# sohamazing/image-stitcher

Hardware: AMD Instinct MI355X
Metric: stitched Mvoxels/s (higher is better)
Workload: dtype u16

## Files before the change

### image-stitcher_amd/csrc/fuse.hip

```cpp
#include "fuse_device.h"

namespace {

template <typename T, int FLAT>
struct Slot {
    static constexpr int VEC = Pix<T>::N;
    u32x4 px;
    f32x4 g32[FLAT == 1 ? VEC / 4 : 1];
    f64x2 g64[FLAT == 2 ? VEC / 2 : 1];
    T edge;
    float eg32;
    double eg64;
};

template <typename T, int FLAT>
__device__ __forceinline__ void slot_load(Slot<T, FLAT> &S, const Row<T> &J, int lane, int k) {
    constexpr int VEC = Pix<T>::N;
    const int v = lane + 64 * k;
    if (v >= J.v_first && v < J.v_end) {
        const int p0 = v * VEC - J.mis;
        S.px = ldg<U32x4U>(J.srow + p0);
        if (FLAT == 1 && J.frow) {
#pragma unroll
            for (int q = 0; q < VEC / 4; ++q) S.g32[q] = ldg<F32x4U>(reinterpret_cast<const float *>(J.frow) + p0 + 4 * q);
// ... 136 lines not shown
                row_zero<T>(d - head, n + head, lane, leave_tail);
            } else {
                row_zero<T>(d, n, lane, leave_tail);
            }
        }
        return;
    }
    for (int rb = wave; rb < rows; rb += 4 * RB) {
        Row<T> J[RB];
#pragma unroll
        for (int j = 0; j < RB; ++j) {
            const int r = rb + 4 * j;
            J[j].n = r < rows ? n : 0;
            J[j].drow = canvas + (int64_t)(it.dst_y + r) * P.canvas_pitch + it.dst_x;
            J[j].srow = tile + (int64_t)(it.b + r) * P.tile_pitch + it.c;
            J[j].frow = flat ? flat + ((int64_t)(it.b + r) * P.tile_w + it.c) * FSZ : nullptr;
            const bool lt = has_left && !lzero;
            J[j].lsrow = lt ? ltile + (int64_t)(seam.b + r) * P.tile_pitch + seam.c : J[j].srow;
            J[j].lfrow = (lt && flat) ? flat + ((int64_t)(seam.b + r) * P.tile_w + seam.c) * FSZ : J[j].frow;
            row_setup<T>(J[j], lane, sflags);
        }
        if (fast) pipeline_rows<T, FLAT, true, RND, RB, SLOTS, DEPTH>(J, lane);
        else pipeline_rows<T, FLAT, false, RND, RB, SLOTS, DEPTH>(J, lane);
    }
}

struct PlaneAux {
    const void *tile, *ltile;
    Seam seam;
};
template <typename T>
__device__ __forceinline__ PlaneAux plane_aux(const FuseParams &P, int plane, const Item &it, int64_t pos) {
    PlaneAux A;
    A.tile = it.nref ? tile_ptr<T>(P, plane, it.a) : nullptr;
    A.seam = (sizeof(T) == 2 && P.seams) ? P.seams[pos] : Seam{-1, 0, 0, 0};
    A.ltile = ((A.seam.flags & SEAM_HAS_LEFT) && !(A.seam.flags & SEAM_LEFT_ZERO)) ? tile_ptr<T>(P, plane, A.seam.a) : nullptr;
    return A;
}

template <typename T, int FLAT, bool DYN>
__global__ __launch_bounds__(256, (FLAT == 1 ? (sizeof(T) == 2 ? WAVES_F32 : 1) : (FLAT == 2 ? WAVES_F64 : WAVES_PLAIN)))
void fuse_overwrite_kernel(const FuseParams P, const int64_t n_items, const int64_t n_work) {
    const int wave = __builtin_amdgcn_readfirstlane(threadIdx.x >> 6);
    const int lane = threadIdx.x & 63;

    if (!DYN) {
        int64_t work = blockIdx.x;
        if (work >= n_work) return;
        int plane = (int)(work / n_items);
        Item it = P.items[work - plane * n_items];
        PlaneAux A = plane_aux<T>(P, plane, it, work - plane * n_items);
        while (true) {
            const int64_t nwork = work + gridDim.x;
            const bool more = nwork < n_work;
            int nplane = plane;
            Item nit = it;
            PlaneAux nA = A;
            if (more) {
                nplane = (int)(nwork / n_items);
                nit = P.items[nwork - nplane * n_items];
                nA = plane_aux<T>(P, nplane, nit, nwork - nplane * n_items);
            }
            process_item<T, FLAT>(P, plane, it, static_cast<const T *>(A.tile), wave, lane, A.seam, static_cast<const T *>(A.ltile));
            if (!more) break;
            work = nwork;
            plane = nplane;
            it = nit;
            A = nA;
        }
        return;
    }
    for_each_queued_item<PlaneAux>(
        P, n_items, (uint32_t)P.n_planes,
        [&](int plane, const Item &it, int64_t pos) -> PlaneAux { return plane_aux<T>(P, plane, it, pos); },
        [&](int plane, const Item &it, const PlaneAux &A) {
            process_item<T, FLAT>(P, plane, it, sgpr(static_cast<const T *>(A.tile)), wave, lane, sgpr(A.seam),
                                  sgpr(static_cast<const T *>(A.ltile)));
        });
}

struct UnitAux {
    PlaneGroup g;
    const void *tile[ZB];
    const void *ltile[ZB];
    Seam seam;
    Seam first;
};
struct FeatherAux : UnitAux {
    Seam xref[2];
    const void *xtile[2][ZB];
};

template <bool FULL, int RND = 0, typename G = float, typename T = uint16_t>
__device__ __forceinline__ void process_item_zg(const FuseParams &P, const UnitAux &A, const int gn, const Item &it,
                                                const int wave, const int lane) {
    constexpr bool GAINS = !std::is_same<G, NoGain>::value;
    typedef typename std::conditional<GAINS, G, float>::type GT;
    constexpr uint32_t GSZ = sizeof(GT), TSZ = sizeof(T), TMAX = sizeof(T) == 1 ? 255u : 65535u;
    constexpr int VEC = 16 / (int)sizeof(T), LINE = 128 / (int)sizeof(T);
    constexpr int SLOTS = BLOCK_COLS / VEC / 64 + 1;
    const int rows = it.hw >> 16, n = it.hw & 0xFFFF;
    const int sflags = sizeof(T) == 2 ? sgpr(A.seam.flags) : 0;
    const bool leave_tail = sflags & SEAM_LEAVE_TAIL;
    T *cplane[ZB];
    const T *tiles[ZB];
#pragma unroll
    for (int z = 0; z < ZB; ++z) {
        const int zz = (FULL || z < gn) ? z : 0;
        cplane[z] = static_cast<T *>(P.canvas) + (int64_t)sgpr(A.g.plane[zz]) * P.canvas_plane_stride;
        tiles[z] = sgpr(static_cast<const T *>(A.tile[zz]));
    }
    if (!it.nref) {
        const bool has_left = sflags & SEAM_HAS_LEFT, lzero = sflags & SEAM_LEFT_ZERO;
        for (int r = wave; r < rows; r += 4) {
            const int64_t doff = (int64_t)(it.dst_y + r) * P.canvas_pitch + it.dst_x;
            const int mis = (int)((reinterpret_cast<uintptr_t>(cplane[0] + doff) / sizeof(T)) & (LINE - 1));
            const int head = (has_left && mis > 0) ? mis : 0;
            if (head && !lzero) {
                const int p = lane - mis;
                const bool left = p < 0;
                const int po = left ? p : -1;
                const int sb = sgpr(A.seam.b), sc = sgpr(A.seam.c);
                GT eg = GT(1), er = GT(1);
                if constexpr (GAINS) {
                    const GT *lflat = static_cast<const GT *>(P.flat_ptrs[sgpr(A.g.plane[0])]);
                    eg = ldg_s<GT>(reinterpret_cast<const char *>(lflat + (int64_t)(sb + r) * P.tile_w + sc) + po * (int)GSZ);
                    er = recip_of<RND>(eg);
                }
#pragma unroll
                for (int z = 0; z < ZB; ++z)
                    if (FULL || z < gn) {
                        const T *lt = sgpr(static_cast<const T *>(A.ltile[z]));
                        const T e = ldg_s<T>(reinterpret_cast<const char *>(lt + (int64_t)(sb + r) * P.tile_pitch + sc) + po * (int)TSZ);
                        uint32_t kq = e;
                        if constexpr (GAINS) kq = min(cvt_u32_sat(quot_of<RND>((GT)e, eg, er)), TMAX);
                        if (!left) kq = 0u;
                        stg_s<T>(reinterpret_cast<char *>(cplane[z] + doff) + p * (int)TSZ, (T)kq);
                    }
            }
#pragma unroll
            for (int z = 0; z < ZB; ++z)
                if (FULL || z < gn) {
                    T *d = cplane[z] + doff;
                    if (head && lzero) row_zero<T>(d - head, n + head, lane, leave_tail);
                    else if (head) row_zero<T>(d + (LINE - head), n - (LINE - head), lane, leave_tail);
                    else row_zero<T>(d, n, lane, leave_tail);
                }
        }
        return;
    }
    const GT *flat = nullptr;
    if constexpr (GAINS) flat = static_cast<const GT *>(P.flat_ptrs[sgpr(A.g.plane[0])]);
    for (int r = wave; r < rows; r += 4) {
        const int64_t doff = (int64_t)(it.dst_y + r) * P.canvas_pitch + it.dst_x;
        const int64_t soff = (int64_t)(it.b + r) * P.tile_pitch + it.c;
        const char *frow = GAINS ? reinterpret_cast<const char *>(flat + (int64_t)(it.b + r) * P.tile_w + it.c) : nullptr;
        const char *srow[ZB];
        char *drow[ZB];
#pragma unroll
        for (int z = 0; z < ZB; ++z) {
            srow[z] = reinterpret_cast<const char *>(tiles[z] + soff);
            drow[z] = reinterpret_cast<char *>(cplane[z] + doff);
        }
        const int mis = (int)((reinterpret_cast<uintptr_t>(drow[0]) / sizeof(T)) & (LINE - 1));
        const bool head_line = (sflags & SEAM_HAS_LEFT) && mis > 0;
        const int n_own = leave_tail ? n - ((n + mis) & (LINE - 1)) : n;
        const int v_first = head_line ? LINE / VEC : (mis + VEC - 1) / VEC, v_end = (n_own + mis) / VEC;
#pragma unroll
        for (int k = 0; k < SLOTS; ++k) {
            if (64 * k >= v_end || v_end <= v_first) break;
            const int v = lane + 64 * k;
            const bool act = v >= v_first && v < v_end;
            const int p0 = v * VEC - mis;
            const uint32_t o = (uint32_t)min(max(p0, v_first * VEC - mis), (v_end - 1) * VEC - mis);
            GT g[VEC], rc[VEC];
            if constexpr (GAINS) load_gains(frow + o * GSZ, g);
            u32x4 px[ZB];
#pragma unroll
            for (int z = 0; z < ZB; ++z)
                if (FULL || z < gn) px[z] = ldg<U32x4U>(srow[z] + o * TSZ);
            if constexpr (GAINS) {
#pragma unroll
                for (int c = 0; c < VEC; ++c) rc[c] = recip_of<RND>(g[c]);
            }
#pragma unroll
            for (int z = 0; z < ZB; ++z)
                if (FULL || z < gn) {
                    u32x4 ov = px[z];
                    if constexpr (GAINS) {
#pragma unroll
                        for (int c = 0; c < 4; ++c) {
                            if constexpr (sizeof(T) == 2) ov[c] = quot_pair<RND, GT>(px[z][c], g[2 * c], g[2 * c + 1], rc[2 * c], rc[2 * c + 1]);
                            else ov[c] = quot_quad<RND, GT>(px[z][c], &g[4 * c], &rc[4 * c]);
                        }
                    }
                    if (act) stg_nt_at(drow[z], o * TSZ, ov);
                }
        }
        if (head_line) {
            const int p = lane - mis;
            const bool left = p < 0, lzero = sflags & SEAM_LEFT_ZERO;
            const int sb = sgpr(A.seam.b), sc = sgpr(A.seam.c);
            const int po = (left && lzero) ? 0 : p;
            GT eg = GT(1), er = GT(1);
            if constexpr (GAINS) {
                const char *lfrow = lzero ? frow : reinterpret_cast<const char *>(flat + (int64_t)(sb + r) * P.tile_w + sc);
                eg = ldg_s<GT>((left ? lfrow : frow) + po * (int)GSZ);
            }
            T e[ZB];
#pragma unroll
            for (int z = 0; z < ZB; ++z)
                if (FULL || z < gn) {
                    const T *lt = sgpr(static_cast<const T *>(A.ltile[z]));
                    const char *lrow = lzero ? srow[z] : reinterpret_cast<const char *>(lt + (int64_t)(sb + r) * P.tile_pitch + sc);
                    e[z] = ldg_s<T>((left ? lrow : srow[z]) + po * (int)TSZ);
                }
            if constexpr (GAINS) er = recip_of<RND>(eg);
#pragma unroll
            for (int z = 0; z < ZB; ++z)
                if (FULL || z < gn) {
                    uint32_t kq = e[z];
                    if constexpr (GAINS) kq = min(cvt_u32_sat(quot_of<RND>((GT)e[z], eg, er)), TMAX);
                    if (left && lzero) kq = 0;
                    stg_s<T>(drow[z] + p * (int)TSZ, (T)kq);
                }
        }
        const int head_end = head_line ? 0 : min(n_own, v_first * VEC - mis);
        const int tail_start = max(head_end, v_end * VEC - mis);
        int ep = -1;
        if (lane < VEC) {
            if (lane < head_end) ep = lane;
        } else if (lane < 2 * VEC) {
            if (tail_start + (lane - VEC) < n_own) ep = tail_start + (lane - VEC);
        }
        if (__builtin_amdgcn_ballot_w64(ep >= 0)) {
            const uint32_t eo = (uint32_t)max(ep, 0);
            GT eg = GT(1), er = GT(1);
            if constexpr (GAINS) eg = ldg_s<GT>(frow + eo * GSZ);
            T e[ZB];
#pragma unroll
            for (int z = 0; z < ZB; ++z)
                if (FULL || z < gn) e[z] = ldg_s<T>(srow[z] + eo * TSZ);
            if constexpr (GAINS) er = recip_of<RND>(eg);
#pragma unroll
            for (int z = 0; z < ZB; ++z)
                if (FULL || z < gn) {
                    uint32_t kq = e[z];
                    if constexpr (GAINS) kq = min(cvt_u32_sat(quot_of<RND>((GT)e[z], eg, er)), TMAX);
                    if (ep >= 0) stg_s<T>(drow[z] + eo * TSZ, (T)kq);
                }
        }
    }
}

constexpr int WAVES_ZG = 1;
template <typename G, bool DYN, typename T = uint16_t>
__global__ __launch_bounds__(256, WAVES_ZG) void fuse_overwrite_zg_kernel(const FuseParams P, const int64_t n_items) {
    constexpr int FLAT = std::is_same<G, NoGain>::value ? 0 : (sizeof(G) == 8 ? 2 : 1);
    const int wave = __builtin_amdgcn_readfirstlane(threadIdx.x >> 6);
    const int lane = threadIdx.x & 63;
    const uint32_t n_groups = *P.n_groups;
    auto pre = [&](int unit, const Item &it, int64_t pos) -> UnitAux {
        UnitAux A;
        A.g = P.groups[unit];
        A.seam = P.seams ? P.seams[pos] : Seam{-1, 0, 0, 0};
        const bool left_tile = (A.seam.flags & SEAM_HAS_LEFT) && !(A.seam.flags & SEAM_LEFT_ZERO);
#pragma unroll
        for (int z = 0; z < ZB; ++z) {
            A.tile[z] = (it.nref && z < A.g.n) ? tile_ptr<T>(P, A.g.plane[z], it.a) : nullptr;
            A.ltile[z] = (left_tile && z < A.g.n) ? tile_ptr<T>(P, A.g.plane[z], A.seam.a) : nullptr;
        }
        return A;
    };
    auto body = [&](int, const Item &it, const UnitAux &A) {
        const int gn = sgpr(A.g.n);
        if (gn == 1) {
            process_item<T, FLAT>(P, sgpr(A.g.plane[0]), it, sgpr(static_cast<const T *>(A.tile[0])), wave, lane, sgpr(A.seam),
                                  sgpr(static_cast<const T *>(A.ltile[0])));
        } else if (gn == ZB) {
            process_item_zg<true, 0, G, T>(P, A, gn, it, wave, lane);
        } else {
            process_item_zg<false, 0, G, T>(P, A, gn, it, wave, lane);
        }
    };
    if (DYN) {
        for_each_queued_item<UnitAux>(P, n_items, n_groups, pre, body);
    } else {
        __shared__ Item s_it;
        __shared__ UnitAux s_A;
        const int64_t n_work = (int64_t)n_groups * n_items;
        for (int64_t work = blockIdx.x; work < n_work; work += gridDim.x) {
            __syncthreads();
            if (threadIdx.x == 0) {
                const int unit = (int)(work / n_items);
                s_it = P.items[work - unit * n_items];
                s_A = pre(unit, s_it, work - unit * n_items);
            }
            __syncthreads();
            body(0, sgpr(s_it), s_A);
        }
    }
}

__global__ __launch_bounds__(256) void build_groups_kernel(const void *const *flat_ptrs, const uint32_t *cls, uint32_t cls_mask,
                                                          int n_planes, int64_t plane_stride_bytes, int zb, uint32_t *n_groups,
                                                          PlaneGroup *groups, bool consecutive) {
    constexpr int CAP = 1024;
    __shared__ uint64_t key[CAP];
    __shared__ int first[CAP], open_group[CAP];
    __shared__ short members[CAP], dealt[CAP];
    __shared__ PlaneGroup out[CAP];
    const int tid = threadIdx.x;
    if (n_planes > CAP || zb <= 1) {
        for (int p = tid; p < n_planes; p += 256) {
            PlaneGroup g{};
            g.n = 1;
            g.plane[0] = p;
            groups[p] = g;
        }
        if (tid == 0) *n_groups = (uint32_t)n_planes;
        return;
    }
    for (int p = tid; p < n_planes; p += 256) {
        const void *f = flat_ptrs ? flat_ptrs[p] : nullptr;
        const bool ok = flat_ptrs ? (f && (cls[p] & cls_mask) == 0) : true;
        key[p] = ok ? ((reinterpret_cast<uint64_t>(f) << 7) | (uint64_t)(((int64_t)p * plane_stride_bytes) & 127) | (1ull << 63)) : 0;
        open_group[p] = -1;
    }
    __syncthreads();
    for (int p = tid; p < n_planes; p += 256) {
        int f = p;
        if (key[p])
            for (int q = 0; q < p; ++q)
                if (key[q] == key[p]) {
                    f = q;
                    break;
                }
        first[p] = f;
    }
    __syncthreads();
    if (tid == 0) {
        int ng = 0;
        for (int p = 0; p < n_planes; ++p) members[p] = dealt[p] = 0;
        for (int p = 0; p < n_planes; ++p)
            if (key[p]) ++members[first[p]];
        for (int p = 0; p < n_planes; ++p) {
            if (!key[p]) {
                open_group[p] = ng++;
            } else if (first[p] == p) {
                open_group[p] = ng;
                ng += (members[p] + zb - 1) / zb;
            }
        }
        for (int g = 0; g < ng; ++g) out[g].n = 0;
        for (int p = 0; p < n_planes; ++p) {
            int g = open_group[p];
            if (key[p]) {
                const int lead = first[p];
                const int j = dealt[lead]++;
                g = open_group[lead] + (consecutive ? j / zb : j % ((members[lead] + zb - 1) / zb));
            }
            out[g].plane[out[g].n++] = p;
        }
        for (int g = 0; g < ng; ++g)
            for (int z = out[g].n; z < 7; ++z) out[g].plane[z] = out[g].plane[0];
        *n_groups = (uint32_t)ng;
        first[0] = ng;
    }
    __syncthreads();
    const int ng = first[0];
    for (int g = tid; g < ng; g += 256) groups[g] = out[g];
}

template <typename OutT>
__device__ __forceinline__ OutT feather_out(float o) {
    if (sizeof(OutT) == 4) return (OutT)o;
    const float hi = sizeof(OutT) == 1 ? 255.0f : 65535.0f;
    return (OutT)fminf(fmaxf(rintf(o), 0.0f), hi);
}

constexpr int BLEND_MAXR = 4;

template <typename T, typename OutT, int FLAT, bool FAST>
__device__ __forceinline__ void blend_group(const FuseParams &P, int plane, const Item &it, const char *flat, int r, int p0,
                                            OutT *dst) {
    constexpr int VEC = 8;
    constexpr int MAXR = BLEND_MAXR;
    const int nref = it.nref;
    float acc[VEC], wsum[VEC], last[VEC];
#pragma unroll
    for (int e = 0; e < VEC; ++e) acc[e] = wsum[e] = last[e] = 0.0f;
    auto blend = [&](const float (&px)[VEC], int y, int x0) {
        const int wy = min(y + 1, P.tile_h - y);
#pragma unroll
        for (int e = 0; e < VEC; ++e) {
            const int x = x0 + e;
            const float w = (float)min(min(x + 1, P.tile_w - x), wy);
            acc[e] = __fadd_rn(acc[e], __fmul_rn(w, px[e]));
            wsum[e] = __fadd_rn(wsum[e], w);
            last[e] = px[e];
        }
    };
    if (sizeof(T) == 2 && FLAT != 2 && nref <= MAXR) {
        u32x4 raw[MAXR];
        f32x4 g[MAXR][2];
        int ys[MAXR], xs[MAXR];
#pragma unroll
        for (int k = 0; k < MAXR; ++k)
            if (k < nref) {
                const Ref rf = P.refs[it.a + k];
                ys[k] = rf.src_y + it.b + r;
                xs[k] = rf.src_x + it.c + p0;
                raw[k] = ldg<U32x4U>(tile_ptr<T>(P, plane, rf.tile) + (int64_t)ys[k] * P.tile_pitch + xs[k]);
                if (FLAT == 1 && flat) {
                    const float *gp = reinterpret_cast<const float *>(flat) + (int64_t)ys[k] * P.tile_w + xs[k];
                    g[k][0] = ldg<F32x4U>(gp);
                    g[k][1] = ldg<F32x4U>(gp + 4);
                }
            }
#pragma unroll
        for (int k = 0; k < MAXR; ++k)
            if (k < nref) {
                float px[VEC];
#pragma unroll
                for (int e = 0; e < VEC; ++e) {
                    px[e] = (float)Pix<uint16_t>::get(raw[k], e);
                    if (FLAT == 1 && flat) px[e] = FAST ? div_u16_normal_ieee(px[e], g[k][e >> 2][e & 3]) : __fdiv_rn(px[e], g[k][e >> 2][e & 3]);
                }
                blend(px, ys[k], xs[k]);
            }
    } else {
        for (int k = 0; k < nref; ++k) {
            const Ref rf = P.refs[it.a + k];
            const T *tile = tile_ptr<T>(P, plane, rf.tile);
            const int y = rf.src_y + it.b + r;
            const int x0 = rf.src_x + it.c + p0;
            const T *src = tile + (int64_t)y * P.tile_pitch + x0;
            float px[VEC];
            if (sizeof(T) == 2) {
                const u32x4 raw = ldg<U32x4U>(src);
#pragma unroll
                for (int e = 0; e < VEC; ++e) px[e] = (float)Pix<uint16_t>::get(raw, e);
            } else {
#pragma unroll
                for (int e = 0; e < VEC; ++e) px[e] = (float)ldg_s<T>(src + e);
            }
            if (FLAT && flat) {
#pragma unroll
                for (int e = 0; e < VEC; ++e) {
                    const char *gp = flat + ((int64_t)y * P.tile_w + x0 + e) * (FLAT == 2 ? 8 : 4);
                    const float gain = FLAT == 2 ? (float)ldg_s<double>(gp) : ldg_s<float>(gp);
                    px[e] = FAST ? div_u16_normal_ieee(px[e], gain) : __fdiv_rn(px[e], gain);
                }
            }
            blend(px, y, x0);
        }
    }
    OutT o[VEC];
#pragma unroll
    for (int e = 0; e < VEC; ++e) o[e] = feather_out<OutT>(nref == 1 ? last[e] : (nref ? __fdiv_rn(acc[e], wsum[e]) : 0.0f));
    if (sizeof(OutT) == 2) {
        u32x4 out;
#pragma unroll
        for (int q = 0; q < 4; ++q) out[q] = (uint32_t)(uint16_t)o[2 * q] | ((uint32_t)(uint16_t)o[2 * q + 1] << 16);
        stg_nt(dst, out);
    } else if (sizeof(OutT) == 4) {
        u32x4 lo, hi;
#pragma unroll
        for (int q = 0; q < 4; ++q) {
            lo[q] = __float_as_uint((float)o[q]);
            hi[q] = __float_as_uint((float)o[4 + q]);
        }
        stg_nt(dst, lo);
        stg_nt(dst + 4, hi);
    } else {
#pragma unroll
        for (int e = 0; e < VEC; ++e) stg_s<OutT>(dst + e, o[e]);
    }
}

template <typename T, typename OutT, int FLAT, bool FAST>
__device__ __forceinline__ void blend_item(const FuseParams &P, int plane, const Item &it, int tid) {
    constexpr int VEC = 8;
    const int rows = it.hw >> 16, n = it.hw & 0xFFFF;
    const int nref = it.nref;
    OutT *canvas = static_cast<OutT *>(P.canvas) + plane * P.canvas_plane_stride;
    const char *flat = (FLAT && P.flat_ptrs) ? static_cast<const char *>(P.flat_ptrs[plane]) : nullptr;
    const int G = n / VEC + 1;
    auto locate = [&](int idx, int &r, int &p0, OutT *&dst) -> bool {
        r = idx / G;
        const int j = idx - r * G;
        OutT *drow = canvas + (int64_t)(it.dst_y + r) * P.canvas_pitch + it.dst_x;
        const int mis = (int)((reinterpret_cast<uintptr_t>(drow) / sizeof(OutT)) & (VEC - 1));
        const int v = (mis ? 1 : 0) + j;
        p0 = v * VEC - mis;
        dst = drow + p0;
        return v < (n + mis) / VEC;
    };
    for (int idx = tid; idx < rows * G; idx += 256) {
        int r, p0;
        OutT *dst;
        if (!locate(idx, r, p0, dst)) continue;
        blend_group<T, OutT, FLAT, FAST>(P, plane, it, flat, r, p0, dst);
    }
    for (int idx = tid; idx < rows * 2 * VEC; idx += 256) {
        const int r = idx / (2 * VEC), l = idx - r * 2 * VEC;
        OutT *drow = canvas + (int64_t)(it.dst_y + r) * P.canvas_pitch + it.dst_x;
        const int mis = (int)((reinterpret_cast<uintptr_t>(drow) / sizeof(OutT)) & (VEC - 1));
        const int v_first = mis ? 1 : 0, v_end = (n + mis) / VEC;
        const int head_end = min(n, v_first * VEC - mis);
        const int tail_start = max(head_end, v_end * VEC - mis);
        int p = -1;
        if (l < VEC) {
            if (l < head_end) p = l;
        } else if (tail_start + (l - VEC) < n) {
            p = tail_start + (l - VEC);
        }
        if (p < 0) continue;
        float acc = 0.0f, wsum = 0.0f, last = 0.0f;
        for (int k = 0; k < nref; ++k) {
            const Ref rf = P.refs[it.a + k];
            const int y = rf.src_y + it.b + r, x = rf.src_x + it.c + p;
            float v = (float)ldg_s<T>(tile_ptr<T>(P, plane, rf.tile) + (int64_t)y * P.tile_pitch + x);
            if (FLAT && flat) {
                const char *gp = flat + ((int64_t)y * P.tile_w + x) * (FLAT == 2 ? 8 : 4);
                const float gain = FLAT == 2 ? (float)ldg_s<double>(gp) : ldg_s<float>(gp);
                v = FAST ? div_u16_normal_ieee(v, gain) : __fdiv_rn(v, gain);
            }
            const float w = (float)min(min(x + 1, P.tile_w - x), min(y + 1, P.tile_h - y));
            acc = __fadd_rn(acc, __fmul_rn(w, v));
            wsum = __fadd_rn(wsum, w);
            last = v;
        }
        stg_s<OutT>(drow + p, feather_out<OutT>(nref == 1 ? last : (nref ? __fdiv_rn(acc, wsum) : 0.0f)));
    }
}

template <typename T, typename OutT, int FLAT>
__device__ __forceinline__ void feather_one_item(const FuseParams &P, int plane, const Item &it, int wave, int lane) {
    const int nref = it.nref;
    if (sizeof(OutT) == sizeof(T) && FLAT != 2 && nref <= 1) {
        Item one = it;
        const T *tile = nullptr;
        if (nref) {
            const Ref rf = P.refs[it.a];
            tile = tile_ptr<T>(P, plane, rf.tile);
            one.a = rf.tile;
            one.b = rf.src_y + it.b;
            one.c = rf.src_x + it.c;
        }
        process_item<T, FLAT == 2 ? 0 : FLAT, 1>(P, plane, one, tile, wave, lane);
        return;
    }
    const bool fast = FLAT == 1 && P.flat_class && (P.flat_class[plane] & 1u) == 0;
    if (fast) blend_item<T, OutT, FLAT, true>(P, plane, it, threadIdx.x);
    else blend_item<T, OutT, FLAT, false>(P, plane, it, threadIdx.x);
}

constexpr int WAVES_FEATHER_F32 = 4;
template <typename T, typename OutT, int FLAT, bool DYN>
__global__ __launch_bounds__(256, (FLAT == 1 && sizeof(T) == 2 && sizeof(OutT) == 2 ? WAVES_FEATHER_F32 : 1))
void fuse_feather_kernel(const FuseParams P, const int64_t n_items, const int64_t n_work) {
    const int wave = __builtin_amdgcn_readfirstlane(threadIdx.x >> 6);
    const int lane = threadIdx.x & 63;
    if (DYN) {
        for_each_queued_item<int>(P, n_items, (uint32_t)P.n_planes, [](int, const Item &, int64_t) -> int { return 0; },
                                  [&](int plane, const Item &it, const int &) { feather_one_item<T, OutT, FLAT>(P, plane, it, wave, lane); });
    } else {
        for (int64_t work = blockIdx.x; work < n_work; work += gridDim.x) {
            const int plane = (int)(work / n_items);
            feather_one_item<T, OutT, FLAT>(P, plane, P.items[work - plane * n_items], wave, lane);
        }
    }
}

__device__ __forceinline__ float div_by_refined(float n, float d, float r) {
    const float q = n * r;
    return fmaf(fmaf(-d, q, n), r, q);
}

template <int FLAT, bool FULL, typename OutT = uint16_t, int NREF = 2>
__device__ __forceinline__ void blend_item_zg(const FuseParams &P, const UnitAux &A, const int gn, const Item &it, const int tid) {
    typedef uint16_t T;
    constexpr int VEC = 8;
    constexpr bool F32OUT = sizeof(OutT) == 4;
    static_assert(NREF == 2 || F32OUT, "one-tile and empty items of an integer canvas take process_item_zg");
    const int rows = it.hw >> 16, n = it.hw & 0xFFFF;
    OutT *cplane[ZB];
    const T *t0[ZB], *t1[ZB];
#pragma unroll
    for (int z = 0; z < ZB; ++z) {
        const int zz = (FULL || z < gn) ? z : 0;
        cplane[z] = static_cast<OutT *>(P.canvas) + (int64_t)sgpr(A.g.plane[zz]) * P.canvas_plane_stride;
        t0[z] = sgpr(static_cast<const T *>(A.tile[zz]));
        t1[z] = sgpr(static_cast<const T *>(A.ltile[zz]));
    }
    typedef typename std::conditional<FLAT == 2, double, float>::type GM;
    const GM *flat = (FLAT && NREF) ? static_cast<const GM *>(P.flat_ptrs[sgpr(A.g.plane[0])]) : nullptr;
    const int ya = sgpr(A.first.b), xa = sgpr(A.first.c), yb = sgpr(A.seam.b), xb = sgpr(A.seam.c);
    const int G = n / VEC + 1;
    auto load_gain8 = [&](int y, int x, f32x2 (&g)[4]) {
        if constexpr (FLAT == 1) {
            const float *gp = reinterpret_cast<const float *>(flat) + (int64_t)y * P.tile_w + x;
            const f32x4 a = ldg<F32x4U>(gp), b = ldg<F32x4U>(gp + 4);
            g[0] = f32x2{a[0], a[1]}, g[1] = f32x2{a[2], a[3]}, g[2] = f32x2{b[0], b[1]}, g[3] = f32x2{b[2], b[3]};
        } else if constexpr (FLAT == 2) {
            const double *gp = reinterpret_cast<const double *>(flat) + (int64_t)y * P.tile_w + x;
#pragma unroll
            for (int h = 0; h < 4; ++h) {
                const f64x2 a = ldg<F64x2U>(gp + 2 * h);
                g[h] = f32x2{(float)a[0], (float)a[1]};
            }
        }
    };
    auto refined = [](f32x2 d) {
        const f32x2 r = {__builtin_amdgcn_rcpf(d[0]), __builtin_amdgcn_rcpf(d[1])};
        return pk_fma(pk_fma(-d, r, f32x2{1.0f, 1.0f}), r, r);
    };
    for (int idx = tid; idx < rows * G; idx += 256) {
        const int r = idx / G, j = idx - r * G;
        const int64_t doff = (int64_t)(it.dst_y + r) * P.canvas_pitch + it.dst_x;
        const int mis = (int)((reinterpret_cast<uintptr_t>(cplane[0] + doff) / sizeof(OutT)) & (VEC - 1));
        const int v = (mis ? 1 : 0) + j;
        if (v >= (n + mis) / VEC) continue;
        const int p0 = v * VEC - mis;
        if constexpr (NREF == 0) {
            const u32x4 zero = {0u, 0u, 0u, 0u};
#pragma unroll
            for (int z = 0; z < ZB; ++z)
                if (FULL || z < gn) {
                    stg_nt(cplane[z] + doff + p0, zero);
                    stg_nt(cplane[z] + doff + p0 + 4, zero);
                }
            continue;
        }
        const int y0 = ya + r, x0 = xa + p0, y1 = yb + r, x1 = xb + p0;
        const int64_t s0 = (int64_t)y0 * P.tile_pitch + x0, s1 = (int64_t)y1 * P.tile_pitch + x1;
        f32x2 g0[4], g1[4];
        if constexpr (FLAT != 0) {
            load_gain8(y0, x0, g0);
            if constexpr (NREF == 2) load_gain8(y1, x1, g1);
        }
        u32x4 ra[ZB], rb[ZB];
#pragma unroll
        for (int z = 0; z < ZB; ++z)
            if (FULL || z < gn) {
                ra[z] = ldg<U32x4U>(t0[z] + s0);
                if constexpr (NREF == 2) rb[z] = ldg<U32x4U>(t1[z] + s1);
            }
        f32x2 r0[4], r1[4], w0[4], w1[4], ws[4], rw[4];
        const int wy0 = min(y0 + 1, P.tile_h - y0), wy1 = min(y1 + 1, P.tile_h - y1);
#pragma unroll
        for (int h = 0; h < 4; ++h) {
            if constexpr (FLAT != 0) {
                r0[h] = refined(g0[h]);
                if constexpr (NREF == 2) r1[h] = refined(g1[h]);
            }
            if constexpr (NREF == 2) {
#pragma unroll
                for (int c = 0; c < 2; ++c) {
                    const int e = 2 * h + c;
                    w0[h][c] = (float)min(min(x0 + e + 1, P.tile_w - (x0 + e)), wy0);
                    w1[h][c] = (float)min(min(x1 + e + 1, P.tile_w - (x1 + e)), wy1);
                }
                ws[h] = w0[h] + w1[h];
                rw[h] = refined(ws[h]);
            }
        }
#pragma unroll
        for (int z = 0; z < ZB; ++z)
            if (FULL || z < gn) {
                f32x2 o[4];
#pragma unroll
                for (int h = 0; h < 4; ++h) {
// ... 169 lines not shown
            }
    }
    for (int idx = tid; idx < rows * 2 * VEC; idx += 256) {
        const int r = idx / (2 * VEC), l = idx - r * 2 * VEC;
        const int64_t doff = (int64_t)(it.dst_y + r) * P.canvas_pitch + it.dst_x;
        const int mis = (int)((reinterpret_cast<uintptr_t>(cplane[0] + doff) / sizeof(float)) & (VEC - 1));
        const int v_first = mis ? 1 : 0, v_end = (n + mis) / VEC;
        const int head_end = min(n, v_first * VEC - mis);
        const int tail_start = max(head_end, v_end * VEC - mis);
        int p = -1;
        if (l < VEC) {
            if (l < head_end) p = l;
        } else if (tail_start + (l - VEC) < n) {
            p = tail_start + (l - VEC);
        }
        if (p < 0) continue;
        if constexpr (NREF == 0) {
#pragma unroll
            for (int z = 0; z < ZB; ++z)
                if (FULL || z < gn) stg_s<float>(cplane[z] + doff + p, 0.0f);
            continue;
        }
        const int y0 = ya + r, x0 = xa + p, y1 = yb + r, x1 = xb + p;
        const float fa = FLAT ? recip_for<1>(ldg_s<float>(flat + (int64_t)y0 * P.tile_w + x0)) : 1.0f;
        const float fb = (FLAT && NREF == 2) ? recip_for<1>(ldg_s<float>(flat + (int64_t)y1 * P.tile_w + x1)) : 1.0f;
        const float wa = (float)min(min(x0 + 1, P.tile_w - x0), min(y0 + 1, P.tile_h - y0));
        const float wb = (float)min(min(x1 + 1, P.tile_w - x1), min(y1 + 1, P.tile_h - y1));
        const float rws = recip_for<1>(__fadd_rn(wa, wb));
#pragma unroll
        for (int z = 0; z < ZB; ++z)
            if (FULL || z < gn) {
                float va = (float)ldg_s<T>(t0[z] + (int64_t)y0 * P.tile_pitch + x0);
                if (FLAT) va = __fmul_rn(va, fa);
                float o = va;
                if constexpr (NREF == 2) {
                    float vb = (float)ldg_s<T>(t1[z] + (int64_t)y1 * P.tile_pitch + x1);
                    if (FLAT) vb = __fmul_rn(vb, fb);
                    o = __fmul_rn(__fadd_rn(__fmul_rn(wa, va), __fmul_rn(wb, vb)), rws);
                }
                stg_s<float>(cplane[z] + doff + p, o);
            }
    }
}

template <int FLAT, bool FULL, typename OutT>
__device__ __forceinline__ void blend_item_zgn(const FuseParams &P, const FeatherAux &A, const int gn, const Item &it, const int tid) {
    static_assert(FLAT == 0 || FLAT == 1, "float32 gains or none");
    typedef uint16_t T;
    constexpr int VEC = 8, MAXR = 4;
    constexpr bool F32OUT = sizeof(OutT) == 4;
    const int rows = it.hw >> 16, n = it.hw & 0xFFFF;
    const bool four = sgpr((int)it.nref) == 4;
    OutT *cplane[ZB];
    const T *tp[MAXR][ZB];
#pragma unroll
    for (int z = 0; z < ZB; ++z) {
        const int zz = (FULL || z < gn) ? z : 0;
        cplane[z] = static_cast<OutT *>(P.canvas) + (int64_t)sgpr(A.g.plane[zz]) * P.canvas_plane_stride;
        tp[0][z] = sgpr(static_cast<const T *>(A.tile[zz]));
        tp[1][z] = sgpr(static_cast<const T *>(A.ltile[zz]));
        tp[2][z] = sgpr(static_cast<const T *>(A.xtile[0][zz]));
        tp[3][z] = sgpr(static_cast<const T *>(A.xtile[1][zz]));
    }
    const float *flat = FLAT ? static_cast<const float *>(P.flat_ptrs[sgpr(A.g.plane[0])]) : nullptr;
    const int ry[MAXR] = {sgpr(A.first.b), sgpr(A.seam.b), sgpr(A.xref[0].b), sgpr(A.xref[1].b)};
    const int rx[MAXR] = {sgpr(A.first.c), sgpr(A.seam.c), sgpr(A.xref[0].c), sgpr(A.xref[1].c)};
    const int G = n / VEC + 1;
    auto refined = [](f32x2 d) {
        const f32x2 r = {__builtin_amdgcn_rcpf(d[0]), __builtin_amdgcn_rcpf(d[1])};
        return pk_fma(pk_fma(-d, r, f32x2{1.0f, 1.0f}), r, r);
    };
    for (int idx = tid; idx < rows * G; idx += 256) {
        const int r = idx / G, j = idx - r * G;
        const int64_t doff = (int64_t)(it.dst_y + r) * P.canvas_pitch + it.dst_x;
        const int mis = (int)((reinterpret_cast<uintptr_t>(cplane[0] + doff) / sizeof(OutT)) & (VEC - 1));
        const int v = (mis ? 1 : 0) + j;
        if (v >= (n + mis) / VEC) continue;
        const int p0 = v * VEC - mis;
        f32x2 acc[ZB][4], ws[4];
#pragma unroll
        for (int k = 0; k < MAXR; ++k)
            if (k < 3 || four) {
                const int y = ry[k] + r, x = rx[k] + p0;
                const int64_t so = (int64_t)y * P.tile_pitch + x;
                f32x2 g[4], rr[4], w[4];
                if constexpr (FLAT != 0) {
                    const float *gp = flat + (int64_t)y * P.tile_w + x;
                    const f32x4 a = ldg<F32x4U>(gp), b = ldg<F32x4U>(gp + 4);
                    g[0] = f32x2{a[0], a[1]}, g[1] = f32x2{a[2], a[3]}, g[2] = f32x2{b[0], b[1]}, g[3] = f32x2{b[2], b[3]};
                }
                u32x4 raw[ZB];
#pragma unroll
                for (int z = 0; z < ZB; ++z)
                    if (FULL || z < gn) raw[z] = ldg<U32x4U>(tp[k][z] + so);
                const int wy = min(y + 1, P.tile_h - y);
#pragma unroll
                for (int h = 0; h < 4; ++h) {
                    if constexpr (FLAT != 0) rr[h] = refined(g[h]);
#pragma unroll
                    for (int c = 0; c < 2; ++c) w[h][c] = (float)min(min(x + 2 * h + c + 1, P.tile_w - (x + 2 * h + c)), wy);
                    ws[h] = k == 0 ? w[h] : ws[h] + w[h];
                }
#pragma unroll
                for (int z = 0; z < ZB; ++z)
                    if (FULL || z < gn) {
#pragma unroll
                        for (int h = 0; h < 4; ++h) {
                            f32x2 px = {(float)(raw[z][h] & 0xFFFFu), (float)(raw[z][h] >> 16)};
                            if constexpr (FLAT != 0) px = F32OUT ? px * rr[h] : div_by_refined2(px, g[h], rr[h]);
                            const f32x2 t = w[h] * px;
                            acc[z][h] = k == 0 ? t : acc[z][h] + t;
                        }
                    }
            }
        f32x2 rw[4];
#pragma unroll
        for (int h = 0; h < 4; ++h) rw[h] = refined(ws[h]);
#pragma unroll
        for (int z = 0; z < ZB; ++z)
            if (FULL || z < gn) {
                f32x2 o[4];
#pragma unroll
                for (int h = 0; h < 4; ++h) o[h] = F32OUT ? acc[z][h] * rw[h] : div_by_refined2(acc[z][h], ws[h], rw[h]);
                if constexpr (F32OUT) {
                    u32x4 lo, hi;
#pragma unroll
                    for (int q = 0; q < 2; ++q) {
                        lo[2 * q] = __float_as_uint(o[q][0]), lo[2 * q + 1] = __float_as_uint(o[q][1]);
                        hi[2 * q] = __float_as_uint(o[2 + q][0]), hi[2 * q + 1] = __float_as_uint(o[2 + q][1]);
                    }
                    stg_nt(cplane[z] + doff + p0, lo);
                    stg_nt(cplane[z] + doff + p0 + 4, hi);
                } else {
                    typedef unsigned short u16x2 __attribute__((ext_vector_type(2)));
                    u32x4 out;
#pragma unroll
                    for (int q = 0; q < 4; ++q) {
                        const u16x2 pk = __builtin_amdgcn_cvt_pk_u16(cvt_u32_sat(__builtin_rintf(o[q][0])), cvt_u32_sat(__builtin_rintf(o[q][1])));
                        out[q] = (uint32_t)pk[0] | ((uint32_t)pk[1] << 16);
                    }
                    stg_nt(cplane[z] + doff + p0, out);
                }
            }
    }
    for (int idx = tid; idx < rows * 2 * VEC; idx += 256) {
        const int r = idx / (2 * VEC), l = idx - r * 2 * VEC;
        const int64_t doff = (int64_t)(it.dst_y + r) * P.canvas_pitch + it.dst_x;
        const int mis = (int)((reinterpret_cast<uintptr_t>(cplane[0] + doff) / sizeof(OutT)) & (VEC - 1));
        const int v_first = mis ? 1 : 0, v_end = (n + mis) / VEC;
        const int head_end = min(n, v_first * VEC - mis);
        const int tail_start = max(head_end, v_end * VEC - mis);
        int p = -1;
        if (l < VEC) {
            if (l < head_end) p = l;
        } else if (tail_start + (l - VEC) < n) {
            p = tail_start + (l - VEC);
        }
        if (p < 0) continue;
        float acc[ZB], wsum = 0.0f;
#pragma unroll
        for (int k = 0; k < MAXR; ++k)
            if (k < 3 || four) {
                const int y = ry[k] + r, x = rx[k] + p;
                const float gk = FLAT ? ldg_s<float>(flat + (int64_t)y * P.tile_w + x) : 1.0f;
                const float fk = FLAT ? recip_for<1>(gk) : 1.0f;
                const float w = (float)min(min(x + 1, P.tile_w - x), min(y + 1, P.tile_h - y));
                wsum = k == 0 ? w : __fadd_rn(wsum, w);
#pragma unroll
                for (int z = 0; z < ZB; ++z)
                    if (FULL || z < gn) {
                        float px = (float)ldg_s<T>(tp[k][z] + (int64_t)y * P.tile_pitch + x);
                        if (FLAT) px = F32OUT ? __fmul_rn(px, fk) : div_by_refined(px, gk, fk);
                        const float t = __fmul_rn(w, px);
                        acc[z] = k == 0 ? t : __fadd_rn(acc[z], t);
                    }
            }
        const float rws = recip_for<1>(wsum);
#pragma unroll
        for (int z = 0; z < ZB; ++z)
            if (FULL || z < gn) {
                const float o = F32OUT ? __fmul_rn(acc[z], rws) : div_by_refined(acc[z], wsum, rws);
                if constexpr (F32OUT) stg_s<OutT>(cplane[z] + doff + p, o);
                else stg_s<OutT>(cplane[z] + doff + p, (OutT)min(cvt_u32_sat(__builtin_rintf(o)), 65535u));
            }
    }
}

constexpr int WAVES_FEATHER_ZG = 3;
template <int FLAT, bool DYN, typename OutT = uint16_t>
__global__ __launch_bounds__(256, FLAT ? WAVES_FEATHER_ZG : 1) void fuse_feather_zg_kernel(const FuseParams P, const int64_t n_items) {
    typedef uint16_t T;
    constexpr bool F32OUT = sizeof(OutT) == 4;
    const int wave = __builtin_amdgcn_readfirstlane(threadIdx.x >> 6);
    const int lane = threadIdx.x & 63;
    const uint32_t n_groups = *P.n_groups;
    auto pre = [&](int unit, const Item &it, int64_t) -> FeatherAux {
        FeatherAux A;
        A.g = P.groups[unit];
        A.seam = Seam{-1, 0, 0, 0};
        A.first = Seam{-1, 0, 0, 0};
        A.xref[0] = A.xref[1] = Seam{-1, 0, 0, 0};
        const bool one = it.nref >= 1 && it.nref <= 4, two = it.nref >= 2 && it.nref <= 4;
        Ref ra{}, rb{};
        if (one) {
            ra = P.refs[it.a];
            A.first = Seam{ra.tile, ra.src_y + it.b, ra.src_x + it.c, 0};
        }
        if (two) {
            rb = P.refs[it.a + 1];
            A.seam = Seam{rb.tile, rb.src_y + it.b, rb.src_x + it.c, 0};
        }
#pragma unroll
        for (int z = 0; z < ZB; ++z) {
            A.tile[z] = (one && z < A.g.n) ? tile_ptr<T>(P, A.g.plane[z], ra.tile) : nullptr;
            A.ltile[z] = (two && z < A.g.n) ? tile_ptr<T>(P, A.g.plane[z], rb.tile) : nullptr;
        }
#pragma unroll
        for (int k = 0; k < 2; ++k) {
            const bool have = it.nref >= 3 + k && it.nref <= 4;
            Ref rk{};
            if (have) {
                rk = P.refs[it.a + 2 + k];
                A.xref[k] = Seam{rk.tile, rk.src_y + it.b, rk.src_x + it.c, 0};
            }
#pragma unroll
            for (int z = 0; z < ZB; ++z) A.xtile[k][z] = (have && z < A.g.n) ? tile_ptr<T>(P, A.g.plane[z], rk.tile) : nullptr;
        }
        return A;
    };
    auto body = [&](int, const Item &it, const FeatherAux &A) {
        const int gn = sgpr(A.g.n);
        if (gn == 1) {
            feather_one_item<T, OutT, FLAT>(P, sgpr(A.g.plane[0]), it, wave, lane);
        } else if (F32OUT && it.nref <= 1) {
            if constexpr (F32OUT && FLAT != 2) {
                if (it.nref == 1) {
                    if (gn == ZB) blend_item_zg4<FLAT, true, 1>(P, A, gn, it, threadIdx.x);
                    else blend_item_zg4<FLAT, false, 1>(P, A, gn, it, threadIdx.x);
                } else {
                    if (gn == ZB) blend_item_zg4<FLAT, true, 0>(P, A, gn, it, threadIdx.x);
                    else blend_item_zg4<FLAT, false, 0>(P, A, gn, it, threadIdx.x);
                }
            } else if constexpr (F32OUT) {
                if (it.nref == 1) {
                    if (gn == ZB) blend_item_zg<FLAT, true, OutT, 1>(P, A, gn, it, threadIdx.x);
                    else blend_item_zg<FLAT, false, OutT, 1>(P, A, gn, it, threadIdx.x);
                } else {
                    if (gn == ZB) blend_item_zg<FLAT, true, OutT, 0>(P, A, gn, it, threadIdx.x);
                    else blend_item_zg<FLAT, false, OutT, 0>(P, A, gn, it, threadIdx.x);
                }
            }
        } else if (FLAT == 2 && it.nref <= 1) {
            for (int z = 0; z < gn; ++z) feather_one_item<T, OutT, FLAT>(P, sgpr(A.g.plane[z]), it, wave, lane);
        } else if (it.nref <= 1) {
            Item one = it;
            one.a = sgpr(A.first.a);
            one.b = sgpr(A.first.b);
            one.c = sgpr(A.first.c);
            if constexpr (FLAT == 2) {
            } else if (!FLAT) {
                for (int z = 0; z < gn; ++z)
                    process_item<T, 0, 1>(P, sgpr(A.g.plane[z]), one, sgpr(static_cast<const T *>(A.tile[z])), wave, lane);
            } else if (gn == ZB) {
                process_item_zg<true, 1>(P, A, gn, one, wave, lane);
            } else {
                process_item_zg<false, 1>(P, A, gn, one, wave, lane);
            }
        } else if (it.nref == 2) {
            if constexpr (F32OUT && FLAT != 2) {
                if (gn == ZB) blend_item_zg4<FLAT, true, 2>(P, A, gn, it, threadIdx.x);
                else blend_item_zg4<FLAT, false, 2>(P, A, gn, it, threadIdx.x);
            } else {
                if (gn == ZB) blend_item_zg<FLAT, true, OutT>(P, A, gn, it, threadIdx.x);
                else blend_item_zg<FLAT, false, OutT>(P, A, gn, it, threadIdx.x);
            }
        } else if (FLAT != 2 && it.nref <= 4) {
            if constexpr (FLAT != 2) {
                if (gn == ZB) blend_item_zgn<FLAT, true, OutT>(P, A, gn, it, threadIdx.x);
                else blend_item_zgn<FLAT, false, OutT>(P, A, gn, it, threadIdx.x);
            }
        } else {
            for (int z = 0; z < gn; ++z) blend_item<T, OutT, FLAT, true>(P, sgpr(A.g.plane[z]), it, threadIdx.x);
        }
    };
    if (DYN) {
        for_each_queued_item<FeatherAux>(P, n_items, n_groups, pre, body);
    } else {
        __shared__ Item s_it;
        __shared__ FeatherAux s_A;
        const int64_t n_work = (int64_t)n_groups * n_items;
        for (int64_t work = blockIdx.x; work < n_work; work += gridDim.x) {
            __syncthreads();
            if (threadIdx.x == 0) {
                const int unit = (int)(work / n_items);
                s_it = P.items[work - unit * n_items];
                s_A = pre(unit, s_it, work - unit * n_items);
            }
            __syncthreads();
            body(0, sgpr(s_it), s_A);
        }
    }
}

template <typename G>
__global__ __launch_bounds__(256) void flat_classify_kernel(const void *const *flat_ptrs, int64_t n, uint32_t *cls) {
    const int plane = blockIdx.y;
    const G *f = static_cast<const G *>(flat_ptrs[plane]);
    if (!f) return;
    for (int q = 0; q < plane; ++q)
        if (flat_ptrs[q] == f) return;
    const G lo = (G)__builtin_ldexp(1.0, FAST_MIN_EXP), hi = (G)__builtin_ldexp(1.0, FAST_END_EXP);
    const G mlo = (G)__builtin_ldexp(1.0, -MODERATE_EXP), mhi = (G)__builtin_ldexp(1.0, MODERATE_EXP);
    bool odd = false, wide = false, neg = false;
    auto look = [&](G g) {
        const G a = g < 0 ? -g : g;
        odd |= !(a >= lo && a < hi);
        wide |= !(a >= mlo && a < mhi);
        neg |= !(g > 0);
    };
    constexpr int PER = 16 / sizeof(G);
    const int64_t head = min<int64_t>(n, (int64_t)((16 - (reinterpret_cast<uintptr_t>(f) & 15)) & 15) / (int64_t)sizeof(G));
    const int64_t nvec = (n - head) / PER;
    const int64_t tid = (int64_t)blockIdx.x * blockDim.x + threadIdx.x, nthr = (int64_t)gridDim.x * blockDim.x;
    for (int64_t v = tid; v < nvec; v += nthr) {
        if constexpr (sizeof(G) == 4) {
            const f32x4 q = *reinterpret_cast<const f32x4 *>(f + head + v * PER);
            look(q[0]), look(q[1]), look(q[2]), look(q[3]);
        } else {
            const F64x2U q = *reinterpret_cast<const F64x2U *>(f + head + v * PER);
            look(q.v[0]), look(q.v[1]);
        }
    }
    for (int64_t i = tid; i < head; i += nthr) look(ldg_s<G>(f + i));
    for (int64_t i = head + nvec * PER + tid; i < n; i += nthr) look(ldg_s<G>(f + i));
    const uint32_t bits = (__builtin_amdgcn_ballot_w64(odd) ? 1u : 0u) | (__builtin_amdgcn_ballot_w64(wide) ? 2u : 0u) |
                          (__builtin_amdgcn_ballot_w64(neg) ? 4u : 0u);
    if (bits && (threadIdx.x & 63) == 0) atomicOr(&cls[plane], bits);
}

__global__ __launch_bounds__(256) void flat_class_share_kernel(const void *const *flat_ptrs, int n_planes, uint32_t *cls) {
    for (int p = threadIdx.x; p < n_planes; p += 256) {
        const void *f = flat_ptrs[p];
        if (!f) continue;
        for (int q = 0; q < p; ++q)
            if (flat_ptrs[q] == f) {
                cls[p] = cls[q];
                break;
            }
    }
}

__global__ __launch_bounds__(256) void selftest_divide_kernel(int exponent0, int negative, unsigned long long *bad) {
    const uint32_t mant = blockIdx.x * 256u + threadIdx.x;
    const int exponent = exponent0 + (int)blockIdx.y;
    const uint32_t bits = ((uint32_t)(exponent + 127) << 23) | mant | (negative ? 0x80000000u : 0u);
    const float g = __uint_as_float(bits);
    unsigned long long local = 0;
    for (int v = 0; v < 65536; ++v)
    {
        const uint32_t want = flat_f32<uint16_t>((uint16_t)v, g);
        const uint32_t pair = flat_f32_fast_pair((uint32_t)v | ((uint32_t)v << 16), g, g);
        local += want != flat_f32_fast<uint16_t>((uint16_t)v, g);
        local += want != (pair & 0xFFFFu);
        local += want != (pair >> 16);
        local += flat_f32<uint16_t, 1>((uint16_t)v, g) != flat_f32_fast<uint16_t, 1>((uint16_t)v, g);
        local += __fdiv_rn((float)v, g) != div_u16_normal_ieee((float)v, g);
    }
    for (int off = 32; off > 0; off >>= 1) local += __shfl_xor(local, off);
    if ((threadIdx.x & 63) == 0 && local) atomicAdd(bad, local);
}

}

extern "C" int sq_selftest_flat_divide(int32_t exponent, int32_t n_binades, int32_t negative, uint64_t *mismatches_dev,
                                       void *stream) {
    if (!mismatches_dev || exponent < FAST_MIN_EXP || n_binades < 1 || exponent + n_binades > FAST_END_EXP)
        return fail(SQ_ERR_INVALID, "sq_selftest_flat_divide: binades [%d, %d] outside the fast path's range [%d, %d]",
                    exponent, exponent + n_binades - 1, FAST_MIN_EXP, FAST_END_EXP - 1);
    hipStream_t s = static_cast<hipStream_t>(stream);
    hipError_t e = hipMemsetAsync(mismatches_dev, 0, sizeof(uint64_t), s);
    if (e == hipSuccess) {
        hipLaunchKernelGGL(selftest_divide_kernel, dim3(1u << 15, n_binades), dim3(256), 0, s, exponent, negative,
                           reinterpret_cast<unsigned long long *>(mismatches_dev));
        e = hipGetLastError();
    }
    if (e != hipSuccess) return fail(SQ_ERR_HIP, "sq_selftest_flat_divide: %s", hipGetErrorString(e));
    return SQ_OK;
}

__global__ __launch_bounds__(256) void selftest_blend_divide_kernel(int exponent0, int negative, unsigned long long *bad) {
    const uint32_t mant = blockIdx.x * 256u + threadIdx.x;
    const int exponent = exponent0 + (int)blockIdx.y;
    const float acc = __uint_as_float(((uint32_t)(exponent + 127) << 23) | mant | (negative ? 0x80000000u : 0u));
    unsigned long long local = 0;
    for (int ws = 2; ws <= BLEND_WSUM_MAX; ++ws) {
        const float d = (float)ws;
        const float want = __fdiv_rn(acc, d), got = div_by_refined(acc, d, recip_for<1>(d));
        local += __float_as_uint(want) != __float_as_uint(got);
    }
    if (local) atomicAdd(bad, local);
}

extern "C" int sq_selftest_blend_divide(int32_t exponent, int32_t n_binades, int32_t negative, uint64_t *mismatches_dev,
                                        void *stream) {
    if (!mismatches_dev || exponent < BLEND_ACC_MIN_EXP || n_binades < 1 || exponent + n_binades > BLEND_ACC_END_EXP)
        return fail(SQ_ERR_INVALID, "sq_selftest_blend_divide: binades [%d, %d] outside the blend's range [%d, %d]", exponent,
                    exponent + n_binades - 1, BLEND_ACC_MIN_EXP, BLEND_ACC_END_EXP - 1);
    hipStream_t s = static_cast<hipStream_t>(stream);
    hipError_t e = hipMemsetAsync(mismatches_dev, 0, sizeof(uint64_t), s);
    if (e == hipSuccess) {
        hipLaunchKernelGGL(selftest_blend_divide_kernel, dim3(1u << 15, n_binades), dim3(256), 0, s, exponent, negative,
                           reinterpret_cast<unsigned long long *>(mismatches_dev));
        e = hipGetLastError();
    }
    if (e != hipSuccess) return fail(SQ_ERR_HIP, "sq_selftest_blend_divide: %s", hipGetErrorString(e));
    return SQ_OK;
}

__global__ __launch_bounds__(256) void selftest_divide_f64_kernel(int exponent0, int negative, uint64_t seed, unsigned long long *bad) {
    const uint64_t id = ((uint64_t)blockIdx.y << 32) | (blockIdx.x * 256u + threadIdx.x);
    uint64_t x = seed + id * 0x9E3779B97F4A7C15ull;
    x ^= x >> 30; x *= 0xBF58476D1CE4E5B9ull; x ^= x >> 27; x *= 0x94D049BB133111EBull; x ^= x >> 31;
    const int exponent = exponent0 + (int)blockIdx.y;
    const uint32_t t = blockIdx.x * 256u + threadIdx.x;
    uint64_t mant = x & ((1ull << 52) - 1);
    if (t == 0) mant = 0;
    else if (t == 1) mant = (1ull << 52) - 1;
    else if (t < 54) mant = 1ull << (t - 2);
    else if (t < 106) mant = ((1ull << 52) - 1) ^ (1ull << (t - 54));
    const uint64_t bits = ((uint64_t)(exponent + 1023) << 52) | mant | (negative ? 0x8000000000000000ull : 0ull);
    const double g = __longlong_as_double((long long)bits);
    unsigned long long local = 0;
    for (int v = 0; v < 65536; ++v) {
        const double want = __ddiv_rn((double)v, g);
        const double got = div_u16_normal_f64((double)v, g);
        local += __double_as_longlong(want) != __double_as_longlong(got) && !(want == 0.0 && got == 0.0);
        local += flat_f64<uint16_t>((uint16_t)v, g) != flat_f64_fast<uint16_t>((uint16_t)v, g);
    }
    for (int off = 32; off > 0; off >>= 1) local += __shfl_xor(local, off);
    if ((threadIdx.x & 63) == 0 && local) atomicAdd(bad, local);
}

extern "C" int sq_selftest_flat_divide_f64(int32_t exponent, int32_t n_binades, int32_t negative, uint64_t seed,
                                           uint64_t *mismatches_dev, void *stream) {
    if (!mismatches_dev || exponent < FAST_MIN_EXP || n_binades < 1 || exponent + n_binades > FAST_END_EXP)
        return fail(SQ_ERR_INVALID, "sq_selftest_flat_divide_f64: binades [%d, %d] outside the fast path's range [%d, %d]",
                    exponent, exponent + n_binades - 1, FAST_MIN_EXP, FAST_END_EXP - 1);
    hipStream_t s = static_cast<hipStream_t>(stream);
    hipError_t e = hipMemsetAsync(mismatches_dev, 0, sizeof(uint64_t), s);
    if (e == hipSuccess) {
        hipLaunchKernelGGL(selftest_divide_f64_kernel, dim3(128, n_binades), dim3(256), 0, s, exponent, negative, seed,
                           reinterpret_cast<unsigned long long *>(mismatches_dev));
        e = hipGetLastError();
    }
    if (e != hipSuccess) return fail(SQ_ERR_HIP, "sq_selftest_flat_divide_f64: %s", hipGetErrorString(e));
    return SQ_OK;
}

extern "C" int64_t sq_fuse_scratch_bytes(int32_t n_planes) {
    if (n_planes < 0) return fail(SQ_ERR_INVALID, "sq_fuse_scratch_bytes: n_planes %d", n_planes);
    return scratch_layout(n_planes).total;
}

extern "C" int sq_fuse_planes(const sq_fuse_args *a, void *stream_) {
    static const char *who = "sq_fuse_planes";
    FuseParams P;
    int32_t fl = 0;
    if (const int rc = fuse_setup(who, a, fl, SQ_FUSE_FORCE_QUEUES | SQ_FUSE_FORCE_STATIC | SQ_FUSE_NO_PLANE_GROUPS | SQ_FUSE_NO_SEAM_OWNERS |
                                      SQ_FUSE_CONSECUTIVE_GROUPS, 0, true, P))
        return rc;
    const TableHeader &h = a->plan->header();
    if (a->canvas_plane_stride < (int64_t)a->canvas_h * a->canvas_pitch && a->n_planes > 1)
        return fail(SQ_ERR_INVALID, "sq_fuse_planes: canvas planes overlap");
    P.canvas_plane_stride = a->canvas_plane_stride;
    const size_t esz = a->canvas_dtype == SQ_F32 ? 4 : (size_t)a->canvas_dtype;
    hipStream_t stream = static_cast<hipStream_t>(stream_);
    const int flat = a->flat_ptrs_dev ? (a->flat_dtype == SQ_F64 ? 2 : 1) : 0;
    const ScratchLayout SL = scratch_layout(a->n_planes);
    const int64_t n_work = (int64_t)a->n_planes * h.n_items;
    if (a->scratch_dev && a->n_planes > 0) {
        if (const int rc = scratch_check(who, a, SL)) return rc;
        if (hipMemsetAsync(a->scratch_dev, 0, (size_t)SL.groups, stream) != hipSuccess)
            return fail(SQ_ERR_HIP, "sq_fuse_planes: cannot clear the scratch");
        if (flat) {
            if (flat == 1)
                hipLaunchKernelGGL(flat_classify_kernel<float>, dim3(256, a->n_planes), dim3(256), 0, stream, a->flat_ptrs_dev,
                                   (int64_t)a->tile_h * a->tile_w, static_cast<uint32_t *>(a->scratch_dev));
            else
                hipLaunchKernelGGL(flat_classify_kernel<double>, dim3(256, a->n_planes), dim3(256), 0, stream, a->flat_ptrs_dev,
                                   (int64_t)a->tile_h * a->tile_w, static_cast<uint32_t *>(a->scratch_dev));
            if (a->n_planes > 1)
                hipLaunchKernelGGL(flat_class_share_kernel, dim3(1), dim3(256), 0, stream, a->flat_ptrs_dev, a->n_planes,
                                   static_cast<uint32_t *>(a->scratch_dev));
            P.flat_class = static_cast<const uint32_t *>(a->scratch_dev);
        }
        if ((n_work >= 100000 || (fl & SQ_FUSE_FORCE_QUEUES)) && n_work < (int64_t(1) << 31) && !(fl & SQ_FUSE_FORCE_STATIC))
            P.queue = reinterpret_cast<uint32_t *>(static_cast<char *>(a->scratch_dev) + SL.queue);
    }
    const int64_t min_units = h.n_items * ((a->n_planes + ZB - 1) / ZB);
    const bool u16 = a->tile_dtype == SQ_U16;
    const bool grouping = a->scratch_dev && a->n_planes > 1 && ZB > 1 && !(fl & SQ_FUSE_NO_PLANE_GROUPS);
    auto build_groups = [&](const void *const *gains, uint32_t cls_mask) {
        char *sc = static_cast<char *>(a->scratch_dev);
        uint32_t *n_groups = reinterpret_cast<uint32_t *>(sc + SL.n_groups);
        PlaneGroup *groups = reinterpret_cast<PlaneGroup *>(sc + SL.groups);
        hipLaunchKernelGGL(build_groups_kernel, dim3(1), dim3(256), 0, stream, gains, P.flat_class, cls_mask, a->n_planes,
                           a->canvas_plane_stride * (int64_t)esz, ZB, n_groups, groups,
                           (fl & SQ_FUSE_CONSECUTIVE_GROUPS) != 0);
        P.groups = groups;
        P.n_groups = n_groups;
    };

    if (a->mode == SQ_FUSE_OVERWRITE) {
        if (a->canvas_dtype != a->tile_dtype)
            return fail(SQ_ERR_INVALID, "sq_fuse_planes: overwrite mode keeps the tile dtype (canvas %d, tile %d)",
                        a->canvas_dtype, a->tile_dtype);
#define SQ_OVERWRITE(T, F)                                                                                  \
    do {                                                                                                      \
        if (P.queue) return launch(who, fuse_overwrite_kernel<T, F, true>, P, n_work, stream, a->grid_blocks, h.n_items, n_work);  \
        return launch(who, fuse_overwrite_kernel<T, F, false>, P, n_work, stream, a->grid_blocks, h.n_items, n_work);        \
    } while (0)
        if (flat && grouping) {
            build_groups(a->flat_ptrs_dev, 1u);
#define SQ_ZG(G, T)                                                                                                                  \
    do {                                                                                                                              \
        if (P.queue) return launch(who, fuse_overwrite_zg_kernel<G, true, T>, P, min_units, stream, a->grid_blocks, h.n_items);          \
        return launch(who, fuse_overwrite_zg_kernel<G, false, T>, P, min_units, stream, a->grid_blocks, h.n_items);                      \
    } while (0)
            if (u16) {
                if (flat == 2) SQ_ZG(double, uint16_t);
                SQ_ZG(float, uint16_t);
            }
            if (flat == 2) SQ_ZG(double, uint8_t);
            SQ_ZG(float, uint8_t);
        }
        if (u16 && !flat && grouping) {
            build_groups(nullptr, 0u);
            SQ_ZG(NoGain, uint16_t);
#undef SQ_ZG
        }
        if (u16) {
            if (flat == 0) SQ_OVERWRITE(uint16_t, 0);
            if (flat == 1) SQ_OVERWRITE(uint16_t, 1);
            SQ_OVERWRITE(uint16_t, 2);
        }
        if (flat == 0) SQ_OVERWRITE(uint8_t, 0);
        if (flat == 1) SQ_OVERWRITE(uint8_t, 1);
        SQ_OVERWRITE(uint8_t, 2);
#undef SQ_OVERWRITE
    }
    const bool f32out = a->canvas_dtype == SQ_F32;
    if (!f32out && a->canvas_dtype != a->tile_dtype)
        return fail(SQ_ERR_INVALID, "sq_fuse_planes: feather canvas must be float32 or the tile dtype");
#define SQ_FEATHER_F(T, O, F)                                                                              \
    do {                                                                                                    \
        if (P.queue) return launch(who, fuse_feather_kernel<T, O, F, true>, P, n_work, stream, a->grid_blocks, h.n_items, n_work);  \
        return launch(who, fuse_feather_kernel<T, O, F, false>, P, n_work, stream, a->grid_blocks, h.n_items, n_work);      \
    } while (0)
#define SQ_FEATHER(T, O)                 \
    do {                                 \
        if (flat == 0) SQ_FEATHER_F(T, O, 0); \
        if (flat == 1) SQ_FEATHER_F(T, O, 1); \
        SQ_FEATHER_F(T, O, 2);           \
    } while (0)
    if (u16 && grouping && std::min(a->tile_h, a->tile_w) <= BLEND_WSUM_MAX) {
        build_groups(a->flat_ptrs_dev, f32out ? 7u : 3u);
#define SQ_FEATHER_ZG(F, O)                                                                                                      \
    do {                                                                                                                          \
        if (P.queue) return launch(who, fuse_feather_zg_kernel<F, true, O>, P, min_units, stream, a->grid_blocks, h.n_items);          \
        return launch(who, fuse_feather_zg_kernel<F, false, O>, P, min_units, stream, a->grid_blocks, h.n_items);                      \
    } while (0)
        if (f32out) {
            if (flat == 2) SQ_FEATHER_ZG(2, float);
            if (flat == 1) SQ_FEATHER_ZG(1, float);
            SQ_FEATHER_ZG(0, float);
        }
        if (flat == 2) SQ_FEATHER_ZG(2, uint16_t);
        if (flat == 1) SQ_FEATHER_ZG(1, uint16_t);
        SQ_FEATHER_ZG(0, uint16_t);
#undef SQ_FEATHER_ZG
    }
    if (u16) {
        if (f32out) SQ_FEATHER(uint16_t, float);
        SQ_FEATHER(uint16_t, uint16_t);
    }
    if (f32out) SQ_FEATHER(uint8_t, float);
    SQ_FEATHER(uint8_t, uint8_t);
#undef SQ_FEATHER
#undef SQ_FEATHER_F
}
```

### image-stitcher_amd/csrc/plan.cpp

```cpp
#include <hip/hip_runtime.h>

#include <algorithm>
#include <cstdlib>
#include <cstring>
#include <exception>
#include <mutex>
#include <thread>
#include <vector>

#include "common.h"

namespace sq {
std::string &last_error_ref() {
    static thread_local std::string msg;
    return msg;
}
}

using namespace sq;

namespace {

template <typename F>
void parallel_ranges(int nthreads, size_t n, F fn) {
    if (nthreads <= 1 || n == 0) {
        fn(0, (size_t)0, n);
        return;
    }
    std::vector<std::thread> pool;
    pool.reserve(nthreads - 1);
    std::exception_ptr failed;
    std::mutex failed_mutex;
    auto bound = [&](int t) { return n * (size_t)t / (size_t)nthreads; };
    auto run = [&](int t) {
        try {
            fn(t, bound(t), bound(t + 1));
        } catch (...) {
            std::lock_guard<std::mutex> lock(failed_mutex);
            if (!failed) failed = std::current_exception();
        }
    };
    try {
        for (int t = 1; t < nthreads; ++t) pool.emplace_back(run, t);
    } catch (...) {
        std::lock_guard<std::mutex> lock(failed_mutex);
        if (!failed) failed = std::current_exception();
    }
    run(0);
    for (auto &th : pool) th.join();
    if (failed) std::rethrow_exception(failed);
}

template <typename F>
sq_fuse_plan *guarded(const char *what, F make) {
    try {
        return make();
    } catch (const std::bad_alloc &) {
        sq::fail(SQ_ERR_INVALID, "%s: out of host memory while planning", what);
    } catch (const std::exception &e) {
        sq::fail(SQ_ERR_INVALID, "%s: %s", what, e.what());
    } catch (...) {
        sq::fail(SQ_ERR_INVALID, "%s: unknown failure while planning", what);
    }
    return nullptr;
}

struct Clipped {
    int y0, y1, x0, x1;
    int src_y, src_x;
    int tile;
};

}

namespace {
struct TableSlab {
    void *ptr;
    size_t capacity;
};
std::mutex g_pool_mutex;
std::vector<TableSlab> g_pool;
constexpr size_t POOL_MAX_SLABS = 4;
bool g_pinning_failed = false;
}

void *sq_table_acquire(size_t bytes, size_t *capacity, bool *pinned) {
    {
        std::lock_guard<std::mutex> lock(g_pool_mutex);
        for (size_t i = 0; i < g_pool.size(); ++i)
            if (g_pool[i].capacity >= bytes && g_pool[i].capacity <= 2 * bytes + (1 << 20)) {
                const TableSlab slab = g_pool[i];
                g_pool.erase(g_pool.begin() + (long)i);
                *capacity = slab.capacity;
                *pinned = true;
                return slab.ptr;
            }
    }
    if (!g_pinning_failed) {
        const size_t cap = (bytes + (bytes >> 2) + 4095) & ~size_t(4095);
        void *p = nullptr;
        if (hipHostMalloc(&p, cap, hipHostMallocDefault) == hipSuccess && p) {
            *capacity = cap;
            *pinned = true;
            return p;
        }
        (void)hipGetLastError();
        g_pinning_failed = true;
    }
    *capacity = bytes;
    *pinned = false;
    return malloc(bytes);
}

void sq_table_release(void *ptr, size_t capacity, bool pinned) {
    if (!pinned) {
        free(ptr);
        return;
    }
    {
        std::lock_guard<std::mutex> lock(g_pool_mutex);
        if (g_pool.size() < POOL_MAX_SLABS) {
            g_pool.push_back({ptr, capacity});
            return;
        }
    }
    (void)hipHostFree(ptr);
}

extern "C" {

int sq_version(void) { return SQ_VERSION; }
const char *sq_last_error(void) { return last_error_ref().c_str(); }

}

namespace {
struct SpanStage {
    std::vector<Span> spans;
    std::vector<Ref> refs;
    int max_refs = 0;
    int64_t covered = 0;
};

bool make_spans(const sq_rect *rects, int32_t n_rects, int32_t tile_h, int32_t tile_w, int32_t canvas_h, int32_t canvas_w,
                int32_t mode, const char *who, SpanStage &S) {
    std::vector<Span> &spans = S.spans;
    std::vector<Ref> &refs = S.refs;
    int &max_refs = S.max_refs;
    int64_t &covered = S.covered;
    if ((!rects && n_rects > 0) || n_rects < 0 || tile_h <= 0 || tile_w <= 0 || canvas_h <= 0 || canvas_w <= 0) {
        fail(SQ_ERR_INVALID, "%s: bad sizes (n_rects=%d tile=%dx%d canvas=%dx%d)", who, n_rects, tile_h,
             tile_w, canvas_h, canvas_w);
        return false;
    }
    if (mode != SQ_FUSE_OVERWRITE && mode != SQ_FUSE_FEATHER) {
        fail(SQ_ERR_INVALID, "%s: unknown mode %d", who, mode);
        return false;
    }
    std::vector<Clipped> cl;
    cl.reserve(n_rects);
    for (int i = 0; i < n_rects; ++i) {
        const sq_rect &r = rects[i];
        if (r.h < 0 || r.w < 0 || r.src_y0 < 0 || r.src_x0 < 0 || r.src_y0 + (int64_t)r.h > tile_h ||
            r.src_x0 + (int64_t)r.w > tile_w) {
            fail(SQ_ERR_INVALID, "%s: rect %d reads outside its %dx%d tile (src %d,%d size %dx%d)", who, i,
                 tile_h, tile_w, r.src_y0, r.src_x0, r.h, r.w);
            return false;
        }
        if (r.dst_y < 0 || r.dst_x < 0) {
            fail(SQ_ERR_INVALID, "%s: rect %d has a negative canvas offset (%d,%d)", who, i, r.dst_y,
                 r.dst_x);
            return false;
        }
        int h = std::min<int64_t>(r.h, (int64_t)canvas_h - r.dst_y);
        int w = std::min<int64_t>(r.w, (int64_t)canvas_w - r.dst_x);
        if (h <= 0 || w <= 0) continue;
        cl.push_back({r.dst_y, r.dst_y + h, r.dst_x, r.dst_x + w, r.src_y0, r.src_x0, i});
    }

    std::vector<int> ys = {0, canvas_h};
    for (auto &c : cl) {
        ys.push_back(c.y0);
        ys.push_back(c.y1);
    }
    std::sort(ys.begin(), ys.end());
    ys.erase(std::unique(ys.begin(), ys.end()), ys.end());

    std::vector<int> by_y0(cl.size());
    for (size_t i = 0; i < cl.size(); ++i) by_y0[i] = (int)i;
    std::stable_sort(by_y0.begin(), by_y0.end(), [&](int a, int b) { return cl[a].y0 < cl[b].y0; });

    struct Owners {
        int n = 0;
        int v[MAX_REFS];
        bool operator==(const Owners &o) const {
            if (n != o.n) return false;
            for (int i = 0; i < n; ++i)
                if (v[i] != o.v[i]) return false;
            return true;
        }
    };
    struct Run {
        int xa, xb;
        Owners own;
    };
    const size_t n_bands = ys.size() - 1;
    const int hw_sweep = (int)std::max(1u, std::min(16u, std::thread::hardware_concurrency()));
    const int sweep_threads = n_bands >= 512 ? hw_sweep : 1;
    std::vector<std::vector<Run>> runs_of(sweep_threads);
    std::vector<std::vector<uint32_t>> run_end(sweep_threads);
    std::vector<size_t> first_band(sweep_threads + 1, 0);
    std::vector<int> overflow_at(sweep_threads, -1);
    std::vector<int> overflow_x(sweep_threads, 0);
    parallel_ranges(sweep_threads, n_bands, [&](int t, size_t b_lo, size_t b_hi) {
        first_band[t] = b_lo;
        if (t + 1 == sweep_threads) first_band[t + 1] = n_bands;
        std::vector<Run> &out = runs_of[t];
        std::vector<uint32_t> &ends = run_end[t];
        out.reserve((b_hi - b_lo) * 72);
        ends.reserve(b_hi - b_lo);
        if (b_lo >= b_hi) return;
        std::vector<int> active;
        const int y_first = ys[b_lo];
        for (size_t i = 0; i < cl.size(); ++i)
            if (cl[i].y0 <= y_first && cl[i].y1 > y_first) active.push_back((int)i);
        size_t next = (size_t)(std::upper_bound(by_y0.begin(), by_y0.end(), y_first, [&](int y, int i) { return y < cl[i].y0; }) - by_y0.begin());
        std::vector<int> xs, owner_of, skip;
        for (size_t b = b_lo; b < b_hi; ++b) {
            const int ya = ys[b];
            while (next < by_y0.size() && cl[by_y0[next]].y0 <= ya) {
                active.insert(std::upper_bound(active.begin(), active.end(), by_y0[next]), by_y0[next]);
                ++next;
            }
            active.erase(std::remove_if(active.begin(), active.end(), [&](int i) { return cl[i].y1 <= ya; }), active.end());

            xs.clear();
            xs.push_back(0);
            xs.push_back(canvas_w);
            for (int i : active) {
                xs.push_back(cl[i].x0);
                xs.push_back(cl[i].x1);
            }
            std::sort(xs.begin(), xs.end());
            xs.erase(std::unique(xs.begin(), xs.end()), xs.end());
            const size_t m = xs.size() - 1;
            if (mode == SQ_FUSE_OVERWRITE) {
                owner_of.assign(m, -1);
                skip.resize(m + 1);
                for (size_t k = 0; k <= m; ++k) skip[k] = (int)k;
                auto find = [&](int k) {
                    while (skip[k] != k) k = skip[k] = skip[skip[k]];
                    return k;
                };
                for (size_t a = active.size(); a-- > 0;) {
                    const Clipped &c = cl[active[a]];
                    const int lo = (int)(std::lower_bound(xs.begin(), xs.end(), c.x0) - xs.begin());
                    const int hi = (int)(std::lower_bound(xs.begin(), xs.end(), c.x1) - xs.begin());
                    for (int k = find(lo); k < hi; k = find(k + 1)) {
                        owner_of[k] = active[a];
                        skip[k] = k + 1;
                    }
                }
            }
            bool have = false;
            Run cur{};
            for (size_t k = 0; k < m; ++k) {
                const int xa = xs[k], xb = xs[k + 1];
                Owners own;
                if (mode == SQ_FUSE_OVERWRITE) {
                    if (owner_of[k] >= 0) own.v[own.n++] = owner_of[k];
                } else {
                    for (int i : active)
                        if (cl[i].x0 <= xa && cl[i].x1 >= xb) {
                            if (own.n == MAX_REFS) {
                                if (overflow_at[t] < 0) {
                                    overflow_at[t] = ya;
                                    overflow_x[t] = xa;
                                }
                                break;
                            }
                            own.v[own.n++] = i;
                        }
                }
                if (have && cur.own == own && cur.xb == xa) {
                    cur.xb = xb;
                } else {
                    if (have) out.push_back(cur);
                    cur.xa = xa;
                    cur.xb = xb;
                    cur.own = own;
                    have = true;
                }
            }
            if (have) out.push_back(cur);
            ends.push_back((uint32_t)out.size());
        }
    });
    for (int t = 0; t < sweep_threads; ++t)
        if (overflow_at[t] >= 0) {
            fail(SQ_ERR_UNSUPPORTED, "%s: more than %d tiles overlap at canvas (%d,%d)", who, MAX_REFS, overflow_at[t],
                 overflow_x[t]);
            return false;
        }
    struct Open {
        int xa, xb;
        int64_t index;
        const Run *run;
    };
    std::vector<Open> open, open_next;
    for (int t = 0; t < sweep_threads; ++t) {
        const std::vector<Run> &rs = runs_of[t];
        size_t at = 0;
        for (size_t k = 0; k < run_end[t].size(); ++k) {
            const size_t b = first_band[t] + k;
            const int ya = ys[b], yb = ys[b + 1];
            open_next.clear();
            size_t op = 0;
            for (; at < run_end[t][k]; ++at) {
                const Run &cur = rs[at];
                while (op < open.size() && open[op].xa < cur.xa) ++op;
                int64_t index;
                if (op < open.size() && open[op].xa == cur.xa && open[op].xb == cur.xb && open[op].run->own == cur.own) {
                    index = open[op].index;
                    spans[index].h += yb - ya;
                } else {
                    Span sp{};
                    sp.dst_y = ya;
                    sp.dst_x = cur.xa;
                    sp.h = yb - ya;
                    sp.w = cur.xb - cur.xa;
                    sp.nref = cur.own.n;
                    sp.ref0 = (int)refs.size();
                    for (int q = 0; q < cur.own.n; ++q) {
                        const Clipped &c = cl[cur.own.v[q]];
                        refs.push_back({c.tile, c.src_y + (ya - c.y0), c.src_x + (cur.xa - c.x0), 0});
                    }
                    index = (int64_t)spans.size();
                    spans.push_back(sp);
                }
                open_next.push_back({cur.xa, cur.xb, index, &cur});
                if (cur.own.n) covered += (int64_t)(yb - ya) * (cur.xb - cur.xa);
                max_refs = std::max(max_refs, cur.own.n);
            }
            open.swap(open_next);
        }
    }
    return true;
}
}

extern "C" {

static sq_fuse_plan *plan_create_impl(const sq_rect *rects, int32_t n_rects, int32_t tile_h, int32_t tile_w,
                                      int32_t canvas_h, int32_t canvas_w, int32_t mode) {
    SpanStage S;
    if (!make_spans(rects, n_rects, tile_h, tile_w, canvas_h, canvas_w, mode, "sq_fuse_plan_create", S)) return nullptr;
    std::vector<Span> &spans = S.spans;
    std::vector<Ref> &refs = S.refs;
    const int max_refs = S.max_refs;
    const int64_t covered = S.covered;

    constexpr int NX = 8;
    const int nblk = tile_h / BLOCK_ROWS + 2;
    const bool ow_mode = mode == SQ_FUSE_OVERWRITE;
    auto rows_of = [&](const Span &sp) { return (!ow_mode && sp.nref >= 2) ? FEATHER_BLEND_ROWS : BLOCK_ROWS; };
    auto col_pieces = [&](const Span &sp) {
        int n = 0;
        for (int c0 = 0; c0 < sp.w; ++n) {
            int cols = std::min(BLOCK_COLS, sp.w - c0);
            const int rest = sp.w - c0 - cols;
            if (ow_mode && rest > 0 && rest < SEAM_MIN_COLS) cols -= SEAM_MIN_COLS;
            c0 += cols;
        }
        return n;
    };
    std::vector<size_t> span_first(spans.size() + 1, 0);
    for (size_t si = 0; si < spans.size(); ++si) {
        const Span &sp = spans[si];
        const int item_rows = rows_of(sp);
        const int64_t row_steps = sp.h <= 0 ? 0
                                  : (ow_mode ? ((int64_t)(sp.dst_y + sp.h - 1) / item_rows - sp.dst_y / item_rows + 1)
                                             : ((int64_t)sp.h + item_rows - 1) / item_rows);
        span_first[si + 1] = span_first[si] + (size_t)(row_steps * col_pieces(sp));
    }
    static thread_local std::vector<Item> items_tls;
    static thread_local std::vector<Seam> seams_tls;
    static thread_local std::vector<int32_t> by_band_tls;
    std::vector<Item> &items = items_tls;
    std::vector<Seam> &seams = seams_tls;
    std::vector<int32_t> &by_band = by_band_tls;
    items.resize(span_first.back());
    const int hw_threads = (int)std::max(1u, std::min(8u, std::thread::hardware_concurrency()));
    const int nthreads = items.size() >= 32768 ? hw_threads : 1;
    parallel_ranges(nthreads, spans.size(), [&](int, size_t si_lo, size_t si_hi) {
        for (size_t si = si_lo; si < si_hi; ++si) {
            const Span &sp = spans[si];
            const bool ow = ow_mode;
            const Ref *rf = (ow && sp.nref) ? &refs[sp.ref0] : nullptr;
            const int item_rows = rows_of(sp);
            Item *out = items.data() + span_first[si];
            for (int r0 = 0; r0 < sp.h;) {
                const int rows = std::min(ow ? item_rows - (sp.dst_y + r0) % item_rows : item_rows, sp.h - r0);
                for (int c0 = 0; c0 < sp.w;) {
                    int cols = std::min(BLOCK_COLS, sp.w - c0);
                    const int rest = sp.w - c0 - cols;
                    if (ow && rest > 0 && rest < SEAM_MIN_COLS) cols -= SEAM_MIN_COLS;
                    Item it;
                    it.dst_y = sp.dst_y + r0;
                    it.dst_x = sp.dst_x + c0;
                    it.hw = (rows << 16) | cols;
                    it.nref = sp.nref;
                    it.span = (int32_t)si;
                    if (ow) {
                        it.a = rf ? rf->tile : -1;
                        it.b = rf ? rf->src_y + r0 : 0;
                        it.c = rf ? rf->src_x + c0 : 0;
                    } else {
                        it.a = sp.ref0;
                        it.b = r0;
                        it.c = c0;
                    }
                    *out++ = it;
                    c0 += cols;
                }
                r0 += rows;
            }
        }
    });
    const int64_t n_items = (int64_t)items.size();

    seams.clear();
    if (mode == SQ_FUSE_OVERWRITE) {
        seams.assign(items.size(), Seam{-1, 0, 0, 0});
        const int nb = canvas_h / BLOCK_ROWS + 1;
        std::vector<int32_t> first(nb + 1, 0);
        by_band.resize(items.size());
        for (const Item &it : items) ++first[it.dst_y / BLOCK_ROWS + 1];
        for (int k = 0; k < nb; ++k) first[k + 1] += first[k];
        {
            std::vector<int32_t> at(first.begin(), first.end() - 1);
            for (size_t i = 0; i < items.size(); ++i) by_band[at[items[i].dst_y / BLOCK_ROWS]++] = (int32_t)i;
        }
        auto end_key = [&](int32_t i) { return ((int64_t)items[i].dst_y << 32) | (uint32_t)(items[i].dst_x + (items[i].hw & 0xFFFF)); };
        parallel_ranges(nthreads, (size_t)nb, [&](int, size_t k_lo, size_t k_hi) {
            for (size_t k = k_lo; k < k_hi; ++k)
                std::sort(by_band.begin() + first[k], by_band.begin() + first[k + 1],
                          [&](int32_t a, int32_t b) { return end_key(a) < end_key(b); });
        });
        parallel_ranges(nthreads, items.size(), [&](int, size_t j_lo, size_t j_hi) {
            for (size_t j = j_lo; j < j_hi; ++j) {
                const Item &J = items[j];
                if ((J.hw & 0xFFFF) < SEAM_MIN_COLS || J.dst_x == 0) continue;
                const int k = J.dst_y / BLOCK_ROWS;
                const int64_t want = ((int64_t)J.dst_y << 32) | (uint32_t)J.dst_x;
                auto lo = std::lower_bound(by_band.begin() + first[k], by_band.begin() + first[k + 1], want,
                                           [&](int32_t a, int64_t key) { return end_key(a) < key; });
                if (lo == by_band.begin() + first[k + 1] || end_key(*lo) != want) continue;
                const Item &I = items[*lo];
                const int in = I.hw & 0xFFFF;
                if ((I.hw >> 16) != (J.hw >> 16) || in < SEAM_MIN_COLS) continue;
                seams[j].a = I.a;
                seams[j].b = I.b;
                seams[j].c = I.c + in;
                __atomic_fetch_or(&seams[j].flags, SEAM_HAS_LEFT | (I.nref ? 0 : SEAM_LEFT_ZERO), __ATOMIC_RELAXED);
                __atomic_fetch_or(&seams[*lo].flags, SEAM_LEAVE_TAIL, __ATOMIC_RELAXED);
            }
        });
    }

    auto key_of = [&](const Item &it) {
        if (!ow_mode) return it.nref ? std::min((refs[it.a].src_y + it.b) / BLOCK_ROWS, nblk - 2) : nblk - 1;
        return it.nref ? std::min(it.b / BLOCK_ROWS, nblk - 2) : nblk - 1;
    };
    std::vector<std::vector<int64_t>> hist(nthreads, std::vector<int64_t>(nblk, 0));
    parallel_ranges(nthreads, items.size(), [&](int t, size_t lo, size_t hi) {
        std::vector<int64_t> &h = hist[t];
        for (size_t i = lo; i < hi; ++i) ++h[key_of(items[i])];
    });
    std::vector<int64_t> count(nblk, 0);
    for (int t = 0; t < nthreads; ++t)
        for (int k = 0; k < nblk; ++k) {
            const int64_t c = hist[t][k];
            hist[t][k] = count[k];
            count[k] += c;
        }
    std::vector<int64_t> lane_base(nblk, 0), lane_len(NX, 0);
    for (int k = 0; k < nblk - 1; ++k) {
        lane_base[k] = lane_len[k % NX];
        lane_len[k % NX] += count[k];
    }
    int64_t common = lane_len[0];
    for (int x = 1; x < NX; ++x) common = std::min(common, lane_len[x]);
    std::vector<int64_t> tail_at(NX, 0);
    int64_t zero_at = common * NX;
    for (int x = 0; x < NX; ++x) {
        tail_at[x] = zero_at;
        zero_at += lane_len[x] - common;
    }

    auto *plan = new sq_fuse_plan;
    TableHeader hd{};
    hd.magic = TABLE_MAGIC;
    hd.mode = mode;
    hd.canvas_h = canvas_h;
    hd.canvas_w = canvas_w;
    hd.tile_h = tile_h;
    hd.tile_w = tile_w;
    hd.n_tiles = n_rects;
    hd.max_refs = max_refs;
    hd.n_spans = (int64_t)spans.size();
    hd.n_refs = (int64_t)refs.size();
    hd.n_items = n_items;
    hd.lane_items = common;
    hd.off_spans = sizeof(TableHeader);
    hd.off_refs = hd.off_spans + hd.n_spans * (int64_t)sizeof(Span);
    hd.off_items = hd.off_refs + hd.n_refs * (int64_t)sizeof(Ref);
    hd.covered_voxels = covered;
    hd.off_seams = seams.empty() ? 0 : hd.off_items + hd.n_items * (int64_t)sizeof(Item);
    const int64_t total = hd.off_items + hd.n_items * (int64_t)sizeof(Item) + (int64_t)(seams.size() * sizeof(Seam));
    if (!plan->table.allocate((size_t)total)) {
        delete plan;
        fail(SQ_ERR_INVALID, "sq_fuse_plan_create: out of host memory for a %lld-byte table", (long long)total);
        return nullptr;
    }
    char *p = plan->table.ptr;
    std::memcpy(p, &hd, sizeof hd);
    if (!spans.empty()) std::memcpy(p + hd.off_spans, spans.data(), spans.size() * sizeof(Span));
    if (!refs.empty()) std::memcpy(p + hd.off_refs, refs.data(), refs.size() * sizeof(Ref));
    Item *dst = reinterpret_cast<Item *>(p + hd.off_items);
    Seam *dst_seam = seams.empty() ? nullptr : reinterpret_cast<Seam *>(p + hd.off_seams);
    auto place = [&](int64_t pos, size_t i) {
        dst[pos] = items[i];
        if (dst_seam) dst_seam[pos] = seams[i];
    };
    parallel_ranges(nthreads, items.size(), [&](int th, size_t lo, size_t hi) {
        std::vector<int64_t> seen = hist[th];
        for (size_t i = lo; i < hi; ++i) {
            const int k = key_of(items[i]);
            const int64_t j = seen[k]++;
            int64_t pos;
            if (k == nblk - 1) {
                pos = zero_at + j;
            } else {
                const int x = k % NX;
                const int64_t t = lane_base[k] + j;
                pos = t < common ? t * NX + x : tail_at[x] + (t - common);
            }
            place(pos, i);
        }
    });
    constexpr size_t SCRATCH_KEEP_BYTES = (size_t)64 << 20;
    if (items.capacity() * sizeof(Item) + seams.capacity() * sizeof(Seam) + by_band.capacity() * sizeof(int32_t) > SCRATCH_KEEP_BYTES) {
        std::vector<Item>().swap(items);
        std::vector<Seam>().swap(seams);
        std::vector<int32_t>().swap(by_band);
    }
    return plan;
}

static sq_fuse_plan *plan_create_spans_impl(const sq_rect *rects, int32_t n_rects, int32_t tile_h, int32_t tile_w,
                                        int32_t canvas_h, int32_t canvas_w, int32_t mode) {
    if (mode != SQ_FUSE_OVERWRITE) {
        fail(SQ_ERR_UNSUPPORTED, "sq_fuse_plan_create_spans: overwrite plans only (mode %d)", mode);
        return nullptr;
    }
    SpanStage S;
    if (!make_spans(rects, n_rects, tile_h, tile_w, canvas_h, canvas_w, mode, "sq_fuse_plan_create_spans", S)) return nullptr;
    const size_t ns = S.spans.size();
    std::vector<int64_t> span_first(ns + 1, 0);
    for (size_t i = 0; i < ns; ++i) {
        const Span &sp = S.spans[i];
        int pieces = 0;
        for (int c0 = 0; c0 < sp.w; ++pieces) {
            int cols = std::min(BLOCK_COLS, sp.w - c0);
            const int rest = sp.w - c0 - cols;
            if (rest > 0 && rest < SEAM_MIN_COLS) cols -= SEAM_MIN_COLS;
            c0 += cols;
        }
        const int64_t row_steps = sp.h <= 0 ? 0 : ((int64_t)(sp.dst_y + sp.h - 1) / BLOCK_ROWS - sp.dst_y / BLOCK_ROWS + 1);
        span_first[i + 1] = span_first[i] + row_steps * pieces;
    }
    const int64_t n_items = span_first[ns];
    if (n_items >= (int64_t(1) << 30)) {
        fail(SQ_ERR_UNSUPPORTED, "sq_fuse_plan_create_spans: %lld items", (long long)n_items);
        return nullptr;
    }
    auto *plan = new sq_fuse_plan;
    TableHeader hd{};
    hd.magic = TABLE_MAGIC;
    hd.mode = mode;
    hd.canvas_h = canvas_h;
    hd.canvas_w = canvas_w;
    hd.tile_h = tile_h;
    hd.tile_w = tile_w;
    hd.n_tiles = n_rects;
    hd.max_refs = S.max_refs;
    hd.n_spans = (int64_t)ns;
    hd.n_refs = (int64_t)S.refs.size();
    hd.n_items = n_items;
    hd.off_spans = sizeof(TableHeader);
    hd.off_refs = hd.off_spans + hd.n_spans * (int64_t)sizeof(Span);
    hd.off_items = hd.off_refs + hd.n_refs * (int64_t)sizeof(Ref);
    hd.covered_voxels = S.covered;
    hd.lane_items = 0;
    hd.off_seams = n_items ? hd.off_items + n_items * (int64_t)sizeof(Item) : 0;
    plan->spans_only = true;
    plan->full_bytes = hd.off_items + n_items * (int64_t)(sizeof(Item) + sizeof(Seam));
    plan->off_span_first = (hd.off_items + 7) & ~int64_t(7);
    const int64_t host_bytes = plan->off_span_first + (int64_t)(ns + 1) * 8;
    if (!plan->table.allocate((size_t)host_bytes)) {
        delete plan;
        fail(SQ_ERR_INVALID, "sq_fuse_plan_create_spans: out of host memory for a %lld-byte table", (long long)host_bytes);
        return nullptr;
    }
    char *p = plan->table.ptr;
    std::memset(p, 0, (size_t)host_bytes);
    std::memcpy(p, &hd, sizeof hd);
    if (ns) std::memcpy(p + hd.off_spans, S.spans.data(), ns * sizeof(Span));
    if (!S.refs.empty()) std::memcpy(p + hd.off_refs, S.refs.data(), S.refs.size() * sizeof(Ref));
    std::memcpy(p + plan->off_span_first, span_first.data(), (ns + 1) * 8);
    return plan;
}


sq_fuse_plan *sq_fuse_plan_create(const sq_rect *rects, int32_t n_rects, int32_t tile_h, int32_t tile_w, int32_t canvas_h,
                                  int32_t canvas_w, int32_t mode) {
    return guarded("sq_fuse_plan_create", [&] { return plan_create_impl(rects, n_rects, tile_h, tile_w, canvas_h, canvas_w, mode); });
}

sq_fuse_plan *sq_fuse_plan_create_spans(const sq_rect *rects, int32_t n_rects, int32_t tile_h, int32_t tile_w, int32_t canvas_h,
                                        int32_t canvas_w, int32_t mode) {
    return guarded("sq_fuse_plan_create_spans",
                   [&] { return plan_create_spans_impl(rects, n_rects, tile_h, tile_w, canvas_h, canvas_w, mode); });
}

void sq_fuse_plan_destroy(sq_fuse_plan *plan) { delete plan; }

int sq_fuse_plan_upload(const sq_fuse_plan *plan, void *table_dev, int64_t table_bytes, void *stream_) {
    if (!plan || !table_dev) return fail(SQ_ERR_INVALID, "sq_fuse_plan_upload: NULL argument");
    if (plan->spans_only) return fail(SQ_ERR_INVALID, "sq_fuse_plan_upload: a plan of sq_fuse_plan_create_spans is completed on the device by sq_fuse_plan_expand");
    if (table_bytes < (int64_t)plan->table.size())
        return fail(SQ_ERR_INVALID, "sq_fuse_plan_upload: buffer %lld < table %zu bytes", (long long)table_bytes,
                    plan->table.size());
    hipStream_t stream = static_cast<hipStream_t>(stream_);
    hipError_t e = hipMemcpyAsync(table_dev, plan->table.data(), plan->table.size(), hipMemcpyHostToDevice, stream);
    if (e == hipSuccess) e = hipStreamSynchronize(stream);
    if (e != hipSuccess) return fail(SQ_ERR_HIP, "sq_fuse_plan_upload: %s", hipGetErrorString(e));
    return SQ_OK;
}

int64_t sq_fuse_plan_table_bytes(const sq_fuse_plan *plan) {
    if (!plan) return fail(SQ_ERR_INVALID, "sq_fuse_plan_table_bytes: NULL plan");
    return plan->device_bytes();
}

int sq_fuse_plan_export(const sq_fuse_plan *plan, void *host_buf, int64_t host_bytes) {
    if (!plan || !host_buf) return fail(SQ_ERR_INVALID, "sq_fuse_plan_export: NULL argument");
    if (plan->spans_only) return fail(SQ_ERR_INVALID, "sq_fuse_plan_export: the items of a plan of sq_fuse_plan_create_spans exist on the device only (read the table back from there)");
    if (host_bytes < (int64_t)plan->table.size())
        return fail(SQ_ERR_INVALID, "sq_fuse_plan_export: buffer %lld < table %zu bytes", (long long)host_bytes,
                    plan->table.size());
    std::memcpy(host_buf, plan->table.data(), plan->table.size());
    return SQ_OK;
}

int sq_fuse_plan_stats(const sq_fuse_plan *plan, int64_t *n_spans, int64_t *n_items, int64_t *covered_voxels,
                       int32_t *max_refs) {
    if (!plan) return fail(SQ_ERR_INVALID, "sq_fuse_plan_stats: NULL plan");
    const TableHeader &h = plan->header();
    if (n_spans) *n_spans = h.n_spans;
    if (n_items) *n_items = h.n_items;
    if (covered_voxels) *covered_voxels = h.covered_voxels;
    if (max_refs) *max_refs = h.max_refs;
    return SQ_OK;
}

}
```

### image-stitcher_amd/native.py

```python
from __future__ import annotations

import contextlib
import ctypes as C
import os
from typing import Optional, Sequence

import numpy as np

_HERE = os.path.dirname(os.path.abspath(__file__))
LIB_PATH = os.environ.get('SQ_LIB_PATH') or os.path.join(_HERE, 'csrc', 'libsquidstitch.so')

SQ_U8, SQ_U16, SQ_F32, SQ_F64 = 1, 2, 4, 8
SQ_ERR_INVALID, SQ_ERR_HIP, SQ_ERR_UNSUPPORTED, SQ_ERR_WORKSPACE, SQ_ERR_NUMERIC = -1, -2, -3, -4, -5
SQ_FUSE_OVERWRITE, SQ_FUSE_FEATHER = 0, 1
SQ_NORM_NONE, SQ_NORM_PHASE = 0, 1
SQ_FUSE_FORCE_QUEUES, SQ_FUSE_FORCE_STATIC, SQ_FUSE_NO_PLANE_GROUPS, SQ_FUSE_NO_SEAM_OWNERS, SQ_FUSE_CONSECUTIVE_GROUPS = 1, 2, 4, 8, 16
SQ_PROJECT_ACCUMULATE = 32
SQ_FOCUS_ACCUMULATE = 32
SQ_SELECT_ACCUMULATE = 32
SQ_FOCUS_MAX_RADIUS = 15
SQ_FOCUS_MAX_PLANES = 256
SQ_VERSION = 108
SQ_ARENA_NATURAL_ORDER = 1
SQ_ARENA_TWO_CLASSES = 2
SQ_ARENA_MAX_CLASSES = 8

RECT_DTYPE = np.dtype([('src_y0', '<i4'), ('src_x0', '<i4'), ('h', '<i4'), ('w', '<i4'),
                       ('dst_y', '<i4'), ('dst_x', '<i4')])
PAIR_DTYPE = np.dtype([('ref_tile', '<i4'), ('mov_tile', '<i4'), ('ref_y0', '<i4'), ('ref_x0', '<i4'),
                       ('mov_y0', '<i4'), ('mov_x0', '<i4')])
RESULT_DTYPE = np.dtype([('coarse', '<i4', (2,)), ('fine', '<i4', (2,)), ('ccmax_re', '<f8'),
                         ('ccmax_im', '<f8'), ('src_amp', '<f8'), ('tgt_amp', '<f8')])
SYNTH_DTYPE = np.dtype([('scene_seed', '<u8'), ('noise_seed', '<u8'), ('oy', '<i8'), ('ox', '<i8')])
OVERLAP_BATCH = 65535
OVERLAP_DTYPE = np.dtype([('ref_tile', '<i4'), ('mov_tile', '<i4'), ('ref_y0', '<i4'), ('ref_x0', '<i4'),
                          ('mov_y0', '<i4'), ('mov_x0', '<i4'), ('h', '<i4'), ('w', '<i4')])


class NativeError(RuntimeError):

    def __init__(self, message, status=None):
        super().__init__(message)
        self.status = status


class _FuseArgs(C.Structure):
    _fields_ = [
        ('plan', C.c_void_p), ('table_dev', C.c_void_p), ('table_bytes', C.c_int64),
        ('tile_ptrs_dev', C.c_void_p), ('tile_base_dev', C.c_void_p),
        ('tile_plane_stride', C.c_int64), ('tile_stride', C.c_int64),
        ('n_tiles', C.c_int32), ('tile_h', C.c_int32), ('tile_w', C.c_int32),
        ('tile_pitch', C.c_int32), ('tile_dtype', C.c_int32),
        ('flat_ptrs_dev', C.c_void_p), ('flat_dtype', C.c_int32),
        ('canvas_dev', C.c_void_p), ('canvas_plane_stride', C.c_int64),
        ('canvas_h', C.c_int32), ('canvas_w', C.c_int32), ('canvas_pitch', C.c_int32),
        ('canvas_dtype', C.c_int32), ('n_planes', C.c_int32), ('mode', C.c_int32),
        ('scratch_dev', C.c_void_p), ('scratch_bytes', C.c_int64),
        ('flags', C.c_int32), ('grid_blocks', C.c_int32),
    ]


class _FocusArgs(C.Structure):
    _fields_ = [
        ('z_levels_dev', C.c_void_p), ('radius', C.c_int32),
        ('scratch_dev', C.c_void_p), ('scratch_bytes', C.c_int64),
        ('key_dev', C.c_void_p), ('key_pitch', C.c_int32),
    ]


class _RegisterArgs(C.Structure):
    _fields_ = [
        ('tile_ptrs_dev', C.c_void_p), ('tile_base_dev', C.c_void_p), ('tile_stride', C.c_int64),
        ('n_tiles', C.c_int32), ('tile_h', C.c_int32), ('tile_w', C.c_int32),
        ('tile_pitch', C.c_int32), ('tile_dtype', C.c_int32),
        ('minmax_dev', C.c_void_p), ('pairs_dev', C.c_void_p), ('n_pairs', C.c_int32),
        ('n0', C.c_int32), ('n1', C.c_int32), ('upsample_factor', C.c_int32), ('normalization', C.c_int32),
        ('results_dev', C.c_void_p), ('workspace_dev', C.c_void_p), ('workspace_bytes', C.c_int64),
    ]


class _RegisterPlan(C.Structure):
    _fields_ = [
        ('m0', C.c_int32), ('m1', C.c_int32), ('long0', C.c_int32), ('long1', C.c_int32),
        ('gen0', C.c_int32), ('gen1', C.c_int32), ('nf0', C.c_int32), ('nf1', C.c_int32),
        ('radix0', C.c_uint8 * 16), ('radix1', C.c_uint8 * 16),
        ('tc', C.c_int32), ('share', C.c_int32), ('col_threads', C.c_int32),
        ('columns_single', C.c_int32), ('columns_single_threads', C.c_int32),
        ('rl_fwd', C.c_int32), ('rl_inv', C.c_int32), ('threads_fwd', C.c_int32), ('threads_inv', C.c_int32),
        ('upsample_rows_tb', C.c_int32), ('upsample_rows_kc', C.c_int32),
        ('grid_fwd', C.c_int32 * 2), ('grid_col', C.c_int32 * 2), ('grid_inv', C.c_int32 * 2),
        ('grid_up_rows', C.c_int32 * 2),
        ('lds_fwd', C.c_int64), ('lds_col', C.c_int64), ('lds_inv', C.c_int64),
    ]


class _ArenaInfo(C.Structure):
    _fields_ = [('base_dev', C.c_void_p), ('bytes', C.c_int64), ('slice_bytes', C.c_int64), ('n_slices', C.c_int32),
                ('n_candidates', C.c_int32), ('n_classes', C.c_int32), ('class_slices', C.c_int32 * 8),
                ('class_candidates', C.c_int32 * 8), ('interleaved', C.c_int32),
                ('probe_ms', C.c_float), ('create_ms', C.c_float), ('min_pair_gbs', C.c_float), ('max_pair_gbs', C.c_float)]


class _BasicInfo(C.Structure):
    _fields_ = [('reweight_iterations', C.c_int32), ('ladmap_iterations', C.c_int32), ('working_size', C.c_int32),
                ('capped_rounds', C.c_int32)]


EXPORTS = {
    'sq_version': (C.c_int, []),
    'sq_last_error': (C.c_char_p, []),
    'sq_fuse_plan_create': (C.c_void_p, [C.c_void_p, C.c_int32, C.c_int32, C.c_int32, C.c_int32, C.c_int32, C.c_int32]),
    'sq_fuse_plan_create_spans': (C.c_void_p, [C.c_void_p, C.c_int32, C.c_int32, C.c_int32, C.c_int32, C.c_int32, C.c_int32]),
    'sq_fuse_plan_expand_scratch_bytes': (C.c_int64, [C.c_void_p]),
    'sq_fuse_plan_expand': (C.c_int, [C.c_void_p, C.c_void_p, C.c_int64, C.c_void_p, C.c_int64, C.c_void_p]),
    'sq_fuse_plan_destroy': (None, [C.c_void_p]),
    'sq_fuse_plan_table_bytes': (C.c_int64, [C.c_void_p]),
    'sq_fuse_plan_upload': (C.c_int, [C.c_void_p, C.c_void_p, C.c_int64, C.c_void_p]),
    'sq_fuse_plan_export': (C.c_int, [C.c_void_p, C.c_void_p, C.c_int64]),
    'sq_fuse_plan_stats': (C.c_int, [C.c_void_p, C.POINTER(C.c_int64), C.POINTER(C.c_int64),
                                     C.POINTER(C.c_int64), C.POINTER(C.c_int32)]),
    'sq_fuse_planes': (C.c_int, [C.POINTER(_FuseArgs), C.c_void_p]),
    'sq_fuse_project_max': (C.c_int, [C.POINTER(_FuseArgs), C.c_int32, C.c_void_p]),
    'sq_focus_scratch_bytes': (C.c_int64, [C.c_int32, C.c_int32, C.c_int32]),
    'sq_fuse_project_focus': (C.c_int, [C.POINTER(_FuseArgs), C.POINTER(_FocusArgs), C.c_int32, C.c_void_p]),
    'sq_focus_depth_plane': (C.c_int, [C.c_void_p, C.c_int32, C.c_int32, C.c_int32, C.c_void_p, C.c_int32, C.c_int32, C.c_void_p]),
    'sq_fuse_select_depth': (C.c_int, [C.POINTER(_FuseArgs), C.c_void_p, C.c_int32, C.c_int32, C.c_void_p, C.c_int32, C.c_void_p]),
    'sq_tile_minmax': (C.c_int, [C.c_void_p, C.c_void_p, C.c_int64, C.c_int32, C.c_int32, C.c_int32, C.c_int32,
                                 C.c_int32, C.c_void_p, C.c_void_p]),
    'sq_pair_overlap_moments': (C.c_int, [C.c_void_p, C.c_void_p, C.c_int64, C.c_int32, C.c_int32, C.c_int32, C.c_int32,
                                          C.c_int32, C.c_void_p, C.c_int32, C.c_void_p, C.c_void_p]),
    'sq_normalize_tiles': (C.c_int, [C.c_void_p, C.c_void_p, C.c_int64, C.c_int32, C.c_int32, C.c_int32, C.c_int32,
                                     C.c_int32, C.c_void_p, C.c_void_p, C.c_void_p]),
    'sq_downsample2': (C.c_int, [C.c_void_p, C.c_int64, C.c_int32, C.c_int32, C.c_int64, C.c_void_p, C.c_int64, C.c_int64,
                                 C.c_int32, C.c_int32, C.c_void_p]),
    'sq_pyramid_mean': (C.c_int, [C.c_void_p, C.c_int64, C.c_int32, C.c_int32, C.c_int64, C.POINTER(C.c_void_p),
                                  C.POINTER(C.c_int64), C.POINTER(C.c_int64), C.c_int32, C.c_int32, C.c_int32, C.c_void_p]),
    'sq_histogram_planes': (C.c_int, [C.c_void_p, C.c_int64, C.c_int32, C.c_int32, C.c_int64, C.c_int32, C.c_int32,
                                      C.POINTER(C.c_int32), C.c_int32, C.c_void_p, C.c_void_p]),
    'sq_block_mean': (C.c_int, [C.c_void_p, C.c_int64, C.c_int32, C.c_int32, C.c_int64, C.c_int32, C.c_int32, C.c_int32, C.c_int32,
                                C.c_int32, C.c_void_p, C.c_int64, C.c_int64, C.c_void_p]),
    'sq_composite_render': (C.c_int, [C.c_void_p, C.c_int64, C.c_int32, C.c_int32, C.c_int64, C.c_int32, C.c_int32,
                                      C.POINTER(C.c_int32), C.POINTER(C.c_uint32), C.c_void_p, C.c_int64, C.c_void_p]),
    'sq_tophat_scratch_bytes': (C.c_int64, [C.c_int32, C.c_int32, C.c_int32, C.c_int32]),
    'sq_tophat_tiles': (C.c_int, [C.c_void_p, C.c_int32, C.c_int32, C.c_int32, C.c_int64, C.c_int64, C.c_int32, C.c_int32,
                                  C.c_void_p, C.c_int64, C.c_void_p]),
    'sq_despeckle_tiles': (C.c_int, [C.c_void_p, C.c_void_p, C.c_int32, C.c_int32, C.c_int32, C.c_int64, C.c_int64, C.c_int64,
                                     C.c_int64, C.c_int32, C.c_int32, C.c_int32, C.c_void_p, C.c_void_p]),
    'sq_tile_stats': (C.c_int, [C.c_void_p, C.c_int32, C.c_int32, C.c_int32, C.c_int64, C.c_int64, C.c_int32, C.c_void_p, C.c_void_p]),
    'sq_seam_stats': (C.c_int, [C.c_void_p, C.c_int32, C.c_int32, C.c_int32, C.c_int32, C.c_int64, C.c_int64, C.c_int64, C.c_int32,
                                C.c_void_p, C.c_void_p, C.c_int32, C.c_int32, C.c_void_p, C.c_void_p]),
    'sq_dpc_tiles': (C.c_int, [C.c_void_p, C.c_void_p, C.c_void_p, C.c_int32, C.c_int32, C.c_int32, C.c_int64, C.c_int64, C.c_int64,
                               C.c_int64, C.c_int64, C.c_int64, C.c_int32, C.c_int32, C.c_void_p]),
    'sq_bin_tiles': (C.c_int, [C.c_void_p, C.c_void_p, C.c_int32, C.c_int32, C.c_int32, C.c_int64, C.c_int64, C.c_int64, C.c_int64,
                               C.c_int32, C.c_int32, C.c_int32, C.c_void_p]),
    'sq_warp_tiles': (C.c_int, [C.c_void_p, C.c_void_p, C.c_int32, C.c_int32, C.c_int32, C.c_int64, C.c_int64, C.c_int64, C.c_int64,
                                C.c_int32, C.c_int32, C.c_void_p]),
    'sq_shift_tiles': (C.c_int, [C.c_void_p, C.c_void_p, C.c_int32, C.c_int32, C.c_int32, C.c_int64, C.c_int64, C.c_int64, C.c_int64,
                                 C.c_int32, C.POINTER(C.c_int32), C.c_int32, C.c_void_p]),
    'sq_affine_tiles': (C.c_int, [C.c_void_p, C.c_void_p, C.c_int32, C.c_int32, C.c_int32, C.c_int64, C.c_int64, C.c_int64, C.c_int64,
                                  C.c_int32, C.POINTER(C.c_int32), C.c_int32, C.c_void_p]),
    'sq_dark_tiles': (C.c_int, [C.c_void_p, C.c_int32, C.c_int32, C.c_int32, C.c_int64, C.c_int64, C.c_int32, C.c_void_p, C.c_int32,
                                C.c_int64, C.c_int64, C.POINTER(C.c_int32), C.c_int32, C.c_int32, C.c_void_p]),
    'sq_register_line_supported': (C.c_int, [C.c_int32]),
    'sq_register_workspace_bytes': (C.c_int64, [C.c_int32, C.c_int32, C.c_int32, C.c_int32]),
    'sq_register_pairs': (C.c_int, [C.POINTER(_RegisterArgs), C.c_void_p]),
    'sq_register_describe': (C.c_int, [C.c_int32, C.c_int32, C.c_int32, C.c_int32, C.c_int32, C.POINTER(_RegisterPlan)]),
    'sq_selftest_flat_divide': (C.c_int, [C.c_int32, C.c_int32, C.c_int32, C.c_void_p, C.c_void_p]),
    'sq_selftest_flat_divide_f64': (C.c_int, [C.c_int32, C.c_int32, C.c_int32, C.c_uint64, C.c_void_p, C.c_void_p]),
    'sq_selftest_normalise_divide': (C.c_int, [C.c_void_p, C.c_void_p]),
    'sq_selftest_blend_divide': (C.c_int, [C.c_int32, C.c_int32, C.c_int32, C.c_void_p, C.c_void_p]),
    'sq_fuse_scratch_bytes': (C.c_int64, [C.c_int32]),
    'sq_arena_create': (C.c_void_p, [C.c_int64, C.c_int64, C.c_int64, C.c_int64, C.c_int32, C.c_void_p, C.POINTER(_ArenaInfo)]),
    'sq_arena_info_get': (C.c_int, [C.c_void_p, C.POINTER(_ArenaInfo)]),
    'sq_arena_destroy': (C.c_int, [C.c_void_p]),
    'sq_write_files': (C.c_int, [C.c_char_p, C.c_void_p, C.c_void_p, C.c_void_p, C.c_int64, C.c_int32, C.POINTER(C.c_int64)]),
    'sq_blosc_chunk_count': (C.c_int64, [C.c_int32] * 5),
    'sq_blosc_out_bound': (C.c_int64, [C.c_int32] * 6),
    'sq_blosc_scratch_bytes': (C.c_int64, [C.c_int32] * 6),
    'sq_blosc_encode_planes': (C.c_int, [C.c_void_p, C.c_int64, C.c_int64, C.c_int32, C.c_int32, C.c_int32, C.c_int32, C.c_int32,
                                         C.c_int32, C.c_void_p, C.c_int64, C.c_void_p, C.c_void_p, C.c_int64, C.c_void_p, C.c_void_p]),
    'sq_deflate_chunk_count': (C.c_int64, [C.c_int32] * 5),
    'sq_deflate_out_bound': (C.c_int64, [C.c_int32] * 6),
    'sq_deflate_scratch_bytes': (C.c_int64, [C.c_int32] * 6),
    'sq_deflate_encode_planes': (C.c_int, [C.c_void_p, C.c_int64, C.c_int64, C.c_int32, C.c_int32, C.c_int32, C.c_int32, C.c_int32,
                                           C.c_int32, C.c_int32, C.c_void_p, C.c_int64, C.c_void_p, C.c_void_p, C.c_int64, C.c_void_p,
                                           C.c_void_p]),
    'sq_basic_workspace_bytes': (C.c_int64, [C.c_int32, C.c_int32, C.c_int32]),
    'sq_basic_fit': (C.c_int, [C.c_void_p, C.c_void_p, C.c_int64, C.c_int32, C.c_int32, C.c_int32, C.c_int32, C.c_int32,
                               C.c_float, C.c_void_p, C.c_void_p, C.c_int64, C.POINTER(_BasicInfo), C.c_void_p]),
    'sq_synth_tiles': (C.c_int, [C.c_void_p, C.c_int32, C.c_int32, C.c_int32, C.c_int32, C.c_int32, C.c_void_p,
                                 C.c_void_p]),
}

_lib = None


def lib() -> C.CDLL:
    global _lib
    if _lib is None:
        if not os.path.exists(LIB_PATH):
            raise NativeError(
                f"{LIB_PATH} is missing: build it with `make -C {os.path.dirname(LIB_PATH)}` "
                "(hipcc --offload-arch=gfx950).  There is no CPU fallback.")
        import torch
        handle = C.CDLL(LIB_PATH)
        for name, (res, args) in EXPORTS.items():
            fn = getattr(handle, name)
            fn.restype = res
            fn.argtypes = args
        if handle.sq_version() != SQ_VERSION:
            raise NativeError(f"{LIB_PATH} is version {handle.sq_version()}, this binding expects {SQ_VERSION}: rebuild it")
        _lib = handle
    return _lib


def _check(status: int, what: str) -> None:
    if status < 0:
        raise NativeError(f"{what} failed ({status}): {lib().sq_last_error().decode()}", status)


def _size(n, what: str) -> int:
    n = int(n)
    _check(n, what)
    return n


def _int_in(value, lo: int, hi: int, what: str) -> int:
    if isinstance(value, bool) or not isinstance(value, (int, np.integer)) or not lo <= int(value) <= hi:
        raise ValueError(f"{what} must be an integer in {lo}..{hi}, got {value!r}")
    return int(value)


def sq_dtype_of(np_dtype) -> int:
    dt = np.dtype(np_dtype)
    table = {np.dtype('uint8'): SQ_U8, np.dtype('uint16'): SQ_U16, np.dtype('float32'): SQ_F32,
             np.dtype('float64'): SQ_F64}
    if dt not in table:
        raise ValueError(f"unsupported dtype {dt} (uint8/uint16 tiles, float32/float64 gains)")
    return table[dt]


def torch_dtype_of(np_dtype):
    import torch
    return {np.dtype('uint8'): torch.uint8, np.dtype('uint16'): torch.uint16,
            np.dtype('float32'): torch.float32, np.dtype('float64'): torch.float64}[np.dtype(np_dtype)]


def np_dtype_of_torch(t) -> np.dtype:
    import torch
    return {torch.uint8: np.dtype('uint8'), torch.uint16: np.dtype('uint16'),
            torch.float32: np.dtype('float32'), torch.float64: np.dtype('float64')}[t]


def _stream_ptr(stream=None) -> int:
    import torch
    s = stream if stream is not None else torch.cuda.current_stream()
    return int(s.cuda_stream)


def _on_stream(stream):
    if stream is None:
        return contextlib.nullcontext()
    import torch
    return torch.cuda.stream(stream)


def as_rects(rects) -> np.ndarray:
    if isinstance(rects, np.ndarray) and rects.dtype == RECT_DTYPE:
        return np.ascontiguousarray(rects)
    a = np.asarray(rects, dtype=np.int64).reshape(-1, 6)
    if a.size and (np.abs(a) >= 2 ** 31).any():
        raise ValueError("rectangle coordinate does not fit int32")
    out = np.zeros(len(a), dtype=RECT_DTYPE)
    for i, name in enumerate(RECT_DTYPE.names):
        out[name] = a[:, i]
    return out


EXPAND_MAX_TILE_H = 8176


class FusePlan:

    def __init__(self, rects, tile_h: int, tile_w: int, canvas_h: int, canvas_w: int, mode: int = SQ_FUSE_OVERWRITE,
                 expand_on_device: bool = False):
        L = lib()
        self.rects = as_rects(rects)
        self.tile_h, self.tile_w = int(tile_h), int(tile_w)
        self.canvas_h, self.canvas_w = int(canvas_h), int(canvas_w)
        self.mode = int(mode)
        self.n_tiles = len(self.rects)
        self.expand_on_device = bool(expand_on_device) and self.mode == SQ_FUSE_OVERWRITE and self.tile_h <= EXPAND_MAX_TILE_H
        create = L.sq_fuse_plan_create_spans if self.expand_on_device else L.sq_fuse_plan_create
        self._h = create(self.rects.ctypes.data if self.n_tiles else None, self.n_tiles,
                         self.tile_h, self.tile_w, self.canvas_h, self.canvas_w, self.mode)
        if not self._h:
            raise NativeError(f"sq_fuse_plan_create failed: {L.sq_last_error().decode()}")
        self.table_bytes = int(L.sq_fuse_plan_table_bytes(self._h))
        self._table = None
        ns, ni, cv, mr = C.c_int64(), C.c_int64(), C.c_int64(), C.c_int32()
        _check(L.sq_fuse_plan_stats(self._h, C.byref(ns), C.byref(ni), C.byref(cv), C.byref(mr)), 'sq_fuse_plan_stats')
        self.n_spans, self.n_items, self.covered_voxels, self.max_refs = ns.value, ni.value, cv.value, mr.value
        self._dev = {}
        import threading
        self._lock = threading.Lock()

    @property
    def handle(self) -> int:
        return self._h

    @property
    def table(self) -> np.ndarray:
        if self._table is None:
            if self.expand_on_device:
                if not self._dev:
                    raise NativeError("FusePlan.table: a plan expanded on the device has no host copy before device_table() has run")
                self._table = next(iter(self._dev.values())).cpu().numpy()
            else:
                self._table = np.empty(self.table_bytes, dtype=np.uint8)
                _check(lib().sq_fuse_plan_export(self._h, self._table.ctypes.data, self.table_bytes), 'sq_fuse_plan_export')
        return self._table

    def device_table(self, device):
        import torch
        key = str(device)
        with self._lock:
            return self._device_table_locked(key, device)

    def _device_table_locked(self, key, device):
        import torch
        if key not in self._dev:
            dev = _side_empty((max(self.table_bytes, 1),), torch.uint8, torch.device(device))
            with torch.cuda.device(dev.device):
                side = _copy_stream(dev.device)
                if self.expand_on_device:
                    need = _size(lib().sq_fuse_plan_expand_scratch_bytes(self._h), 'sq_fuse_plan_expand_scratch_bytes')
                    with torch.cuda.stream(side):
                        scratch = torch.empty(max(need, 1), dtype=torch.uint8, device=dev.device)
                    _check(lib().sq_fuse_plan_expand(self._h, dev.data_ptr(), dev.numel(), scratch.data_ptr(), scratch.numel(),
                                                     _stream_ptr(side)), 'sq_fuse_plan_expand')
                    del scratch
                else:
                    _check(lib().sq_fuse_plan_upload(self._h, dev.data_ptr(), dev.numel(), _stream_ptr(side)), 'sq_fuse_plan_upload')
            self._dev[key] = dev
        else:
            self._dev[key].record_stream(torch.cuda.current_stream(self._dev[key].device))
        return self._dev[key]

    def close(self) -> None:
        if getattr(self, '_h', None):
            lib().sq_fuse_plan_destroy(self._h)
            self._h = None

    def __del__(self):
        try:
            self.close()
        except Exception:
            pass


def _side_empty(shape, dtype, device):
    import torch
    device = torch.device(device)
    if device.index is None:
        device = torch.device('cuda', torch.cuda.current_device())
    with torch.cuda.stream(_copy_stream(device)):
        t = torch.empty(shape, dtype=dtype, device=device)
    t.record_stream(torch.cuda.current_stream(device))
    return t


def upload_small(host, device):
    import torch
    dst = _side_empty(tuple(host.shape), host.dtype, device)
    if dst.numel():
        with torch.cuda.stream(_copy_stream(dst.device)):
            dst.copy_(host)
    return dst


def pointer_table(tensors: Sequence, device):
    import torch
    ptrs = [0 if t is None else int(t.data_ptr()) for t in tensors]
    return upload_small(torch.tensor(ptrs, dtype=torch.int64), device)


def _fuse_args(plan: FusePlan, tiles, n_planes: int, out, plane_stride: int, pitch: int, flats, tile_ptrs, flat_ptrs, keep):
    import torch
    L = lib()
    hc, wc = int(out.shape[-2]), int(out.shape[-1])
    a = _FuseArgs()
    a.plan = plan.handle
    table = plan.device_table(out.device)
    a.table_dev = table.data_ptr()
    a.table_bytes = table.numel()
    keep.append(table)
    if tile_ptrs is not None:
        if tile_ptrs.dtype != torch.int64 or tile_ptrs.numel() != n_planes * plan.n_tiles:
            raise ValueError("tile_ptrs must be int64 with n_planes * n_tiles entries")
        a.tile_ptrs_dev = tile_ptrs.data_ptr()
        a.tile_base_dev = None
        tile_np = np_dtype_of_torch(out.dtype) if plan.mode == SQ_FUSE_OVERWRITE else np.dtype('uint16')
        if tiles is not None:
            tile_np = np_dtype_of_torch(tiles.dtype)
    else:
        if tiles is None or not tiles.is_cuda or not tiles.is_contiguous():
            raise ValueError("tiles must be a contiguous device tensor")
        if tiles.numel() != n_planes * plan.n_tiles * plan.tile_h * plan.tile_w:
            raise ValueError(f"tiles has {tiles.numel()} elements, expected "
                             f"{n_planes}x{plan.n_tiles}x{plan.tile_h}x{plan.tile_w}")
        a.tile_ptrs_dev = None
        a.tile_base_dev = tiles.data_ptr()
        a.tile_stride = plan.tile_h * plan.tile_w
        a.tile_plane_stride = plan.n_tiles * plan.tile_h * plan.tile_w
        tile_np = np_dtype_of_torch(tiles.dtype)
    a.n_tiles, a.tile_h, a.tile_w, a.tile_pitch = plan.n_tiles, plan.tile_h, plan.tile_w, plan.tile_w
    a.tile_dtype = sq_dtype_of(tile_np)
    a.flat_ptrs_dev = None
    a.flat_dtype = SQ_F32
    if flats is not None and any(f is not None for f in flats):
        if len(flats) != n_planes:
            raise ValueError("flats needs one entry per plane")
        dts = {f.dtype for f in flats if f is not None}
# ... 1246 lines not shown
```

### include/squidstitch.h

```cpp
#ifndef SQUIDSTITCH_H
#define SQUIDSTITCH_H

#include <stddef.h>
#include <stdint.h>

#ifdef __cplusplus
extern "C" {
#endif

#define SQ_VERSION 108

typedef enum sq_status {
    SQ_OK = 0,
    SQ_ERR_INVALID = -1,
    SQ_ERR_HIP = -2,
    SQ_ERR_UNSUPPORTED = -3,
    SQ_ERR_WORKSPACE = -4,
    SQ_ERR_NUMERIC = -5
} sq_status;

typedef enum sq_dtype { SQ_U8 = 1, SQ_U16 = 2, SQ_F32 = 4, SQ_F64 = 8 } sq_dtype;

int sq_version(void);
const char *sq_last_error(void);


typedef struct sq_rect {
    int32_t src_y0, src_x0;
    int32_t h, w;
    int32_t dst_y, dst_x;
} sq_rect;

typedef enum sq_fuse_mode {
    SQ_FUSE_OVERWRITE = 0,
    SQ_FUSE_FEATHER = 1
} sq_fuse_mode;

typedef struct sq_fuse_plan sq_fuse_plan;

sq_fuse_plan *sq_fuse_plan_create(const sq_rect *rects, int32_t n_rects, int32_t tile_h, int32_t tile_w,
                                  int32_t canvas_h, int32_t canvas_w, int32_t mode);
void sq_fuse_plan_destroy(sq_fuse_plan *plan);
int64_t sq_fuse_plan_table_bytes(const sq_fuse_plan *plan);
int sq_fuse_plan_export(const sq_fuse_plan *plan, void *host_buf, int64_t host_bytes);

int sq_fuse_plan_upload(const sq_fuse_plan *plan, void *table_dev, int64_t table_bytes, void *stream);
sq_fuse_plan *sq_fuse_plan_create_spans(const sq_rect *rects, int32_t n_rects, int32_t tile_h, int32_t tile_w,
                                        int32_t canvas_h, int32_t canvas_w, int32_t mode);
int64_t sq_fuse_plan_expand_scratch_bytes(const sq_fuse_plan *plan);
int sq_fuse_plan_expand(sq_fuse_plan *plan, void *table_dev, int64_t table_bytes, void *scratch_dev, int64_t scratch_bytes,
                        void *stream);
int sq_fuse_plan_stats(const sq_fuse_plan *plan, int64_t *n_spans, int64_t *n_items, int64_t *covered_voxels,
                       int32_t *max_refs);

typedef struct sq_fuse_args {
    const sq_fuse_plan *plan;
    const void *table_dev;
    int64_t table_bytes;
    const void *const *tile_ptrs_dev;
    const void *tile_base_dev;
    int64_t tile_plane_stride, tile_stride;
    int32_t n_tiles, tile_h, tile_w;
    int32_t tile_pitch;
    int32_t tile_dtype;
    const void *const *flat_ptrs_dev;
    int32_t flat_dtype;
    void *canvas_dev;
    int64_t canvas_plane_stride;
    int32_t canvas_h, canvas_w, canvas_pitch;
    int32_t canvas_dtype;
    int32_t n_planes;
    int32_t mode;
    void *scratch_dev;
    int64_t scratch_bytes;
    int32_t flags;
    int32_t grid_blocks;
} sq_fuse_args;

typedef enum sq_fuse_flags {
    SQ_FUSE_FORCE_QUEUES = 1,
    SQ_FUSE_FORCE_STATIC = 2,
    SQ_FUSE_NO_PLANE_GROUPS = 4,
    SQ_FUSE_NO_SEAM_OWNERS = 8,
    SQ_FUSE_CONSECUTIVE_GROUPS = 16
} sq_fuse_flags;

int64_t sq_fuse_scratch_bytes(int32_t n_planes);

int sq_fuse_planes(const sq_fuse_args *args, void *stream);

#define SQ_PROJECT_ACCUMULATE 32
int sq_fuse_project_max(const sq_fuse_args *args, int32_t flags, void *stream);

#define SQ_FOCUS_ACCUMULATE 32
#define SQ_FOCUS_MAX_RADIUS 15
#define SQ_FOCUS_MAX_PLANES 256
typedef struct sq_focus_args {
    const uint32_t *z_levels_dev;
    int32_t radius;
    void *scratch_dev;
    int64_t scratch_bytes;
    void *key_dev;
    int32_t key_pitch;
} sq_focus_args;
int64_t sq_focus_scratch_bytes(int32_t n_tiles, int32_t tile_h, int32_t tile_w);
int sq_fuse_project_focus(const sq_fuse_args *args, const sq_focus_args *focus, int32_t flags, void *stream);

#define SQ_SELECT_ACCUMULATE 32
int sq_focus_depth_plane(const void *key_dev, int32_t key_pitch, int32_t h, int32_t w, void *depth_dev, int32_t depth_pitch,
                         int32_t depth_dtype, void *stream);
int sq_fuse_select_depth(const sq_fuse_args *args, const void *depth_dev, int32_t depth_pitch, int32_t depth_dtype,
                         const uint32_t *z_levels_dev, int32_t flags, void *stream);

#define SQ_ARENA_MAX_CLASSES 8
typedef enum sq_arena_flags { SQ_ARENA_NATURAL_ORDER = 1, SQ_ARENA_TWO_CLASSES = 2 } sq_arena_flags;
typedef struct sq_arena sq_arena;
typedef struct sq_arena_info {
    void *base_dev;
    int64_t bytes;
    int64_t slice_bytes;
    int32_t n_slices;
    int32_t n_candidates;
    int32_t n_classes;
    int32_t class_slices[SQ_ARENA_MAX_CLASSES];
    int32_t class_candidates[SQ_ARENA_MAX_CLASSES];
    int32_t interleaved;
    float probe_ms;
    float create_ms;
    float min_pair_gbs, max_pair_gbs;
} sq_arena_info;
sq_arena *sq_arena_create(int64_t bytes, int64_t candidate_bytes, int64_t slice_bytes, int64_t unit_bytes, int32_t flags,
                          void *stream, sq_arena_info *info);
int sq_arena_info_get(const sq_arena *arena, sq_arena_info *info);
int sq_arena_destroy(sq_arena *arena);

int sq_downsample2(const void *src_dev, int64_t src_plane_stride, int32_t src_h, int32_t src_w, int64_t src_pitch,
                   void *dst_dev, int64_t dst_plane_stride, int64_t dst_pitch, int32_t n_planes, int32_t dtype,
                   void *stream);

#define SQ_PYRAMID_MEAN_MAX_LEVELS 5
int sq_pyramid_mean(const void *src_dev, int64_t src_plane_stride, int32_t src_h, int32_t src_w, int64_t src_pitch,
                    void *const *dst_dev, const int64_t *dst_plane_stride, const int64_t *dst_pitch, int32_t n_levels,
                    int32_t n_planes, int32_t dtype, void *stream);

int sq_histogram_planes(const void *planes_dev, int64_t plane_stride, int32_t h, int32_t w, int64_t pitch,
                        int32_t n_planes, int32_t dtype, const int32_t *row_of_plane, int32_t n_rows,
                        uint64_t *hist_dev, void *stream);

int sq_block_mean(const void *planes_dev, int64_t plane_stride, int32_t h, int32_t w, int64_t pitch, int32_t n_planes,
                  int32_t dtype, int32_t k, int32_t row0, int32_t n_rows, void *dst_dev, int64_t dst_plane_stride,
                  int64_t dst_pitch, void *stream);

int sq_composite_render(const void *means_dev, int64_t plane_stride, int32_t h, int32_t w, int64_t pitch, int32_t n_planes,
                        int32_t dtype, const int32_t *windows, const uint32_t *colors, uint8_t *rgb_dev, int64_t rgb_pitch,
                        void *stream);

#define SQ_TOPHAT_MAX_RADIUS 127
int64_t sq_tophat_scratch_bytes(int32_t n_images, int32_t h, int32_t w, int32_t dtype);
int sq_tophat_tiles(void *tiles_dev, int32_t n_images, int32_t h, int32_t w, int64_t plane_stride, int64_t pitch,
                    int32_t dtype, int32_t radius, void *scratch_dev, int64_t scratch_bytes, void *stream);

#define SQ_DESPECKLE_HOT  1
#define SQ_DESPECKLE_BOTH 2
int sq_despeckle_tiles(const void *src_dev, void *dst_dev, int32_t n_images, int32_t h, int32_t w,
                       int64_t src_plane_stride, int64_t src_pitch, int64_t dst_plane_stride, int64_t dst_pitch,
                       int32_t dtype, int32_t mode, int32_t threshold, uint64_t *counts_dev ,
                       void *stream);

#define SQ_TILE_STATS_WORDS 8
#define SQ_TILE_STATS_ROWS_PER_THREAD 64
int sq_tile_stats(const void *src_dev, int32_t n_images, int32_t h, int32_t w, int64_t plane_stride, int64_t pitch,
                  int32_t dtype, uint64_t *out_dev , void *stream);

#define SQ_DPC_MAX_GAIN 16
int sq_dpc_tiles(const void *left_dev, const void *right_dev, void *out_dev, int32_t n_images, int32_t h, int32_t w,
                 int64_t left_plane_stride, int64_t left_pitch, int64_t right_plane_stride, int64_t right_pitch,
                 int64_t out_plane_stride, int64_t out_pitch, int32_t dtype, int32_t gain, void *stream);

#define SQ_BIN_MEAN 1
#define SQ_BIN_SUM  2
#define SQ_BIN_MAX_FACTOR 8
int sq_bin_tiles(const void *src_dev, void *dst_dev, int32_t n_images, int32_t h, int32_t w,
                 int64_t src_plane_stride, int64_t src_pitch, int64_t dst_plane_stride, int64_t dst_pitch,
                 int32_t dtype, int32_t factor, int32_t method, void *stream);

#define SQ_WARP_MAX_PPM 50000
#define SQ_WARP_MAX_SIDE 65535
#define SQ_WARP_PLANES_PER_THREAD 16
int sq_warp_tiles(const void *src_dev, void *dst_dev, int32_t n_images, int32_t h, int32_t w,
                  int64_t src_plane_stride, int64_t src_pitch, int64_t dst_plane_stride, int64_t dst_pitch,
                  int32_t dtype, int32_t ppm, void *stream);

#define SQ_SHIFT_MAX 16384
#define SQ_SHIFT_MAX_SIDE 65535
#define SQ_SHIFT_ROWS_PER_THREAD 32
int sq_shift_tiles(const void *src_dev, void *dst_dev, int32_t n_images, int32_t h, int32_t w,
                   int64_t src_plane_stride, int64_t src_pitch, int64_t dst_plane_stride, int64_t dst_pitch,
                   int32_t dtype, const int32_t *shifts_host, int32_t images_per_shift, void *stream);

#define SQ_AFFINE_MAX_PPM 50000
#define SQ_AFFINE_MAX_SIDE 65535
#define SQ_AFFINE_PLANES_PER_THREAD 16
int sq_affine_tiles(const void *src_dev, void *dst_dev, int32_t n_images, int32_t h, int32_t w,
                    int64_t src_plane_stride, int64_t src_pitch, int64_t dst_plane_stride, int64_t dst_pitch,
                    int32_t dtype, const int32_t *params_host, int32_t images_per_param, void *stream);

#ifndef SQ_DARK_IMAGES_PER_THREAD
#define SQ_DARK_IMAGES_PER_THREAD 1
#endif
int sq_dark_tiles(void *tiles_dev, int32_t n_images, int32_t h, int32_t w, int64_t plane_stride, int64_t pitch, int32_t dtype,
                  const void *frames_dev, int32_t n_frames, int64_t frame_stride, int64_t frame_pitch,
                  const int32_t *params_host , int32_t images_per_param,
                  int32_t pedestal, void *stream);


int sq_tile_minmax(const void *const *tile_ptrs_dev, const void *tile_base_dev, int64_t tile_stride, int32_t n_tiles,
                   int32_t tile_h, int32_t tile_w, int32_t tile_pitch, int32_t tile_dtype,
                   uint32_t *out_minmax_dev, void *stream);

int sq_normalize_tiles(const void *const *tile_ptrs_dev, const void *tile_base_dev, int64_t tile_stride, int32_t n_tiles,
                       int32_t tile_h, int32_t tile_w, int32_t tile_pitch, int32_t tile_dtype,
                       const uint32_t *minmax_dev, void *out_dev, void *stream);

typedef enum sq_normalization {
    SQ_NORM_NONE = 0,
    SQ_NORM_PHASE = 1
} sq_normalization;

typedef struct sq_pair {
    int32_t ref_tile, mov_tile;
    int32_t ref_y0, ref_x0;
    int32_t mov_y0, mov_x0;
} sq_pair;

typedef struct sq_pair_result {
    int32_t coarse[2];
    int32_t fine[2];
    double ccmax_re, ccmax_im;
    double src_amp, tgt_amp;
} sq_pair_result;

typedef struct sq_register_args {
    const void *const *tile_ptrs_dev;
    const void *tile_base_dev;
    int64_t tile_stride;
    int32_t n_tiles, tile_h, tile_w, tile_pitch, tile_dtype;
    const uint32_t *minmax_dev;
    const sq_pair *pairs_dev;
    int32_t n_pairs;
    int32_t n0, n1;
    int32_t upsample_factor;
    int32_t normalization;
    sq_pair_result *results_dev;
    void *workspace_dev;
    int64_t workspace_bytes;
} sq_register_args;

int sq_register_line_supported(int32_t n);
int64_t sq_register_workspace_bytes(int32_t n_pairs, int32_t n0, int32_t n1, int32_t upsample_factor);
int sq_register_pairs(const sq_register_args *args, void *stream);

typedef struct sq_register_plan {
    int32_t m0, m1;
    int32_t long0, long1;
    int32_t gen0, gen1;
    int32_t nf0, nf1;
    uint8_t radix0[16], radix1[16];
    int32_t tc;
    int32_t share;
    int32_t col_threads;
    int32_t columns_single;
    int32_t columns_single_threads;
    int32_t rl_fwd, rl_inv;
    int32_t threads_fwd, threads_inv;
    int32_t upsample_rows_tb, upsample_rows_kc;
    int32_t grid_fwd[2], grid_col[2], grid_inv[2], grid_up_rows[2];
    int64_t lds_fwd, lds_col, lds_inv;
} sq_register_plan;
int sq_register_describe(int32_t n_pairs, int32_t n0, int32_t n1, int32_t upsample_factor, int32_t tile_dtype,
                         sq_register_plan *out);

typedef struct sq_overlap {
    int32_t ref_tile, mov_tile, ref_y0, ref_x0, mov_y0, mov_x0, h, w;
} sq_overlap;
int sq_pair_overlap_moments(const void *const *tile_ptrs_dev, const void *tile_base_dev, int64_t tile_stride, int32_t n_tiles,
                            int32_t tile_h, int32_t tile_w, int32_t tile_pitch, int32_t tile_dtype,
                            const sq_overlap *pairs_dev, int32_t n_pairs, uint64_t *out_dev, void *stream);

#define SQ_SEAM_MAX_RADIUS 3
int sq_seam_stats(const void *tiles_dev, int32_t n_planes, int32_t n_tiles, int32_t h, int32_t w, int64_t plane_stride,
                  int64_t tile_stride, int64_t pitch, int32_t dtype, const sq_overlap *pairs_host, const sq_overlap *pairs_dev,
                  int32_t n_pairs, int32_t radius, uint64_t *out_dev ,
                  void *stream);

int64_t sq_blosc_chunk_count(int32_t n_planes, int32_t h, int32_t w, int32_t chunk_h, int32_t chunk_w);
int64_t sq_blosc_out_bound(int32_t n_planes, int32_t h, int32_t w, int32_t dtype, int32_t chunk_h, int32_t chunk_w);
int64_t sq_blosc_scratch_bytes(int32_t n_planes, int32_t h, int32_t w, int32_t dtype, int32_t chunk_h, int32_t chunk_w);
int sq_blosc_encode_planes(const void *planes_dev, int64_t plane_stride, int64_t pitch, int32_t n_planes, int32_t h, int32_t w,
                           int32_t dtype, int32_t chunk_h, int32_t chunk_w, void *scratch_dev, int64_t scratch_bytes,
                           uint64_t *offsets_dev, void *out_dev, int64_t out_capacity, uint32_t *status_dev, void *stream);

int64_t sq_deflate_chunk_count(int32_t n_planes, int32_t h, int32_t w, int32_t tile_h, int32_t tile_w);
int64_t sq_deflate_out_bound(int32_t n_planes, int32_t h, int32_t w, int32_t dtype, int32_t tile_h, int32_t tile_w);
int64_t sq_deflate_scratch_bytes(int32_t n_planes, int32_t h, int32_t w, int32_t dtype, int32_t tile_h, int32_t tile_w);
int sq_deflate_encode_planes(const void *planes_dev, int64_t plane_stride, int64_t pitch, int32_t n_planes, int32_t h, int32_t w,
                             int32_t dtype, int32_t tile_h, int32_t tile_w, int32_t predictor, void *scratch_dev,
                             int64_t scratch_bytes, uint64_t *offsets_dev, void *out_dev, int64_t out_capacity,
                             uint32_t *status_dev, void *stream);

int sq_write_files(const char *paths, const int64_t *path_offsets, const void *data, const int64_t *data_offsets, int64_t n_files,
                   int32_t n_threads, int64_t *bytes_written);

typedef struct sq_basic_info {
    int32_t reweight_iterations;
    int32_t ladmap_iterations;
    int32_t working_size;
    int32_t capped_rounds;
} sq_basic_info;

int64_t sq_basic_workspace_bytes(int32_t n_images, int32_t tile_h, int32_t tile_w);
int sq_basic_fit(const void *const *tile_ptrs_dev, const void *tile_base_dev, int64_t tile_stride, int32_t n_images,
                 int32_t tile_h, int32_t tile_w, int32_t tile_pitch, int32_t tile_dtype, float smoothness_flatfield,
                 float *flatfield_dev, void *workspace_dev, int64_t workspace_bytes, sq_basic_info *info, void *stream);

int sq_selftest_flat_divide(int32_t exponent, int32_t n_binades, int32_t negative, uint64_t *mismatches_dev,
                            void *stream);

int sq_selftest_flat_divide_f64(int32_t exponent, int32_t n_binades, int32_t negative, uint64_t seed,
                                uint64_t *mismatches_dev, void *stream);

int sq_selftest_normalise_divide(uint64_t *mismatches_dev, void *stream);

int sq_selftest_blend_divide(int32_t exponent, int32_t n_binades, int32_t negative, uint64_t *mismatches_dev,
                             void *stream);

typedef struct sq_synth_tile {
    uint64_t scene_seed, noise_seed;
    int64_t oy, ox;
} sq_synth_tile;

int sq_synth_tiles(const sq_synth_tile *tiles_dev, int32_t n_tiles, int32_t tile_h, int32_t tile_w, int32_t noise_amp,
                   int32_t tile_dtype, void *out_dev, void *stream);

#ifdef __cplusplus
}
#endif
#endif
```

Measured before the change: 1.617 million.

## Merge flat classify, class share and plane grouping into one prepass kernel

Replaces the separate flat_classify, flat_class_share and single-thread build_groups launches with one fuse_prepass kernel. The last block, found through an atomic ticket, shares classes and builds plane groups, and the grouping is now computed in parallel per plane. The host plan builder is also restructured to emit items straight from spans in parallel, with phase timing and a thread-cap API added. This cuts kernel launches and serial work but adds last-block ticket synchronisation that is delicate to get right.

```diff
diff --git a/image-stitcher_amd/csrc/fuse.hip b/image-stitcher_amd/csrc/fuse.hip
--- a/image-stitcher_amd/csrc/fuse.hip
+++ b/image-stitcher_amd/csrc/fuse.hip
@@ -462,74 +462,92 @@
     }
 }
 
-__global__ __launch_bounds__(256) void build_groups_kernel(const void *const *flat_ptrs, const uint32_t *cls, uint32_t cls_mask,
-                                                          int n_planes, int64_t plane_stride_bytes, int zb, uint32_t *n_groups,
-                                                          PlaneGroup *groups, bool consecutive) {
-    constexpr int CAP = 1024;
-    __shared__ uint64_t key[CAP];
-    __shared__ int first[CAP], open_group[CAP];
-    __shared__ short members[CAP], dealt[CAP];
-    __shared__ PlaneGroup out[CAP];
-    const int tid = threadIdx.x;
-    if (n_planes > CAP || zb <= 1) {
+struct GroupArgs {
+    const void *const *gains;
+    uint32_t cls_mask;
+    int n_planes;
+    int64_t plane_stride_bytes;
+    int zb;
+    uint32_t *n_groups;
+    PlaneGroup *groups;
+    bool consecutive;
+};
+constexpr int GROUP_CAP = 1024;
+struct GroupScratch {
+    uint64_t key[GROUP_CAP];
+    short slots[GROUP_CAP], lead[GROUP_CAP], rank[GROUP_CAP], members[GROUP_CAP];
+    uint8_t cls[GROUP_CAP];
+};
+__device__ void build_groups(const GroupArgs &A, GroupScratch &S) {
+    const int tid = threadIdx.x, n_planes = A.n_planes, zb = A.zb;
+    if (n_planes > GROUP_CAP || zb <= 1) {
         for (int p = tid; p < n_planes; p += 256) {
             PlaneGroup g{};
             g.n = 1;
             g.plane[0] = p;
-            groups[p] = g;
-        }
-        if (tid == 0) *n_groups = (uint32_t)n_planes;
+            A.groups[p] = g;
+        }
+        if (tid == 0) *A.n_groups = (uint32_t)n_planes;
         return;
     }
     for (int p = tid; p < n_planes; p += 256) {
-        const void *f = flat_ptrs ? flat_ptrs[p] : nullptr;
-        const bool ok = flat_ptrs ? (f && (cls[p] & cls_mask) == 0) : true;
-        key[p] = ok ? ((reinterpret_cast<uint64_t>(f) << 7) | (uint64_t)(((int64_t)p * plane_stride_bytes) & 127) | (1ull << 63)) : 0;
-        open_group[p] = -1;
+        const void *f = A.gains ? A.gains[p] : nullptr;
+        const bool ok = A.gains ? (f && (S.cls[p] & A.cls_mask) == 0) : true;
+        S.key[p] = ok ? ((reinterpret_cast<uint64_t>(f) << 7) | (uint64_t)(((int64_t)p * A.plane_stride_bytes) & 127) | (1ull << 63)) : 0;
     }
     __syncthreads();
     for (int p = tid; p < n_planes; p += 256) {
-        int f = p;
-        if (key[p])
-            for (int q = 0; q < p; ++q)
-                if (key[q] == key[p]) {
-                    f = q;
-                    break;
-                }
-        first[p] = f;
+        const uint64_t k = S.key[p];
+        int lead = p, rank = 0, members = 1;
+        if (k) {
+            lead = -1;
+            members = 0;
+            for (int q = 0; q < n_planes; ++q)
+                if (S.key[q] == k) {
+                    if (lead < 0) lead = q;
+                    rank += q < p;
+                    ++members;
+                }
+        }
+        S.lead[p] = (short)lead;
+        S.rank[p] = (short)rank;
+        S.members[p] = (short)members;
+        S.slots[p] = (short)(!k ? 1 : (lead == p ? (members + zb - 1) / zb : 0));
     }
     __syncthreads();
-    if (tid == 0) {
-        int ng = 0;
-        for (int p = 0; p < n_planes; ++p) members[p] = dealt[p] = 0;
-        for (int p = 0; p < n_planes; ++p)
-            if (key[p]) ++members[first[p]];
-        for (int p = 0; p < n_planes; ++p) {
-            if (!key[p]) {
-                open_group[p] = ng++;
-            } else if (first[p] == p) {
-                open_group[p] = ng;
-                ng += (members[p] + zb - 1) / zb;
-            }
-        }
-        for (int g = 0; g < ng; ++g) out[g].n = 0;
-        for (int p = 0; p < n_planes; ++p) {
-            int g = open_group[p];
-            if (key[p]) {
-                const int lead = first[p];
-                const int j = dealt[lead]++;
-                g = open_group[lead] + (consecutive ? j / zb : j % ((members[lead] + zb - 1) / zb));
-            }
-            out[g].plane[out[g].n++] = p;
-        }
-        for (int g = 0; g < ng; ++g)
-            for (int z = out[g].n; z < 7; ++z) out[g].plane[z] = out[g].plane[0];
-        *n_groups = (uint32_t)ng;
-        first[0] = ng;
-    }
-    __syncthreads();
-    const int ng = first[0];
-    for (int g = tid; g < ng; g += 256) groups[g] = out[g];
+    for (int p = tid; p < n_planes; p += 256) {
+        const int lead = S.lead[p], j = S.rank[p], m = S.members[p];
+        int g = 0;
+        for (int q = 0; q < lead; ++q) g += S.slots[q];
+        int pos = 0, count = 1;
+        if (S.key[p]) {
+            const int key_groups = (m + zb - 1) / zb;
+            if (A.consecutive) {
+                g += j / zb;
+                pos = j % zb;
+                count = min(zb, m - (j / zb) * zb);
+            } else {
+                g += j % key_groups;
+                pos = j / key_groups;
+                count = (m - j % key_groups + key_groups - 1) / key_groups;
+            }
+        }
+        A.groups[g].plane[pos] = p;
+        if (pos == 0) {
+            A.groups[g].n = count;
+            for (int z = count; z < 7; ++z) A.groups[g].plane[z] = p;
+        }
+        if (p == n_planes - 1) {
+            int ng = 0;
+            for (int q = 0; q < n_planes; ++q) ng += S.slots[q];
+            *A.n_groups = (uint32_t)ng;
+        }
+    }
+}
+
+__global__ __launch_bounds__(256) void plane_groups_kernel(GroupArgs A) {
+    __shared__ GroupScratch S;
+    build_groups(A, S);
 }
 
 template <typename OutT>
@@ -1305,53 +1323,91 @@
     }
 }
 
+struct PrepassShared {
+    GroupScratch g;
+    int firsts;
+    uint32_t ticket;
+};
 template <typename G>
-__global__ __launch_bounds__(256) void flat_classify_kernel(const void *const *flat_ptrs, int64_t n, uint32_t *cls) {
+__global__ __launch_bounds__(256) void fuse_prepass_kernel(const void *const *flat_ptrs, int64_t n, int n_planes, uint32_t *cls,
+                                                          uint32_t *ticket, bool with_groups, GroupArgs A) {
+    __shared__ PrepassShared S;
     const int plane = blockIdx.y;
     const G *f = static_cast<const G *>(flat_ptrs[plane]);
-    if (!f) return;
-    for (int q = 0; q < plane; ++q)
-        if (flat_ptrs[q] == f) return;
-    const G lo = (G)__builtin_ldexp(1.0, FAST_MIN_EXP), hi = (G)__builtin_ldexp(1.0, FAST_END_EXP);
-    const G mlo = (G)__builtin_ldexp(1.0, -MODERATE_EXP), mhi = (G)__builtin_ldexp(1.0, MODERATE_EXP);
-    bool odd = false, wide = false, neg = false;
-    auto look = [&](G g) {
-        const G a = g < 0 ? -g : g;
-        odd |= !(a >= lo && a < hi);
-        wide |= !(a >= mlo && a < mhi);
-        neg |= !(g > 0);
+    if (f) {
+        for (int q = 0; q < plane; ++q)
+            if (flat_ptrs[q] == f) return;
+    } else if (blockIdx.x || blockIdx.y) {
+        return;
+    }
+    const bool reads = f != nullptr;
+    if (reads) {
+        const G lo = (G)__builtin_ldexp(1.0, FAST_MIN_EXP), hi = (G)__builtin_ldexp(1.0, FAST_END_EXP);
+        const G mlo = (G)__builtin_ldexp(1.0, -MODERATE_EXP), mhi = (G)__builtin_ldexp(1.0, MODERATE_EXP);
+        bool odd = false, wide = false, neg = false;
+        auto look = [&](G g) {
+            const G a = g < 0 ? -g : g;
+            odd |= !(a >= lo && a < hi);
+            wide |= !(a >= mlo && a < mhi);
+            neg |= !(g > 0);
+        };
+        constexpr int PER = 16 / sizeof(G);
+        const int64_t head = min<int64_t>(n, (int64_t)((16 - (reinterpret_cast<uintptr_t>(f) & 15)) & 15) / (int64_t)sizeof(G));
+        const int64_t nvec = (n - head) / PER;
+        const int64_t tid = (int64_t)blockIdx.x * blockDim.x + threadIdx.x, nthr = (int64_t)gridDim.x * blockDim.x;
+        for (int64_t v = tid; v < nvec; v += nthr) {
+            if constexpr (sizeof(G) == 4) {
+                const f32x4 q = *reinterpret_cast<const f32x4 *>(f + head + v * PER);
+                look(q[0]), look(q[1]), look(q[2]), look(q[3]);
+            } else {
+                const F64x2U q = *reinterpret_cast<const F64x2U *>(f + head + v * PER);
+                look(q.v[0]), look(q.v[1]);
+            }
+        }
+        for (int64_t i = tid; i < head; i += nthr) look(ldg_s<G>(f + i));
+        for (int64_t i = head + nvec * PER + tid; i < n; i += nthr) look(ldg_s<G>(f + i));
+        const uint32_t bits = (__builtin_amdgcn_ballot_w64(odd) ? 1u : 0u) | (__builtin_amdgcn_ballot_w64(wide) ? 2u : 0u) |
+                              (__builtin_amdgcn_ballot_w64(neg) ? 4u : 0u);
+        if (bits && (threadIdx.x & 63) == 0) __hip_atomic_fetch_or(&cls[plane], bits, __ATOMIC_RELAXED, __HIP_MEMORY_SCOPE_AGENT);
+    }
+    asm volatile("s_waitcnt vmcnt(0)" ::: "memory");
+    __syncthreads();
+    if (threadIdx.x == 0) S.ticket = reads ? __hip_atomic_fetch_add(ticket, 1u, __ATOMIC_RELAXED, __HIP_MEMORY_SCOPE_AGENT) : 0u;
+    __syncthreads();
+    if (reads && (S.ticket + 1u) % gridDim.x) return;
+    const bool in_lds = n_planes <= GROUP_CAP;
+    auto image_of = [&](int p) { return in_lds ? reinterpret_cast<const void *>(S.g.key[p]) : flat_ptrs[p]; };
+    auto first_with = [&](int p) {
+        const void *g = image_of(p);
+        if (!g) return -1;
+        int first = p;
+        for (int q = p - 1; q >= 0; --q)
+            if (image_of(q) == g) first = q;
+        return first;
     };
-    constexpr int PER = 16 / sizeof(G);
-    const int64_t head = min<int64_t>(n, (int64_t)((16 - (reinterpret_cast<uintptr_t>(f) & 15)) & 15) / (int64_t)sizeof(G));
-    const int64_t nvec = (n - head) / PER;
-    const int64_t tid = (int64_t)blockIdx.x * blockDim.x + threadIdx.x, nthr = (int64_t)gridDim.x * blockDim.x;
-    for (int64_t v = tid; v < nvec; v += nthr) {
-        if constexpr (sizeof(G) == 4) {
-            const f32x4 q = *reinterpret_cast<const f32x4 *>(f + head + v * PER);
-            look(q[0]), look(q[1]), look(q[2]), look(q[3]);
-        } else {
-            const F64x2U q = *reinterpret_cast<const F64x2U *>(f + head + v * PER);
-            look(q.v[0]), look(q.v[1]);
-        }
-    }
-    for (int64_t i = tid; i < head; i += nthr) look(ldg_s<G>(f + i));
-    for (int64_t i = head + nvec * PER + tid; i < n; i += nthr) look(ldg_s<G>(f + i));
-    const uint32_t bits = (__builtin_amdgcn_ballot_w64(odd) ? 1u : 0u) | (__builtin_amdgcn_ballot_w64(wide) ? 2u : 0u) |
-                          (__builtin_amdgcn_ballot_w64(neg) ? 4u : 0u);
-    if (bits && (threadIdx.x & 63) == 0) atomicOr(&cls[plane], bits);
-}
-
-__global__ __launch_bounds__(256) void flat_class_share_kernel(const void *const *flat_ptrs, int n_planes, uint32_t *cls) {
+    if (in_lds)
+        for (int p = threadIdx.x; p < n_planes; p += 256) S.g.key[p] = reinterpret_cast<uint64_t>(flat_ptrs[p]);
+    if (threadIdx.x == 0) S.firsts = 0;
+    __syncthreads();
+    for (int p = threadIdx.x; p < n_planes; p += 256)
+        if (first_with(p) == p) atomicAdd(&S.firsts, 1);
+    __syncthreads();
+    if (reads ? S.ticket + 1u != (uint32_t)S.firsts * gridDim.x : S.firsts != 0) return;
+    if (threadIdx.x == 0) {
+        __builtin_amdgcn_fence(__ATOMIC_ACQUIRE, "agent");
+        asm volatile("s_waitcnt vmcnt(0)" ::: "memory");
+    }
+    __syncthreads();
     for (int p = threadIdx.x; p < n_planes; p += 256) {
-        const void *f = flat_ptrs[p];
-        if (!f) continue;
-        for (int q = 0; q < p; ++q)
-            if (flat_ptrs[q] == f) {
-                cls[p] = cls[q];
-                break;
-            }
-    }
-}
+        const int q = first_with(p);
+        const uint32_t c = q < 0 ? 0u : __hip_atomic_load(&cls[q], __ATOMIC_RELAXED, __HIP_MEMORY_SCOPE_AGENT);
+        if (q >= 0 && q != p) cls[p] = c;
+        if (p < GROUP_CAP) S.g.cls[p] = (uint8_t)c;
+    }
+    __syncthreads();
+    if (with_groups) build_groups(A, S.g);
+}
+
 
 __global__ __launch_bounds__(256) void selftest_divide_kernel(int exponent0, int negative, unsigned long long *bad) {
     const uint32_t mant = blockIdx.x * 256u + threadIdx.x;
@@ -1485,33 +1541,31 @@
         if (const int rc = scratch_check(who, a, SL)) return rc;
         if (hipMemsetAsync(a->scratch_dev, 0, (size_t)SL.groups, stream) != hipSuccess)
             return fail(SQ_ERR_HIP, "sq_fuse_planes: cannot clear the scratch");
-        if (flat) {
-            if (flat == 1)
-                hipLaunchKernelGGL(flat_classify_kernel<float>, dim3(256, a->n_planes), dim3(256), 0, stream, a->flat_ptrs_dev,
-                                   (int64_t)a->tile_h * a->tile_w, static_cast<uint32_t *>(a->scratch_dev));
-            else
-                hipLaunchKernelGGL(flat_classify_kernel<double>, dim3(256, a->n_planes), dim3(256), 0, stream, a->flat_ptrs_dev,
-                                   (int64_t)a->tile_h * a->tile_w, static_cast<uint32_t *>(a->scratch_dev));
-            if (a->n_planes > 1)
-                hipLaunchKernelGGL(flat_class_share_kernel, dim3(1), dim3(256), 0, stream, a->flat_ptrs_dev, a->n_planes,
-                                   static_cast<uint32_t *>(a->scratch_dev));
-            P.flat_class = static_cast<const uint32_t *>(a->scratch_dev);
-        }
+        if (flat) P.flat_class = static_cast<const uint32_t *>(a->scratch_dev);
         if ((n_work >= 100000 || (fl & SQ_FUSE_FORCE_QUEUES)) && n_work < (int64_t(1) << 31) && !(fl & SQ_FUSE_FORCE_STATIC))
             P.queue = reinterpret_cast<uint32_t *>(static_cast<char *>(a->scratch_dev) + SL.queue);
     }
     const int64_t min_units = h.n_items * ((a->n_planes + ZB - 1) / ZB);
     const bool u16 = a->tile_dtype == SQ_U16;
     const bool grouping = a->scratch_dev && a->n_planes > 1 && ZB > 1 && !(fl & SQ_FUSE_NO_PLANE_GROUPS);
-    auto build_groups = [&](const void *const *gains, uint32_t cls_mask) {
+    auto prepass = [&](bool groups_too, const void *const *gains, uint32_t cls_mask) {
+        if (!a->scratch_dev || a->n_planes <= 0) return;
         char *sc = static_cast<char *>(a->scratch_dev);
         uint32_t *n_groups = reinterpret_cast<uint32_t *>(sc + SL.n_groups);
-        PlaneGroup *groups = reinterpret_cast<PlaneGroup *>(sc + SL.groups);
-        hipLaunchKernelGGL(build_groups_kernel, dim3(1), dim3(256), 0, stream, gains, P.flat_class, cls_mask, a->n_planes,
-                           a->canvas_plane_stride * (int64_t)esz, ZB, n_groups, groups,
-                           (fl & SQ_FUSE_CONSECUTIVE_GROUPS) != 0);
-        P.groups = groups;
-        P.n_groups = n_groups;
+        GroupArgs G{gains, cls_mask, a->n_planes, a->canvas_plane_stride * (int64_t)esz, ZB, n_groups,
+                    reinterpret_cast<PlaneGroup *>(sc + SL.groups), (fl & SQ_FUSE_CONSECUTIVE_GROUPS) != 0};
+        if (flat == 1)
+            hipLaunchKernelGGL(fuse_prepass_kernel<float>, dim3(256, a->n_planes), dim3(256), 0, stream, a->flat_ptrs_dev,
+                               (int64_t)a->tile_h * a->tile_w, a->n_planes, static_cast<uint32_t *>(a->scratch_dev), n_groups + 1, groups_too, G);
+        else if (flat == 2)
+            hipLaunchKernelGGL(fuse_prepass_kernel<double>, dim3(256, a->n_planes), dim3(256), 0, stream, a->flat_ptrs_dev,
+                               (int64_t)a->tile_h * a->tile_w, a->n_planes, static_cast<uint32_t *>(a->scratch_dev), n_groups + 1, groups_too, G);
+        else if (groups_too)
+            hipLaunchKernelGGL(plane_groups_kernel, dim3(1), dim3(256), 0, stream, G);
+        if (groups_too) {
+            P.groups = G.groups;
+            P.n_groups = n_groups;
+        }
     };
 
     if (a->mode == SQ_FUSE_OVERWRITE) {
@@ -1524,8 +1578,8 @@
         return launch(who, fuse_overwrite_kernel<T, F, false>, P, n_work, stream, a->grid_blocks, h.n_items, n_work);        \
     } while (0)
         if (flat && grouping) {
-            build_groups(a->flat_ptrs_dev, 1u);
-#define SQ_ZG(G, T)                                                                                                                  \
+            prepass(true, a->flat_ptrs_dev, 1u);
+#define SQ_ZG(G, T)                                                                                                                 \
     do {                                                                                                                              \
         if (P.queue) return launch(who, fuse_overwrite_zg_kernel<G, true, T>, P, min_units, stream, a->grid_blocks, h.n_items);          \
         return launch(who, fuse_overwrite_zg_kernel<G, false, T>, P, min_units, stream, a->grid_blocks, h.n_items);                      \
@@ -1538,10 +1592,11 @@
             SQ_ZG(float, uint8_t);
         }
         if (u16 && !flat && grouping) {
-            build_groups(nullptr, 0u);
+            prepass(true, nullptr, 0u);
             SQ_ZG(NoGain, uint16_t);
 #undef SQ_ZG
         }
+        prepass(false, nullptr, 0u);
         if (u16) {
             if (flat == 0) SQ_OVERWRITE(uint16_t, 0);
             if (flat == 1) SQ_OVERWRITE(uint16_t, 1);
@@ -1567,7 +1622,7 @@
         SQ_FEATHER_F(T, O, 2);           \
     } while (0)
     if (u16 && grouping && std::min(a->tile_h, a->tile_w) <= BLEND_WSUM_MAX) {
-        build_groups(a->flat_ptrs_dev, f32out ? 7u : 3u);
+        prepass(true, a->flat_ptrs_dev, f32out ? 7u : 3u);
 #define SQ_FEATHER_ZG(F, O)                                                                                                      \
     do {                                                                                                                          \
         if (P.queue) return launch(who, fuse_feather_zg_kernel<F, true, O>, P, min_units, stream, a->grid_blocks, h.n_items);          \
@@ -1583,6 +1638,7 @@
         SQ_FEATHER_ZG(0, uint16_t);
 #undef SQ_FEATHER_ZG
     }
+    prepass(false, nullptr, 0u);
     if (u16) {
         if (f32out) SQ_FEATHER(uint16_t, float);
         SQ_FEATHER(uint16_t, uint16_t);
diff --git a/image-stitcher_amd/csrc/plan.cpp b/image-stitcher_amd/csrc/plan.cpp
--- a/image-stitcher_amd/csrc/plan.cpp
+++ b/image-stitcher_amd/csrc/plan.cpp
@@ -1,6 +1,8 @@
 #include <hip/hip_runtime.h>
 
 #include <algorithm>
+#include <chrono>
+#include <condition_variable>
 #include <cstdlib>
 #include <cstring>
 #include <exception>
@@ -21,34 +23,119 @@
 
 namespace {
 
+class Workers {
+public:
+    using Call = void (*)(void *, int);
+    void run(int n, Call call, void *ctx) {
+        std::unique_lock<std::mutex> section(submit_, std::try_to_lock);
+        if (!section.owns_lock()) {
+            for (int t = 0; t < n; ++t) call(ctx, t);
+            return;
+        }
+        start();
+        std::unique_lock<std::mutex> lock(m_);
+        call_ = call;
+        ctx_ = ctx;
+        n_tasks_ = n;
+        next_ = finished_ = 0;
+        lock.unlock();
+        wake_.notify_all();
+        lock.lock();
+        while (next_ < n_tasks_) {
+            const int t = next_++;
+            lock.unlock();
+            call(ctx, t);
+            lock.lock();
+            ++finished_;
+        }
+        done_.wait(lock, [&] { return finished_ == n_tasks_; });
+        n_tasks_ = next_ = finished_ = 0;
+    }
+    ~Workers() {
+        {
+            std::lock_guard<std::mutex> lock(m_);
+            stop_ = true;
+        }
+        wake_.notify_all();
+        for (auto &th : threads_) th.join();
+    }
+
+private:
+    void start() {
+        if (started_) return;
+        started_ = true;
+        const int want = (int)std::max(1u, std::min(8u, std::thread::hardware_concurrency())) - 1;
+        try {
+            threads_.reserve(want);
+            for (int i = 0; i < want; ++i) threads_.emplace_back([this] { loop(); });
+        } catch (...) {
+        }
+    }
+    void loop() {
+        std::unique_lock<std::mutex> lock(m_);
+        for (;;) {
+            wake_.wait(lock, [&] { return stop_ || next_ < n_tasks_; });
+            if (stop_) return;
+            const int t = next_++;
+            const Call call = call_;
+            void *const ctx = ctx_;
+            lock.unlock();
+            call(ctx, t);
+            lock.lock();
+            if (++finished_ == n_tasks_) done_.notify_all();
+        }
+    }
+    std::mutex submit_;
+    std::mutex m_;
+    std::condition_variable wake_, done_;
+    std::vector<std::thread> threads_;
+    bool started_ = false, stop_ = false;
+    Call call_ = nullptr;
+    void *ctx_ = nullptr;
+    int n_tasks_ = 0, next_ = 0, finished_ = 0;
+};
+Workers g_workers;
+
+thread_local int g_thread_cap = 0;
+thread_local double g_phase_ms[6];
+double now_ms() { return std::chrono::duration<double, std::milli>(std::chrono::steady_clock::now().time_since_epoch()).count(); }
+
+int plan_threads(unsigned most) {
+    const int hw = (int)std::max(1u, std::min(most, std::thread::hardware_concurrency()));
+    return g_thread_cap > 0 ? std::min(g_thread_cap, hw) : hw;
+}
+
+template <typename F>
+void parallel_tasks(int n_tasks, F task) {
+    if (n_tasks <= 1) {
+        if (n_tasks == 1) task(0);
+        return;
+    }
+    struct Section {
+        F *task;
+        std::exception_ptr failed;
+        std::mutex failed_mutex;
+    } S{&task, nullptr, {}};
+    g_workers.run(n_tasks, [](void *ctx, int t) {
+        Section &s = *static_cast<Section *>(ctx);
+        try {
+            (*s.task)(t);
+        } catch (...) {
+            std::lock_guard<std::mutex> lock(s.failed_mutex);
+            if (!s.failed) s.failed = std::current_exception();
+        }
+    }, &S);
+    if (S.failed) std::rethrow_exception(S.failed);
+}
+
 template <typename F>
 void parallel_ranges(int nthreads, size_t n, F fn) {
     if (nthreads <= 1 || n == 0) {
         fn(0, (size_t)0, n);
         return;
     }
-    std::vector<std::thread> pool;
-    pool.reserve(nthreads - 1);
-    std::exception_ptr failed;
-    std::mutex failed_mutex;
     auto bound = [&](int t) { return n * (size_t)t / (size_t)nthreads; };
-    auto run = [&](int t) {
-        try {
-            fn(t, bound(t), bound(t + 1));
-        } catch (...) {
-            std::lock_guard<std::mutex> lock(failed_mutex);
-            if (!failed) failed = std::current_exception();
-        }
-    };
-    try {
-        for (int t = 1; t < nthreads; ++t) pool.emplace_back(run, t);
-    } catch (...) {
-        std::lock_guard<std::mutex> lock(failed_mutex);
-        if (!failed) failed = std::current_exception();
-    }
-    run(0);
-    for (auto &th : pool) th.join();
-    if (failed) std::rethrow_exception(failed);
+    parallel_tasks(nthreads, [&](int t) { fn(t, bound(t), bound(t + 1)); });
 }
 
 template <typename F>
@@ -142,8 +229,9 @@
     int64_t covered = 0;
 };
 
-bool make_spans(const sq_rect *rects, int32_t n_rects, int32_t tile_h, int32_t tile_w, int32_t canvas_h, int32_t canvas_w,
-                int32_t mode, const char *who, SpanStage &S) {
+template <int CAP>
+bool make_spans_of(const sq_rect *rects, int32_t n_rects, int32_t tile_h, int32_t tile_w, int32_t canvas_h, int32_t canvas_w,
+                   int32_t mode, const char *who, SpanStage &S) {
     std::vector<Span> &spans = S.spans;
     std::vector<Ref> &refs = S.refs;
     int &max_refs = S.max_refs;
@@ -192,7 +280,7 @@
 
     struct Owners {
         int n = 0;
-        int v[MAX_REFS];
+        int v[CAP];
         bool operator==(const Owners &o) const {
             if (n != o.n) return false;
             for (int i = 0; i < n; ++i)
@@ -203,86 +291,76 @@
     struct Run {
         int xa, xb;
         Owners own;
+        int64_t index;
+    };
+    struct Part {
+        std::vector<Span> spans;
+        std::vector<Ref> refs;
+        std::vector<Run> first, last;
+        int64_t covered = 0;
+        int max_refs = 0;
+        int overflow_at = -1, overflow_x = 0;
     };
     const size_t n_bands = ys.size() - 1;
-    const int hw_sweep = (int)std::max(1u, std::min(16u, std::thread::hardware_concurrency()));
-    const int sweep_threads = n_bands >= 512 ? hw_sweep : 1;
-    std::vector<std::vector<Run>> runs_of(sweep_threads);
-    std::vector<std::vector<uint32_t>> run_end(sweep_threads);
-    std::vector<size_t> first_band(sweep_threads + 1, 0);
-    std::vector<int> overflow_at(sweep_threads, -1);
-    std::vector<int> overflow_x(sweep_threads, 0);
+    const int sweep_threads = n_bands >= 512 ? plan_threads(16u) : 1;
+    std::vector<Part> parts(sweep_threads);
     parallel_ranges(sweep_threads, n_bands, [&](int t, size_t b_lo, size_t b_hi) {
-        first_band[t] = b_lo;
-        if (t + 1 == sweep_threads) first_band[t + 1] = n_bands;
-        std::vector<Run> &out = runs_of[t];
-        std::vector<uint32_t> &ends = run_end[t];
-        out.reserve((b_hi - b_lo) * 72);
-        ends.reserve(b_hi - b_lo);
+        Part &part = parts[t];
         if (b_lo >= b_hi) return;
+        std::vector<Run> out, open;
         std::vector<int> active;
         const int y_first = ys[b_lo];
         for (size_t i = 0; i < cl.size(); ++i)
             if (cl[i].y0 <= y_first && cl[i].y1 > y_first) active.push_back((int)i);
         size_t next = (size_t)(std::upper_bound(by_y0.begin(), by_y0.end(), y_first, [&](int y, int i) { return y < cl[i].y0; }) - by_y0.begin());
-        std::vector<int> xs, owner_of, skip;
+        auto edge = [&](int i, bool begins) { return ((uint64_t)(begins ? cl[i].x0 : cl[i].x1) << 33) | ((uint64_t)(uint32_t)i << 1) | (begins ? 1u : 0u); };
+        std::vector<uint64_t> edges;
+        edges.reserve(2 * active.size() + 16);
+        for (int i : active) {
+            edges.push_back(edge(i, true));
+            edges.push_back(edge(i, false));
+        }
+        std::sort(edges.begin(), edges.end());
+        auto put = [&](uint64_t e) { edges.insert(std::upper_bound(edges.begin(), edges.end(), e), e); };
+        auto take = [&](uint64_t e) { edges.erase(std::lower_bound(edges.begin(), edges.end(), e)); };
+        std::vector<int> cover;
         for (size_t b = b_lo; b < b_hi; ++b) {
             const int ya = ys[b];
             while (next < by_y0.size() && cl[by_y0[next]].y0 <= ya) {
-                active.insert(std::upper_bound(active.begin(), active.end(), by_y0[next]), by_y0[next]);
+                const int i = by_y0[next];
+                active.insert(std::upper_bound(active.begin(), active.end(), i), i);
+                put(edge(i, true));
+                put(edge(i, false));
                 ++next;
             }
-            active.erase(std::remove_if(active.begin(), active.end(), [&](int i) { return cl[i].y1 <= ya; }), active.end());
-
-            xs.clear();
-            xs.push_back(0);
-            xs.push_back(canvas_w);
-            for (int i : active) {
-                xs.push_back(cl[i].x0);
-                xs.push_back(cl[i].x1);
-            }
-            std::sort(xs.begin(), xs.end());
-            xs.erase(std::unique(xs.begin(), xs.end()), xs.end());
-            const size_t m = xs.size() - 1;
-            if (mode == SQ_FUSE_OVERWRITE) {
-                owner_of.assign(m, -1);
-                skip.resize(m + 1);
-                for (size_t k = 0; k <= m; ++k) skip[k] = (int)k;
-                auto find = [&](int k) {
-                    while (skip[k] != k) k = skip[k] = skip[skip[k]];
-                    return k;
-                };
-                for (size_t a = active.size(); a-- > 0;) {
-                    const Clipped &c = cl[active[a]];
-                    const int lo = (int)(std::lower_bound(xs.begin(), xs.end(), c.x0) - xs.begin());
-                    const int hi = (int)(std::lower_bound(xs.begin(), xs.end(), c.x1) - xs.begin());
-                    for (int k = find(lo); k < hi; k = find(k + 1)) {
-                        owner_of[k] = active[a];
-                        skip[k] = k + 1;
+            active.erase(std::remove_if(active.begin(), active.end(), [&](int i) {
+                if (cl[i].y1 > ya) return false;
+                take(edge(i, true));
+                take(edge(i, false));
+                return true;
+            }), active.end());
+
+            bool have = false;
+            Run cur{};
+            cover.clear();
+            auto interval = [&](int xa, int xb) {
+                if (xa >= xb) return;
+                Owners own;
+                if (mode == SQ_FUSE_OVERWRITE) {
+                    if (!cover.empty()) own.v[own.n++] = cover.back();
+                } else {
+                    for (int i : cover) {
+                        if (own.n == CAP) {
+                            if (part.overflow_at < 0) {
+                                part.overflow_at = ya;
+                                part.overflow_x = xa;
+                            }
+                            break;
+                        }
+                        own.v[own.n++] = i;
                     }
                 }
-            }
-            bool have = false;
-            Run cur{};
-            for (size_t k = 0; k < m; ++k) {
-                const int xa = xs[k], xb = xs[k + 1];
-                Owners own;
-                if (mode == SQ_FUSE_OVERWRITE) {
-                    if (owner_of[k] >= 0) own.v[own.n++] = owner_of[k];
-                } else {
-                    for (int i : active)
-                        if (cl[i].x0 <= xa && cl[i].x1 >= xb) {
-                            if (own.n == MAX_REFS) {
-                                if (overflow_at[t] < 0) {
-                                    overflow_at[t] = ya;
-                                    overflow_x[t] = xa;
-                                }
-                                break;
-                            }
-                            own.v[own.n++] = i;
-                        }
-                }
-                if (have && cur.own == own && cur.xb == xa) {
+                if (have && cur.own == own) {
                     cur.xb = xb;
                 } else {
                     if (have) out.push_back(cur);
@@ -291,61 +369,91 @@
                     cur.own = own;
                     have = true;
                 }
+            };
+            int x_at = 0;
+            for (size_t e = 0; e < edges.size();) {
+                const int x = (int)(edges[e] >> 33);
+                interval(x_at, x);
+                for (; e < edges.size() && (int)(edges[e] >> 33) == x; ++e) {
+                    const int i = (int)(uint32_t)((edges[e] >> 1) & 0xFFFFFFFFu);
+                    if (edges[e] & 1) cover.insert(std::upper_bound(cover.begin(), cover.end(), i), i);
+                    else cover.erase(std::lower_bound(cover.begin(), cover.end(), i));
+                }
+                x_at = x;
             }
+            interval(x_at, canvas_w);
             if (have) out.push_back(cur);
-            ends.push_back((uint32_t)out.size());
-        }
-    });
-    for (int t = 0; t < sweep_threads; ++t)
-        if (overflow_at[t] >= 0) {
-            fail(SQ_ERR_UNSUPPORTED, "%s: more than %d tiles overlap at canvas (%d,%d)", who, MAX_REFS, overflow_at[t],
-                 overflow_x[t]);
-            return false;
-        }
-    struct Open {
-        int xa, xb;
-        int64_t index;
-        const Run *run;
-    };
-    std::vector<Open> open, open_next;
-    for (int t = 0; t < sweep_threads; ++t) {
-        const std::vector<Run> &rs = runs_of[t];
-        size_t at = 0;
-        for (size_t k = 0; k < run_end[t].size(); ++k) {
-            const size_t b = first_band[t] + k;
-            const int ya = ys[b], yb = ys[b + 1];
-            open_next.clear();
+            const int yb = ys[b + 1];
             size_t op = 0;
-            for (; at < run_end[t][k]; ++at) {
-                const Run &cur = rs[at];
-                while (op < open.size() && open[op].xa < cur.xa) ++op;
-                int64_t index;
-                if (op < open.size() && open[op].xa == cur.xa && open[op].xb == cur.xb && open[op].run->own == cur.own) {
-                    index = open[op].index;
-                    spans[index].h += yb - ya;
+            for (Run &r : out) {
+                while (op < open.size() && open[op].xa < r.xa) ++op;
+                if (op < open.size() && open[op].xa == r.xa && open[op].xb == r.xb && open[op].own == r.own) {
+                    r.index = open[op].index;
+                    part.spans[r.index].h += yb - ya;
                 } else {
                     Span sp{};
                     sp.dst_y = ya;
-                    sp.dst_x = cur.xa;
+                    sp.dst_x = r.xa;
                     sp.h = yb - ya;
-                    sp.w = cur.xb - cur.xa;
-                    sp.nref = cur.own.n;
-                    sp.ref0 = (int)refs.size();
-                    for (int q = 0; q < cur.own.n; ++q) {
-                        const Clipped &c = cl[cur.own.v[q]];
-                        refs.push_back({c.tile, c.src_y + (ya - c.y0), c.src_x + (cur.xa - c.x0), 0});
+                    sp.w = r.xb - r.xa;
+                    sp.nref = r.own.n;
+                    sp.ref0 = (int)part.refs.size();
+                    for (int q = 0; q < r.own.n; ++q) {
+                        const Clipped &c = cl[r.own.v[q]];
+                        part.refs.push_back({c.tile, c.src_y + (ya - c.y0), c.src_x + (r.xa - c.x0), 0});
                     }
-                    index = (int64_t)spans.size();
-                    spans.push_back(sp);
+                    r.index = (int64_t)part.spans.size();
+                    part.spans.push_back(sp);
                 }
-                open_next.push_back({cur.xa, cur.xb, index, &cur});
-                if (cur.own.n) covered += (int64_t)(yb - ya) * (cur.xb - cur.xa);
-                max_refs = std::max(max_refs, cur.own.n);
+                if (r.own.n) part.covered += (int64_t)(yb - ya) * (r.xb - r.xa);
+                part.max_refs = std::max(part.max_refs, r.own.n);
             }
-            open.swap(open_next);
-        }
+            if (b == b_lo) part.first = out;
+            open.swap(out);
+            out.clear();
+        }
+        part.last.swap(open);
+    });
+    for (const Part &part : parts)
+        if (part.overflow_at >= 0) {
+            fail(SQ_ERR_UNSUPPORTED, "%s: more than %d tiles overlap at canvas (%d,%d)", who, MAX_REFS, part.overflow_at,
+                 part.overflow_x);
+            return false;
+        }
+    std::vector<Run> above;
+    std::vector<int64_t> number;
+    for (Part &part : parts) {
+        if (part.spans.empty()) continue;
+        number.assign(part.spans.size(), -1);
+        size_t op = 0;
+        for (const Run &r : part.first) {
+            while (op < above.size() && above[op].xa < r.xa) ++op;
+            if (op < above.size() && above[op].xa == r.xa && above[op].xb == r.xb && above[op].own == r.own) {
+                number[r.index] = above[op].index;
+                spans[above[op].index].h += part.spans[r.index].h;
+            }
+        }
+        for (size_t i = 0; i < part.spans.size(); ++i) {
+            if (number[i] >= 0) continue;
+            Span sp = part.spans[i];
+            const size_t ref0 = (size_t)sp.ref0;
+            sp.ref0 = (int)refs.size();
+            refs.insert(refs.end(), part.refs.begin() + (long)ref0, part.refs.begin() + (long)(ref0 + (size_t)sp.nref));
+            number[i] = (int64_t)spans.size();
+            spans.push_back(sp);
+        }
+        above.swap(part.last);
+        for (Run &r : above) r.index = number[r.index];
+        covered += part.covered;
+        max_refs = std::max(max_refs, part.max_refs);
     }
     return true;
+}
+
+bool make_spans(const sq_rect *rects, int32_t n_rects, int32_t tile_h, int32_t tile_w, int32_t canvas_h, int32_t canvas_w,
+                int32_t mode, const char *who, SpanStage &S) {
+    if (mode == SQ_FUSE_FEATHER) return make_spans_of<MAX_REFS>(rects, n_rects, tile_h, tile_w, canvas_h, canvas_w, mode, who, S);
+    return make_spans_of<1>(rects, n_rects, tile_h, tile_w, canvas_h, canvas_w, mode, who, S);
 }
 }
 
@@ -354,7 +462,10 @@
 static sq_fuse_plan *plan_create_impl(const sq_rect *rects, int32_t n_rects, int32_t tile_h, int32_t tile_w,
                                       int32_t canvas_h, int32_t canvas_w, int32_t mode) {
     SpanStage S;
+    for (double &ms : g_phase_ms) ms = 0;
+    const double t_sweep = now_ms();
     if (!make_spans(rects, n_rects, tile_h, tile_w, canvas_h, canvas_w, mode, "sq_fuse_plan_create", S)) return nullptr;
+    g_phase_ms[0] = now_ms() - t_sweep;
     std::vector<Span> &spans = S.spans;
     std::vector<Ref> &refs = S.refs;
     const int max_refs = S.max_refs;
@@ -364,118 +475,82 @@
     const int nblk = tile_h / BLOCK_ROWS + 2;
     const bool ow_mode = mode == SQ_FUSE_OVERWRITE;
     auto rows_of = [&](const Span &sp) { return (!ow_mode && sp.nref >= 2) ? FEATHER_BLEND_ROWS : BLOCK_ROWS; };
-    auto col_pieces = [&](const Span &sp) {
+    auto col_pieces = [&](const Span &sp, int32_t &first, int32_t &last) {
         int n = 0;
+        first = last = 0;
         for (int c0 = 0; c0 < sp.w; ++n) {
             int cols = std::min(BLOCK_COLS, sp.w - c0);
             const int rest = sp.w - c0 - cols;
             if (ow_mode && rest > 0 && rest < SEAM_MIN_COLS) cols -= SEAM_MIN_COLS;
+            if (!n) first = cols;
+            last = cols;
             c0 += cols;
         }
         return n;
     };
-    std::vector<size_t> span_first(spans.size() + 1, 0);
-    for (size_t si = 0; si < spans.size(); ++si) {
+    double t_phase = now_ms();
+    const size_t ns = spans.size();
+    std::vector<size_t> span_first(ns + 1, 0);
+    std::vector<int32_t> pieces(ns), first_cols(ns), last_cols(ns);
+    for (size_t si = 0; si < ns; ++si) {
         const Span &sp = spans[si];
         const int item_rows = rows_of(sp);
         const int64_t row_steps = sp.h <= 0 ? 0
                                   : (ow_mode ? ((int64_t)(sp.dst_y + sp.h - 1) / item_rows - sp.dst_y / item_rows + 1)
                                              : ((int64_t)sp.h + item_rows - 1) / item_rows);
-        span_first[si + 1] = span_first[si] + (size_t)(row_steps * col_pieces(sp));
-    }
-    static thread_local std::vector<Item> items_tls;
-    static thread_local std::vector<Seam> seams_tls;
-    static thread_local std::vector<int32_t> by_band_tls;
-    std::vector<Item> &items = items_tls;
-    std::vector<Seam> &seams = seams_tls;
-    std::vector<int32_t> &by_band = by_band_tls;
-    items.resize(span_first.back());
-    const int hw_threads = (int)std::max(1u, std::min(8u, std::thread::hardware_concurrency()));
-    const int nthreads = items.size() >= 32768 ? hw_threads : 1;
-    parallel_ranges(nthreads, spans.size(), [&](int, size_t si_lo, size_t si_hi) {
-        for (size_t si = si_lo; si < si_hi; ++si) {
+        pieces[si] = col_pieces(sp, first_cols[si], last_cols[si]);
+        span_first[si + 1] = span_first[si] + (size_t)(row_steps * pieces[si]);
+    }
+    const int64_t n_items = (int64_t)span_first.back();
+    const int nthreads = n_items >= 32768 ? plan_threads(8u) : 1;
+    std::vector<size_t> cut(nthreads + 1, ns);
+    for (int t = 0; t < nthreads; ++t)
+        cut[t] = (size_t)(std::lower_bound(span_first.begin(), span_first.begin() + (long)ns, (size_t)n_items * (size_t)t / (size_t)nthreads) -
+                          span_first.begin());
+
+    using EdgeSpan = std::pair<uint64_t, int32_t>;
+    std::vector<EdgeSpan> by_right, by_left;
+    if (ow_mode) {
+        by_right.reserve(ns);
+        by_left.reserve(ns);
+        for (size_t si = 0; si < ns; ++si) {
             const Span &sp = spans[si];
-            const bool ow = ow_mode;
-            const Ref *rf = (ow && sp.nref) ? &refs[sp.ref0] : nullptr;
-            const int item_rows = rows_of(sp);
-            Item *out = items.data() + span_first[si];
-            for (int r0 = 0; r0 < sp.h;) {
-                const int rows = std::min(ow ? item_rows - (sp.dst_y + r0) % item_rows : item_rows, sp.h - r0);
-                for (int c0 = 0; c0 < sp.w;) {
-                    int cols = std::min(BLOCK_COLS, sp.w - c0);
-                    const int rest = sp.w - c0 - cols;
-                    if (ow && rest > 0 && rest < SEAM_MIN_COLS) cols -= SEAM_MIN_COLS;
-                    Item it;
-                    it.dst_y = sp.dst_y + r0;
-                    it.dst_x = sp.dst_x + c0;
-                    it.hw = (rows << 16) | cols;
-                    it.nref = sp.nref;
-                    it.span = (int32_t)si;
-                    if (ow) {
-                        it.a = rf ? rf->tile : -1;
-                        it.b = rf ? rf->src_y + r0 : 0;
-                        it.c = rf ? rf->src_x + c0 : 0;
-                    } else {
-                        it.a = sp.ref0;
-                        it.b = r0;
-                        it.c = c0;
-                    }
-                    *out++ = it;
-                    c0 += cols;
-                }
-                r0 += rows;
-            }
-        }
-    });
-    const int64_t n_items = (int64_t)items.size();
-
-    seams.clear();
-    if (mode == SQ_FUSE_OVERWRITE) {
-        seams.assign(items.size(), Seam{-1, 0, 0, 0});
-        const int nb = canvas_h / BLOCK_ROWS + 1;
-        std::vector<int32_t> first(nb + 1, 0);
-        by_band.resize(items.size());
-        for (const Item &it : items) ++first[it.dst_y / BLOCK_ROWS + 1];
-        for (int k = 0; k < nb; ++k) first[k + 1] += first[k];
-        {
-            std::vector<int32_t> at(first.begin(), first.end() - 1);
-            for (size_t i = 0; i < items.size(); ++i) by_band[at[items[i].dst_y / BLOCK_ROWS]++] = (int32_t)i;
-        }
-        auto end_key = [&](int32_t i) { return ((int64_t)items[i].dst_y << 32) | (uint32_t)(items[i].dst_x + (items[i].hw & 0xFFFF)); };
-        parallel_ranges(nthreads, (size_t)nb, [&](int, size_t k_lo, size_t k_hi) {
-            for (size_t k = k_lo; k < k_hi; ++k)
-                std::sort(by_band.begin() + first[k], by_band.begin() + first[k + 1],
-                          [&](int32_t a, int32_t b) { return end_key(a) < end_key(b); });
-        });
-        parallel_ranges(nthreads, items.size(), [&](int, size_t j_lo, size_t j_hi) {
-            for (size_t j = j_lo; j < j_hi; ++j) {
-                const Item &J = items[j];
-                if ((J.hw & 0xFFFF) < SEAM_MIN_COLS || J.dst_x == 0) continue;
-                const int k = J.dst_y / BLOCK_ROWS;
-                const int64_t want = ((int64_t)J.dst_y << 32) | (uint32_t)J.dst_x;
-                auto lo = std::lower_bound(by_band.begin() + first[k], by_band.begin() + first[k + 1], want,
-                                           [&](int32_t a, int64_t key) { return end_key(a) < key; });
-                if (lo == by_band.begin() + first[k + 1] || end_key(*lo) != want) continue;
-                const Item &I = items[*lo];
-                const int in = I.hw & 0xFFFF;
-                if ((I.hw >> 16) != (J.hw >> 16) || in < SEAM_MIN_COLS) continue;
-                seams[j].a = I.a;
-                seams[j].b = I.b;
-                seams[j].c = I.c + in;
-                __atomic_fetch_or(&seams[j].flags, SEAM_HAS_LEFT | (I.nref ? 0 : SEAM_LEFT_ZERO), __ATOMIC_RELAXED);
-                __atomic_fetch_or(&seams[*lo].flags, SEAM_LEAVE_TAIL, __ATOMIC_RELAXED);
-            }
-        });
-    }
-
-    auto key_of = [&](const Item &it) {
-        if (!ow_mode) return it.nref ? std::min((refs[it.a].src_y + it.b) / BLOCK_ROWS, nblk - 2) : nblk - 1;
-        return it.nref ? std::min(it.b / BLOCK_ROWS, nblk - 2) : nblk - 1;
+            by_right.push_back({((uint64_t)(uint32_t)(sp.dst_x + sp.w) << 32) | (uint32_t)sp.dst_y, (int32_t)si});
+            by_left.push_back({((uint64_t)(uint32_t)sp.dst_x << 32) | (uint32_t)sp.dst_y, (int32_t)si});
+        }
+        std::sort(by_right.begin(), by_right.end());
+        std::sort(by_left.begin(), by_left.end());
+    }
+    auto locate = [](const std::vector<EdgeSpan> &tab, int x, int y) {
+        const auto it = std::upper_bound(tab.begin(), tab.end(), EdgeSpan{((uint64_t)(uint32_t)x << 32) | (uint32_t)y, INT32_MAX});
+        return it == tab.begin() ? (size_t)0 : (size_t)(it - tab.begin()) - 1;
+    };
+    auto covering = [&](const std::vector<EdgeSpan> &tab, size_t &at, int x, int y) -> int32_t {
+        while (at + 1 < tab.size() && (int)(tab[at].first >> 32) == x && spans[tab[at].second].dst_y + spans[tab[at].second].h <= y) ++at;
+        if (at >= tab.size() || (int)(tab[at].first >> 32) != x) return -1;
+        const Span &s = spans[tab[at].second];
+        return (s.dst_y <= y && y < s.dst_y + s.h) ? tab[at].second : -1;
+    };
+    auto row_matches = [](const Span &s, int y, int rows) {
+        return (y % BLOCK_ROWS == 0 || s.dst_y == y) && std::min(BLOCK_ROWS - y % BLOCK_ROWS, s.dst_y + s.h - y) == rows;
+    };
+
+    auto key_of = [&](const Span &sp, int r0) {
+        return sp.nref ? std::min((refs[sp.ref0].src_y + r0) / BLOCK_ROWS, nblk - 2) : nblk - 1;
+    };
+    auto rows_at = [&](const Span &sp, int item_rows, int r0) {
+        return std::min(ow_mode ? BLOCK_ROWS - (sp.dst_y + r0) % BLOCK_ROWS : item_rows, sp.h - r0);
     };
     std::vector<std::vector<int64_t>> hist(nthreads, std::vector<int64_t>(nblk, 0));
-    parallel_ranges(nthreads, items.size(), [&](int t, size_t lo, size_t hi) {
+    g_phase_ms[1] = now_ms() - t_phase;
+    t_phase = now_ms();
+    parallel_tasks(nthreads, [&](int t) {
         std::vector<int64_t> &h = hist[t];
-        for (size_t i = lo; i < hi; ++i) ++h[key_of(items[i])];
+        for (size_t si = cut[t]; si < cut[t + 1]; ++si) {
+            const Span &sp = spans[si];
+            const int item_rows = rows_of(sp);
+            for (int r0 = 0; r0 < sp.h; r0 += rows_at(sp, item_rows, r0)) h[key_of(sp, r0)] += pieces[si];
+        }
     });
     std::vector<int64_t> count(nblk, 0);
     for (int t = 0; t < nthreads; ++t)
@@ -499,6 +574,7 @@
     }
 
     auto *plan = new sq_fuse_plan;
+    const bool with_seams = ow_mode && n_items > 0;
     TableHeader hd{};
     hd.magic = TABLE_MAGIC;
     hd.mode = mode;
@@ -516,8 +592,8 @@
     hd.off_refs = hd.off_spans + hd.n_spans * (int64_t)sizeof(Span);
     hd.off_items = hd.off_refs + hd.n_refs * (int64_t)sizeof(Ref);
     hd.covered_voxels = covered;
-    hd.off_seams = seams.empty() ? 0 : hd.off_items + hd.n_items * (int64_t)sizeof(Item);
-    const int64_t total = hd.off_items + hd.n_items * (int64_t)sizeof(Item) + (int64_t)(seams.size() * sizeof(Seam));
+    hd.off_seams = with_seams ? hd.off_items + hd.n_items * (int64_t)sizeof(Item) : 0;
+    const int64_t total = hd.off_items + hd.n_items * (int64_t)sizeof(Item) + (with_seams ? hd.n_items * (int64_t)sizeof(Seam) : 0);
     if (!plan->table.allocate((size_t)total)) {
         delete plan;
         fail(SQ_ERR_INVALID, "sq_fuse_plan_create: out of host memory for a %lld-byte table", (long long)total);
@@ -528,33 +604,94 @@
     if (!spans.empty()) std::memcpy(p + hd.off_spans, spans.data(), spans.size() * sizeof(Span));
     if (!refs.empty()) std::memcpy(p + hd.off_refs, refs.data(), refs.size() * sizeof(Ref));
     Item *dst = reinterpret_cast<Item *>(p + hd.off_items);
-    Seam *dst_seam = seams.empty() ? nullptr : reinterpret_cast<Seam *>(p + hd.off_seams);
-    auto place = [&](int64_t pos, size_t i) {
-        dst[pos] = items[i];
-        if (dst_seam) dst_seam[pos] = seams[i];
-    };
-    parallel_ranges(nthreads, items.size(), [&](int th, size_t lo, size_t hi) {
-        std::vector<int64_t> seen = hist[th];
-        for (size_t i = lo; i < hi; ++i) {
-            const int k = key_of(items[i]);
-            const int64_t j = seen[k]++;
-            int64_t pos;
-            if (k == nblk - 1) {
-                pos = zero_at + j;
-            } else {
-                const int x = k % NX;
-                const int64_t t = lane_base[k] + j;
-                pos = t < common ? t * NX + x : tail_at[x] + (t - common);
+    Seam *dst_seam = with_seams ? reinterpret_cast<Seam *>(p + hd.off_seams) : nullptr;
+    g_phase_ms[4] = now_ms() - t_phase;
+    t_phase = now_ms();
+    try {
+        parallel_tasks(nthreads, [&](int th) {
+            std::vector<int64_t> seen = hist[th];
+            for (size_t si = cut[th]; si < cut[th + 1]; ++si) {
+                const Span &sp = spans[si];
+                const bool ow = ow_mode;
+                const Ref *rf = (ow && sp.nref) ? &refs[sp.ref0] : nullptr;
+                const int item_rows = rows_of(sp);
+                const bool seam_left = ow && sp.dst_x > 0 && first_cols[si] >= SEAM_MIN_COLS;
+                const bool seam_right = ow && sp.dst_x + sp.w < canvas_w && last_cols[si] >= SEAM_MIN_COLS;
+                size_t left_at = seam_left ? locate(by_right, sp.dst_x, sp.dst_y) : 0;
+                size_t right_at = seam_right ? locate(by_left, sp.dst_x + sp.w, sp.dst_y) : 0;
+                for (int r0 = 0; r0 < sp.h;) {
+                    const int rows = rows_at(sp, item_rows, r0);
+                    const int k = key_of(sp, r0);
+                    Seam *first_seam = nullptr, *sm = nullptr;
+                    int before = 0, before_c = 0;
+                    for (int c0 = 0; c0 < sp.w;) {
+                        int cols = std::min(BLOCK_COLS, sp.w - c0);
+                        const int rest = sp.w - c0 - cols;
+                        if (ow && rest > 0 && rest < SEAM_MIN_COLS) cols -= SEAM_MIN_COLS;
+                        const int64_t j = seen[k]++;
+                        int64_t pos;
+                        if (k == nblk - 1) {
+                            pos = zero_at + j;
+                        } else {
+                            const int x = k % NX;
+                            const int64_t t = lane_base[k] + j;
+                            pos = t < common ? t * NX + x : tail_at[x] + (t - common);
+                        }
+                        Item it;
+                        it.dst_y = sp.dst_y + r0;
+                        it.dst_x = sp.dst_x + c0;
+                        it.hw = (rows << 16) | cols;
+                        it.nref = sp.nref;
+                        it.span = (int32_t)si;
+                        if (ow) {
+                            it.a = rf ? rf->tile : -1;
+                            it.b = rf ? rf->src_y + r0 : 0;
+                            it.c = rf ? rf->src_x + c0 : 0;
+                            Seam *const prev = sm;
+                            sm = dst_seam + pos;
+                            if (!first_seam) first_seam = sm;
+                            if (c0 > 0 && cols >= SEAM_MIN_COLS && before >= SEAM_MIN_COLS) {
+                                *sm = Seam{it.a, it.b, before_c + before, SEAM_HAS_LEFT | (sp.nref ? 0 : SEAM_LEFT_ZERO)};
+                                prev->flags |= SEAM_LEAVE_TAIL;
+                            } else {
+                                *sm = Seam{-1, 0, 0, 0};
+                            }
+                            before_c = it.c;
+                        } else {
+                            it.a = sp.ref0;
+                            it.b = r0;
+                            it.c = c0;
+                        }
+                        dst[pos] = it;
+                        before = cols;
+                        c0 += cols;
+                    }
+                    if (seam_left) {
+                        const int y = sp.dst_y + r0;
+                        const int32_t li = covering(by_right, left_at, sp.dst_x, y);
+                        if (li >= 0 && row_matches(spans[li], y, rows) && last_cols[li] >= SEAM_MIN_COLS) {
+                            const Span &l = spans[li];
+                            const Ref *lr = l.nref ? &refs[l.ref0] : nullptr;
+                            first_seam->a = lr ? lr->tile : -1;
+                            first_seam->b = lr ? lr->src_y + (y - l.dst_y) : 0;
+                            first_seam->c = lr ? lr->src_x + l.w : last_cols[li];
+                            first_seam->flags |= SEAM_HAS_LEFT | (l.nref ? 0 : SEAM_LEFT_ZERO);
+                        }
+                    }
+                    if (seam_right) {
+                        const int y = sp.dst_y + r0;
+                        const int32_t ri = covering(by_left, right_at, sp.dst_x + sp.w, y);
+                        if (ri >= 0 && row_matches(spans[ri], y, rows) && first_cols[ri] >= SEAM_MIN_COLS) sm->flags |= SEAM_LEAVE_TAIL;
+                    }
+                    r0 += rows;
+                }
             }
-            place(pos, i);
-        }
-    });
-    constexpr size_t SCRATCH_KEEP_BYTES = (size_t)64 << 20;
-    if (items.capacity() * sizeof(Item) + seams.capacity() * sizeof(Seam) + by_band.capacity() * sizeof(int32_t) > SCRATCH_KEEP_BYTES) {
-        std::vector<Item>().swap(items);
-        std::vector<Seam>().swap(seams);
-        std::vector<int32_t>().swap(by_band);
-    }
+        });
+    } catch (...) {
+        delete plan;
+        throw;
+    }
+    g_phase_ms[5] = now_ms() - t_phase;
     return plan;
 }
 
@@ -565,7 +702,10 @@
         return nullptr;
     }
     SpanStage S;
+    for (double &ms : g_phase_ms) ms = 0;
+    const double t_sweep = now_ms();
     if (!make_spans(rects, n_rects, tile_h, tile_w, canvas_h, canvas_w, mode, "sq_fuse_plan_create_spans", S)) return nullptr;
+    g_phase_ms[0] = now_ms() - t_sweep;
     const size_t ns = S.spans.size();
     std::vector<int64_t> span_first(ns + 1, 0);
     for (size_t i = 0; i < ns; ++i) {
@@ -636,6 +776,17 @@
 
 void sq_fuse_plan_destroy(sq_fuse_plan *plan) { delete plan; }
 
+int32_t sq_fuse_plan_phase_ms(double *ms, int32_t n) {
+    for (int32_t i = 0; ms && i < n && i < 6; ++i) ms[i] = g_phase_ms[i];
+    return 6;
+}
+
+int32_t sq_fuse_plan_max_threads(int32_t n) {
+    const int32_t before = g_thread_cap;
+    g_thread_cap = n > 0 ? n : 0;
+    return before;
+}
+
 int sq_fuse_plan_upload(const sq_fuse_plan *plan, void *table_dev, int64_t table_bytes, void *stream_) {
     if (!plan || !table_dev) return fail(SQ_ERR_INVALID, "sq_fuse_plan_upload: NULL argument");
     if (plan->spans_only) return fail(SQ_ERR_INVALID, "sq_fuse_plan_upload: a plan of sq_fuse_plan_create_spans is completed on the device by sq_fuse_plan_expand");
diff --git a/image-stitcher_amd/native.py b/image-stitcher_amd/native.py
--- a/image-stitcher_amd/native.py
+++ b/image-stitcher_amd/native.py
@@ -119,6 +119,8 @@
     'sq_fuse_plan_export': (C.c_int, [C.c_void_p, C.c_void_p, C.c_int64]),
     'sq_fuse_plan_stats': (C.c_int, [C.c_void_p, C.POINTER(C.c_int64), C.POINTER(C.c_int64),
                                      C.POINTER(C.c_int64), C.POINTER(C.c_int32)]),
+    'sq_fuse_plan_phase_ms': (C.c_int32, [C.POINTER(C.c_double), C.c_int32]),
+    'sq_fuse_plan_max_threads': (C.c_int32, [C.c_int32]),
     'sq_fuse_planes': (C.c_int, [C.POINTER(_FuseArgs), C.c_void_p]),
     'sq_fuse_project_max': (C.c_int, [C.POINTER(_FuseArgs), C.c_int32, C.c_void_p]),
     'sq_focus_scratch_bytes': (C.c_int64, [C.c_int32, C.c_int32, C.c_int32]),
diff --git a/include/squidstitch.h b/include/squidstitch.h
--- a/include/squidstitch.h
+++ b/include/squidstitch.h
@@ -52,6 +52,8 @@
                         void *stream);
 int sq_fuse_plan_stats(const sq_fuse_plan *plan, int64_t *n_spans, int64_t *n_items, int64_t *covered_voxels,
                        int32_t *max_refs);
+int32_t sq_fuse_plan_phase_ms(double *ms, int32_t n);
+int32_t sq_fuse_plan_max_threads(int32_t n);
 
 typedef struct sq_fuse_args {
     const sq_fuse_plan *plan;
```

Measured after the change: 1.616 million. About the same (-0.1%).
